# daijifeng001/MNC

Hardware: AMD Instinct MI355X
Metric: images/sec (600x1000, 300 RoIs) VGG16 MNC-5stage (higher is better)
Workload: dtype f32; 1 GPU; VGG16 MNC 5-stage inference + gpu_mask_voting; one 600x1000 uint8 image per GPU per step (8 seeded images rotating), 300 RoIs per stage, H2D + device prep + forward + tail + gpu_mask_voting + D2H of the voted instances all inside the timed region; synthetic weights; math=fp32, images_in_flight_per_gpu=12, engine=native, parallelism=single GPU

## Files before the change

### include/mnc_hip.h

```cpp
#ifndef MNC_HIP_H_
#define MNC_HIP_H_

#include <stddef.h>

#ifdef __cplusplus
extern "C" {
#endif

#define MNC_API __attribute__((visibility("default")))

enum {
  MNC_OK = 0,
  MNC_ERR_INVALID = 1,
  MNC_ERR_HIP = 2,
  MNC_ERR_NOMEM = 3,
  MNC_ERR_STATE = 4,
  MNC_ERR_UNSUPPORTED = 5
};

MNC_API const char* mnc_last_error(void);
MNC_API int mnc_device_count(int* count);
MNC_API int mnc_device_mem_info(int device_id, size_t* free_bytes, size_t* total_bytes);
MNC_API const char* mnc_version(void);

MNC_API int mnc_nms(int* keep_out, int* num_out, const float* boxes_host, int boxes_num, int boxes_dim,
                    float nms_overlap_thresh, int device_id);
MNC_API int mnc_nms_topk(int* keep_out, int* num_out, const float* boxes_host, int boxes_num, int boxes_dim,
                         float nms_overlap_thresh, int max_keep, int device_id);
MNC_API int mnc_nms_batched(int* keep_out, int* num_out, const float* boxes_host, int boxes_num, int boxes_dim,
                            const int* order_host, int batch, float nms_overlap_thresh, int max_keep, int device_id);
MNC_API int mnc_nms_mask(unsigned long long* mask_host, const float* boxes_host, int boxes_num, int boxes_dim,
                         float nms_overlap_thresh, int device_id);
#if defined(__cplusplus) && defined(MNC_HIP_REF_CXX_NAMES)
}
MNC_API void _nms(int* keep_out, int* num_out, const float* boxes_host, int boxes_num, int boxes_dim,
                  float nms_overlap_thresh, int device_id);
MNC_API void _mv(const float* all_boxes, const float* all_masks, const int all_boxes_num, const int* candidate_inds,
                 const int* candidate_start, const float* candidate_weights, const int candidate_num,
                 const int image_height, const int image_width, const int box_dim, const int mask_size,
                 const int result_num, float* finalize_output_mask, int* finalize_output_box, const int device_id);
extern "C" {
#else
MNC_API void _nms(int* keep_out, int* num_out, const float* boxes_host, int boxes_num, int boxes_dim,
                  float nms_overlap_thresh, int device_id);
#endif

MNC_API int mnc_mv(const float* all_boxes, const float* all_masks, int all_boxes_num, const int* candidate_inds,
                   const int* candidate_start, const float* candidate_weights, int candidate_num, int image_height,
                   int image_width, int box_dim, int mask_size, int result_num, float* finalize_output_mask,
                   int* finalize_output_box, int device_id);
#if !(defined(__cplusplus) && defined(MNC_HIP_REF_CXX_NAMES))
MNC_API void _mv(const float* all_boxes, const float* all_masks, const int all_boxes_num, const int* candidate_inds,
                 const int* candidate_start, const float* candidate_weights, const int candidate_num,
                 const int image_height, const int image_width, const int box_dim, const int mask_size,
                 const int result_num, float* finalize_output_mask, int* finalize_output_box, const int device_id);
#endif

MNC_API int mnc_mask_voting(const float* boxes, const float* masks, const float* scores, const int* order, int n,
                            int num_classes, int mask_size, int max_per_image, float nms_thresh, float iou_thresh,
                            int image_height, int image_width, float* out_mask, int* out_box, float* out_score,
                            int* class_count, int* result_num, int device_id);

MNC_API int mnc_mask_voting_image(const float* boxes, const float* masks, const float* scores, int n, int num_classes,
                                  int mask_size, int max_per_image, float nms_thresh, float iou_thresh, double binarize_thresh,
                                  int image_height, int image_width, float* out_mask, int* out_box, float* out_score,
                                  int* class_count, int* result_num, int device_id);

MNC_API int mnc_sds_best_overlap(const double* boxes, const unsigned char* masks, int P, int mask_size, const int* gt_begin,
                                 const int* gt_end, int G, const int* gt_bounds, const long long* gt_offsets,
                                 const unsigned char* gt_bits, size_t gt_bytes, const long long* gt_areas,
                                 double binarize_thresh, int* best_gt, long long* best_inter, long long* best_union,
                                 int device_id);

MNC_API int mnc_render_instances(const double* boxes, const float* masks, const int* classes, int n, int mask_size,
                                 double binarize_thresh, int image_height, int image_width, int* inst_img, int* cls_img,
                                 int device_id);

typedef struct mnc_mask_info {
  int x1, y1, x2, y2;
  int cls;
  float score;
  int row;
  int reserved0;
  long long offset;
  long long area;
  long long work;
  long long reserved1;
} mnc_mask_info;
typedef struct mnc_mask_head {
  int kept;
  int reserved0;
  long long bits_bytes;
  long long items;
  long long reserved1[29];
} mnc_mask_head;
MNC_API int mnc_instance_masks(const double* boxes, const float* masks, int n, int mask_size, double binarize_thresh,
                               int image_height, int image_width, int clip, int* bounds, long long* offsets, long long* areas,
                               void* bits, size_t bits_cap, size_t* bits_bytes, int device_id);

MNC_API int mnc_mask_overlaps(const int* a_bounds, const long long* a_offsets, const long long* a_areas, const void* a_bits,
                              size_t a_bytes, int na, const int* b_bounds, const long long* b_offsets, const long long* b_areas,
                              const void* b_bits, size_t b_bytes, int nb, long long* inter, double* iou, int device_id);
MNC_API int mnc_mask_nms(const int* bounds, const long long* offsets, const long long* areas, const void* bits, size_t bytes,
                         int n, const int* classes, const float* scores, double thresh, int class_aware, int* keep_out,
                         int* num_out, int device_id);

MNC_API int mnc_mask_rle(const int* bounds, const long long* offsets, const void* bits, size_t bytes, int n, int H, int W,
                         long long* run_ptr, unsigned* runs, size_t runs_cap, size_t* runs_total, int device_id);
MNC_API int mnc_mask_from_rle(const long long* run_ptr, const unsigned* runs, int n, int H, int W, int* bounds, long long* offsets,
                              long long* areas, void* bits, size_t bits_cap, size_t* bits_bytes, int device_id);

MNC_API int mnc_mask_match(const int* dt_bounds, const long long* dt_offsets, const long long* dt_areas, const void* dt_bits,
                           size_t dt_bytes, int nd, const int* dt_classes, const float* dt_scores, const int* gt_bounds,
                           const long long* gt_offsets, const long long* gt_areas, const void* gt_bits, size_t gt_bytes, int ng,
                           const int* gt_classes, const unsigned char* gt_crowd, const unsigned char* gt_ignore_in,
                           const double* gt_eval_area, const double* iou_thrs, int T, const double* area_rngs, int A, int max_det,
                           int* rank, int* dt_match, unsigned char* dt_ignore, int* gt_match, unsigned char* gt_ignore,
                           double* iou, int device_id);

MNC_API int mnc_mask_from_polygons(const double* xy, const long long* vert_ptr, const long long* poly_ptr, int n, int H, int W,
                                   int* bounds, long long* offsets, long long* areas, void* bits, size_t bits_cap,
                                   size_t* bits_bytes, int device_id);
MNC_API int mnc_mask_poly_timing(int on, double* last_ms);

MNC_API int mnc_coco_accumulate(const int* dt_class_idx, const float* dt_score, const int* dt_rank, const unsigned char* dt_flags,
                                int N, const int* gt_class_idx, const unsigned char* gt_ignore, int Gn, int K, int T, int A,
                                const int* max_dets, int M, const double* rec_thrs, int R, double* precision, double* recall,
                                long long* npig, int device_id);
MNC_API int mnc_coco_accum_timing(int on, double* last_ms);

MNC_API int mnc_mask_boundary(const int* bounds, const long long* offsets, const void* bits, size_t bytes, int n, int H, int W,
                              int d, int* out_bounds, long long* out_offsets, long long* out_areas, void* out_bits,
                              size_t bits_cap, size_t* bits_bytes, int device_id);
MNC_API int mnc_mask_match_boundary(const int* dt_bounds, const long long* dt_offsets, const long long* dt_areas, const void* dt_bits,
                                    size_t dt_bytes, int nd, const int* dt_classes, const float* dt_scores, const int* gt_bounds,
                                    const long long* gt_offsets, const long long* gt_areas, const void* gt_bits, size_t gt_bytes,
                                    int ng, const int* gt_classes, const unsigned char* gt_crowd, const unsigned char* gt_ignore_in,
                                    const double* gt_eval_area, const double* iou_thrs, int T, const double* area_rngs, int A,
                                    int max_det, int H, int W, int d, int* rank, int* dt_match, unsigned char* dt_ignore,
                                    int* gt_match, unsigned char* gt_ignore, double* iou, double* biou, int device_id);
MNC_API int mnc_mask_boundary_timing(int on, double* last_ms);

MNC_API int mnc_mask_components(const int* bounds, const long long* offsets, const void* bits, size_t bytes, int n, int connectivity,
                                long long* comp_ptr, long long* area, int* bbox, int* anchor, size_t comp_cap, size_t* n_comp,
                                int device_id);
MNC_API int mnc_mask_select(const int* bounds, const long long* offsets, const void* bits, size_t bytes, int n, int connectivity,
                            int min_area, int keep, long long* out_areas, void* out_bits, size_t bits_cap, int device_id);
MNC_API int mnc_mask_fill_holes(const int* bounds, const long long* offsets, const void* bits, size_t bytes, int n, int connectivity,
                                long long* out_areas, void* out_bits, size_t bits_cap, int device_id);
MNC_API int mnc_mask_split(const int* bounds, const long long* offsets, const void* bits, size_t bytes, int n, int connectivity,
                           int* out_bounds, long long* out_offsets, long long* out_areas, int* out_source, size_t comp_cap,
                           size_t* n_comp, void* out_bits, size_t bits_cap, size_t* bits_bytes, int device_id);
MNC_API int mnc_mask_components_timing(int on, double* last_ms);

MNC_API int mnc_mask_contours(const int* bounds, const long long* offsets, const void* bits, size_t bytes, int n, int connectivity,
                              long long* loop_ptr, long long* vert_ptr, long long* area, int* xy, size_t loop_cap, size_t vert_cap,
                              size_t* n_loops, size_t* n_verts, int device_id);
MNC_API int mnc_mask_contours_timing(int on, double* last_ms);

MNC_API int mnc_contours_simplify(const long long* vert_ptr, const int* xy, size_t n_loops, size_t n_verts, int q,
                                  long long* out_vert_ptr, int* out_xy, long long* out_index, size_t* out_verts, int device_id);
MNC_API int mnc_contours_simplify_timing(int on, double* last_ms);

MNC_API int mnc_mcg_maskdb(const int* superpixels, int H, int W, const int* label_ptr, const int* label_ids, int n,
                           int mask_size, double* boxes, unsigned char* masks, int device_id);

MNC_API int mnc_bbox_overlaps(const double* boxes, int n, const double* query_boxes, int k, double* overlaps);

typedef struct mnc_ctx mnc_ctx;

MNC_API int mnc_ctx_create(mnc_ctx** out, int device_id);
MNC_API int mnc_ctx_destroy(mnc_ctx* ctx);
MNC_API int mnc_ctx_sync(mnc_ctx* ctx);
MNC_API int mnc_ctx_device(const mnc_ctx* ctx, int* device_id);
MNC_API int mnc_ctx_arena_generation(const mnc_ctx* ctx, unsigned long* generation);

typedef struct mnc_layer_conventions {
  int warp_sample;
  int warp_round_edges;
  int warp_no_plus_one;
  int warp_oob;
  int resize_mode;
  int maskpool_binary;
  float maskpool_thresh;
  int inherit;
} mnc_layer_conventions;
MNC_API int mnc_ctx_set_layer_conventions(mnc_ctx* ctx, const mnc_layer_conventions* conv);
MNC_API int mnc_ctx_set_tuning(mnc_ctx* ctx, const char* name, const char* value);
MNC_API int mnc_ctx_get_layer_conventions(const mnc_ctx* ctx, mnc_layer_conventions* conv);

typedef struct mnc_graph mnc_graph;
MNC_API int mnc_ctx_capture_begin(mnc_ctx* ctx);
MNC_API int mnc_ctx_capture_end(mnc_ctx* ctx, mnc_graph** out);
MNC_API int mnc_graph_launch(mnc_ctx* ctx, mnc_graph* graph);
MNC_API int mnc_graph_destroy(mnc_graph* graph);
MNC_API int mnc_proposal_count_ptr(mnc_ctx* ctx, void** d_count);

MNC_API int mnc_dev_alloc(mnc_ctx* ctx, size_t bytes, void** d_ptr);
MNC_API int mnc_dev_free(mnc_ctx* ctx, void* d_ptr);
MNC_API int mnc_h2d(mnc_ctx* ctx, void* d_dst, const void* src_host, size_t bytes);
MNC_API int mnc_d2h(mnc_ctx* ctx, void* dst_host, const void* d_src, size_t bytes);
MNC_API int mnc_d2d(mnc_ctx* ctx, void* d_dst, const void* d_src, size_t bytes);
MNC_API int mnc_dev_zero(mnc_ctx* ctx, void* d_ptr, size_t bytes);
MNC_API int mnc_host_alloc(mnc_ctx* ctx, size_t bytes, void** host_ptr);
MNC_API int mnc_host_free(mnc_ctx* ctx, void* host_ptr);
MNC_API int mnc_h2d_async(mnc_ctx* ctx, void* d_dst, const void* src_host, size_t bytes);
MNC_API int mnc_d2h_async(mnc_ctx* ctx, void* dst_host, const void* d_src, size_t bytes);

MNC_API int mnc_prof_enable(mnc_ctx* ctx, int enable);
MNC_API int mnc_prof_reset(mnc_ctx* ctx);
MNC_API int mnc_prof_count(mnc_ctx* ctx, int* n_records);
MNC_API int mnc_prof_get(mnc_ctx* ctx, int index, char* name_buf, int name_cap, float* ms, double* flops,
                         double* bytes);

MNC_API int mnc_nchw_to_c8(mnc_ctx* ctx, const float* d_nchw, float* d_c8, int C, int H, int W);
MNC_API int mnc_c8_to_nchw(mnc_ctx* ctx, const float* d_c8, float* d_nchw, int C, int H, int W);
MNC_API int mnc_rchw_to_rhwc(mnc_ctx* ctx, const float* d_in, float* d_out, int R, int C, int PH, int PW);
MNC_API int mnc_rhwc_to_rchw(mnc_ctx* ctx, const float* d_in, float* d_out, int R, int C, int PH, int PW);
MNC_API int mnc_pack_conv3x3_weights(mnc_ctx* ctx, const float* d_oihw, float* d_packed, int Cout, int Cin);
MNC_API int mnc_pack_fc_weights(mnc_ctx* ctx, const float* d_nchw_cols, float* d_hwc_cols, int N, int C, int PH, int PW);

MNC_API int mnc_conv3x3_c3(mnc_ctx* ctx, const float* d_in_nchw, const float* d_w_oihw, const float* d_bias,
                           float* d_out_c8, int H, int W, int Cout, int relu);
MNC_API int mnc_conv3x3(mnc_ctx* ctx, const float* d_in_c8, const float* d_w_packed, const float* d_bias,
                        float* d_out_c8, int H, int W, int Cin, int Cout, int relu);
MNC_API int mnc_pack_conv3x3_bf16x3(mnc_ctx* ctx, const float* d_oihw, void* d_packed, int Cout, int Cin);
MNC_API int mnc_conv3x3_bf16x3(mnc_ctx* ctx, const float* d_in_c8, const void* d_w_packed, const float* d_bias,
                               float* d_out_c8, int H, int W, int Cin, int Cout, int relu);
MNC_API int mnc_pack_conv3x3_wino(mnc_ctx* ctx, const float* d_oihw, float* d_packed, int Cout, int Cin);
MNC_API int mnc_conv3x3_wino(mnc_ctx* ctx, const float* d_in_c8, const float* d_w_packed, const float* d_bias, float* d_out_c8,
                             int H, int W, int Cin, int Cout, int relu);
MNC_API int mnc_conv3x3_wino_pool(mnc_ctx* ctx, const float* d_in_c8, const float* d_w_packed, const float* d_bias,
                                  float* d_out_pooled_c8, int H, int W, int Cin, int Cout, int relu);
MNC_API int mnc_pack_conv3x3_wino4(mnc_ctx* ctx, const float* d_oihw, float* d_packed, int Cout, int Cin);
MNC_API int mnc_conv3x3_wino4(mnc_ctx* ctx, const float* d_in_c8, const float* d_w_packed, const float* d_bias, float* d_out_c8,
                              int H, int W, int Cin, int Cout, int relu);
MNC_API int mnc_conv3x3_wino4_pool(mnc_ctx* ctx, const float* d_in_c8, const float* d_w_packed, const float* d_bias,
                                   float* d_out_pooled_c8, int H, int W, int Cin, int Cout, int relu);
MNC_API int mnc_pack_conv3x3_wino4_split(mnc_ctx* ctx, const float* d_oihw, float* d_packed, int Cout, int Cin);
MNC_API size_t mnc_conv3x3_wino4_split_ws_bytes(int H, int W, int Cin, int Cout);
MNC_API int mnc_conv3x3_wino4_split_selected(mnc_ctx* ctx, int H, int W, int Cin, int Cout);
MNC_API int mnc_conv3x3_wino4_split(mnc_ctx* ctx, const float* d_in_c8, const float* d_w_split, const float* d_bias, float* d_out_c8,
                                    void* d_ws, int H, int W, int Cin, int Cout, int relu);
MNC_API int mnc_conv3x3_wino4_split_pool(mnc_ctx* ctx, const float* d_in_c8, const float* d_w_split, const float* d_bias,
                                         float* d_out_pooled_c8, void* d_ws, int H, int W, int Cin, int Cout, int relu);
MNC_API int mnc_maxpool2_c8(mnc_ctx* ctx, const float* d_in, float* d_out, int C, int H, int W);
MNC_API int mnc_conv1x1_to_nchw(mnc_ctx* ctx, const float* d_in_c8, const float* d_w, const float* d_bias,
                                float* d_out_nchw, int H, int W, int Cin, int Cout);
MNC_API int mnc_rpn_softmax(mnc_ctx* ctx, const float* d_score_nchw, float* d_prob_nchw, int A, int H, int W);
MNC_API int mnc_rpn_heads(mnc_ctx* ctx, const float* d_in_c8, const float* d_w, const float* d_bias, float* d_score_nchw,
                          float* d_prob_nchw, int H, int W, int Cin, int A);
MNC_API int mnc_roi_warp(mnc_ctx* ctx, const float* d_feat_c8, int C, int H, int W, const float* d_rois, int R,
                         int PH, int PW, float spatial_scale, int pool2, float* d_out_rhwc);
MNC_API int mnc_pack_conv_weights(mnc_ctx* ctx, const float* d_oihw, float* d_packed, int Cout, int Cin, int KH, int KW);
MNC_API int mnc_conv2d(mnc_ctx* ctx, const float* d_in_c8, const float* d_w_packed, const float* d_bias,
                       const float* d_residual_c8, float* d_out_c8, int H, int W, int Cin, int Cout, int KH, int KW, int stride,
                       int pad, int relu);
MNC_API int mnc_pack_conv_weights_f16(mnc_ctx* ctx, const float* d_oihw, void* d_packed, int Cout, int Cin, int KH, int KW);
MNC_API int mnc_conv2d_f16(mnc_ctx* ctx, const float* d_in_c8, const void* d_w_packed, const float* d_bias,
                           const float* d_residual_c8, float* d_out_c8, int H, int W, int Cin, int Cout, int KH, int KW,
                           int stride, int pad, int relu);
MNC_API int mnc_pack_conv1x1(mnc_ctx* ctx, const float* d_w, void* d_packed, int Cout, int Cin, int f16);
MNC_API int mnc_conv1x1(mnc_ctx* ctx, const float* d_in_c8, const void* d_w_packed, const float* d_bias,
                        const float* d_residual_c8, float* d_out_c8, int H, int W, int Cin, int Cout, int stride, int relu);
MNC_API int mnc_conv1x1_f16_pk(mnc_ctx* ctx, const void* d_in_pk, const void* d_w_packed, const float* d_bias,
                               const void* d_residual, void* d_out, int H, int W, int Cin, int Cout, int stride, int relu,
                               int res_packed, int out_packed);
MNC_API int mnc_conv_stem_c3(mnc_ctx* ctx, const float* d_in_nchw, const float* d_w_oihw, const float* d_bias, float* d_out_c8,
                             int H, int W, int Cout, int K, int stride, int pad, int relu);
MNC_API int mnc_conv_stem_c3_fmt(mnc_ctx* ctx, const float* d_in_nchw, const float* d_w_oihw, const float* d_bias, void* d_out,
                                 int H, int W, int Cout, int K, int stride, int pad, int relu, int out_packed);
MNC_API int mnc_pack_conv_stem_f16(mnc_ctx* ctx, const float* d_w_oihw, void* d_packed, int Cout, int K);
MNC_API int mnc_conv_stem_f16(mnc_ctx* ctx, const float* d_in_nchw, const void* d_w_packed, const float* d_bias, void* d_out, int H,
                              int W, int Cout, int K, int stride, int pad, int relu, int out_packed);
MNC_API int mnc_maxpool_c8(mnc_ctx* ctx, const float* d_in, float* d_out, int C, int H, int W, int K, int stride, int pad);
MNC_API int mnc_maxpool_c8_f16(mnc_ctx* ctx, const void* d_in, void* d_out, int C, int H, int W, int K, int stride, int pad);
MNC_API int mnc_add(mnc_ctx* ctx, const float* d_a, const float* d_b, float* d_out, size_t n, int relu);
MNC_API int mnc_prep_image(mnc_ctx* ctx, const unsigned char* d_bgr_hwc, int H, int W, const double* means_host,
                           const int* d_x0, const float* d_ax, int OW, const int* d_y0, const float* d_ay, int OH,
                           float* d_out_chw, int PH, int PW);
MNC_API int mnc_roi_pool(mnc_ctx* ctx, const float* d_feat_c8, int N, int C, int H, int W, const float* d_rois, int R,
                         int PH, int PW, float spatial_scale, float* d_out_rhwc);
MNC_API int mnc_maxpool2_rhwc(mnc_ctx* ctx, const float* d_in, float* d_out, int R, int PH, int PW, int C);
MNC_API int mnc_mask_resize(mnc_ctx* ctx, const float* d_in, float* d_out, int R, int IH, int IW, int OH, int OW);
MNC_API int mnc_mask_pool(mnc_ctx* ctx, const float* d_feat, const float* d_mask, float* d_out, int R, int PH,
                          int PW, int C, int pool2);
MNC_API int mnc_fc(mnc_ctx* ctx, const float* d_a, const float* d_w, const float* d_bias, float* d_out, int M,
                   int N, int K, int ldc, int act);
MNC_API int mnc_fc_pair(mnc_ctx* ctx, const float* d_a0, const float* d_w0, const float* d_bias0, float* d_out0, const float* d_a1,
                        const float* d_w1, const float* d_bias1, float* d_out1, int M, int N, int K, int ldc, int act);
MNC_API int mnc_fc_batch(mnc_ctx* ctx, const float* d_a, long stride_a, const float* d_w, long stride_w, float* d_out,
                         long stride_out, int B, int M, int N, int K, int ldc);
MNC_API int mnc_pack_fc_bf16x3(mnc_ctx* ctx, const float* d_w, void* d_packed, int N, int K);
MNC_API int mnc_fc_bf16x3(mnc_ctx* ctx, const float* d_a, const void* d_w_packed, const float* d_bias, float* d_out, int M,
                          int N, int K, int ldc, int act);
MNC_API size_t mnc_conv3x3_lowp_weight_bytes(int mode, int Cout, int Cin);
MNC_API int mnc_pack_conv3x3_lowp(mnc_ctx* ctx, int mode, const float* d_oihw, void* d_packed, int Cout, int Cin);
MNC_API int mnc_conv3x3_lowp(mnc_ctx* ctx, int mode, const void* d_in_packed, const void* d_w_packed, const float* d_bias,
                             void* d_out_packed, float* d_out_c8, int H, int W, int Cin, int Cout, int relu);
MNC_API int mnc_conv3x3_lowp_pool(mnc_ctx* ctx, int mode, const void* d_in_packed, const void* d_w_packed, const float* d_bias,
                                  void* d_out_pooled_packed, int H, int W, int Cin, int Cout, int relu);
MNC_API int mnc_pack_conv3x3_f16(mnc_ctx* ctx, const float* d_oihw, void* d_packed, int Cout, int Cin);
MNC_API int mnc_pack_conv3x3_bf16(mnc_ctx* ctx, const float* d_oihw, void* d_packed, int Cout, int Cin);
MNC_API int mnc_conv3x3_bf16(mnc_ctx* ctx, const float* d_in_c8, const void* d_w_packed, const float* d_bias, float* d_out_c8,
                             int H, int W, int Cin, int Cout, int relu);
MNC_API int mnc_conv3x3_f16(mnc_ctx* ctx, const float* d_in_c8, const void* d_w_packed, const float* d_bias, float* d_out_c8,
                            int H, int W, int Cin, int Cout, int relu);
MNC_API int mnc_conv3x3_bf16x3_pk(mnc_ctx* ctx, const void* d_in, const void* d_w_packed, const float* d_bias, void* d_out,
                                  int H, int W, int Cin, int Cout, int relu, int in_packed, int out_packed);
MNC_API int mnc_conv3x3_f16_pk(mnc_ctx* ctx, const void* d_in, const void* d_w_packed, const float* d_bias, void* d_out,
                               int H, int W, int Cin, int Cout, int relu, int in_packed, int out_packed);
MNC_API int mnc_conv3x3_bf16_pk(mnc_ctx* ctx, const void* d_in, const void* d_w_packed, const float* d_bias, void* d_out,
                                int H, int W, int Cin, int Cout, int relu, int in_packed, int out_packed);
MNC_API int mnc_conv3x3_c3_fmt(mnc_ctx* ctx, const float* d_in_nchw, const float* d_w_oihw, const float* d_bias, void* d_out,
                               int H, int W, int Cout, int relu, int out_fmt);
MNC_API int mnc_maxpool2_c8_bf16x3(mnc_ctx* ctx, const void* d_in, void* d_out, int C, int H, int W);
MNC_API int mnc_maxpool2_c8_f16(mnc_ctx* ctx, const void* d_in, void* d_out, int C, int H, int W);
MNC_API int mnc_maxpool2_c8_bf16(mnc_ctx* ctx, const void* d_in, void* d_out, int C, int H, int W);
MNC_API int mnc_act_pack(mnc_ctx* ctx, const float* d_c8, void* d_packed, size_t n, int f16);
MNC_API int mnc_act_unpack(mnc_ctx* ctx, const void* d_packed, float* d_c8, size_t n, int f16);
MNC_API int mnc_pack_fc_f16(mnc_ctx* ctx, const float* d_w, void* d_packed, int N, int K);
MNC_API int mnc_pack_fc_bf16(mnc_ctx* ctx, const float* d_w, void* d_packed, int N, int K);
MNC_API int mnc_fc_bf16(mnc_ctx* ctx, const float* d_a, const void* d_w_packed, const float* d_bias, float* d_out, int M, int N,
                        int K, int ldc, int act);
MNC_API int mnc_fc_f16(mnc_ctx* ctx, const float* d_a, const void* d_w_packed, const float* d_bias, float* d_out, int M, int N,
                       int K, int ldc, int act);
MNC_API int mnc_fc_lowp_pair(mnc_ctx* ctx, int mode, const float* d_a0, const void* d_a_sm0, const float* d_a1, const void* d_a_sm1,
                             int m_stride, const void* d_w0, const void* d_w1, const float* d_bias0, const float* d_bias1,
                             float* d_out0, float* d_out1, int M, int N, int K, int ldc, int act, void* d_out_sm0, void* d_out_sm1,
                             int out_sm_fmt);
MNC_API int mnc_fc_pack_act(mnc_ctx* ctx, const float* d_a, void* d_a_sm, int M, int K, int f16);
MNC_API int mnc_fc_unpack_act(mnc_ctx* ctx, const void* d_a_sm, float* d_a, int M, int K, int fmt);
MNC_API int mnc_roi_warp_sm_only_ok(mnc_ctx* ctx, int C, int pool2, int* ok);
MNC_API int mnc_fc_f16_pre(mnc_ctx* ctx, const void* d_a_sm, int m_stride, const void* d_w_packed, const float* d_bias,
                           float* d_out, int M, int N, int K, int ldc, int act);
MNC_API int mnc_fc_bf16x3_pre(mnc_ctx* ctx, const void* d_a_sm, int m_stride, const void* d_w_packed, const float* d_bias,
                              float* d_out, int M, int N, int K, int ldc, int act);
MNC_API int mnc_fc_f16_ex(mnc_ctx* ctx, const float* d_a, const void* d_a_sm, int m_stride, const void* d_w_packed,
                          const float* d_bias, float* d_out, int M, int N, int K, int ldc, int act, void* d_out_sm, int out_sm_fmt);
MNC_API int mnc_fc_bf16x3_ex(mnc_ctx* ctx, const float* d_a, const void* d_a_sm, int m_stride, const void* d_w_packed,
                             const float* d_bias, float* d_out, int M, int N, int K, int ldc, int act, void* d_out_sm,
                             int out_sm_fmt);
MNC_API int mnc_fc_bf16_ex(mnc_ctx* ctx, const float* d_a, const void* d_a_sm, int m_stride, const void* d_w_packed,
                           const float* d_bias, float* d_out, int M, int N, int K, int ldc, int act, void* d_out_sm, int out_sm_fmt);
MNC_API int mnc_roi_warp_sm(mnc_ctx* ctx, const float* d_feat_c8, int C, int H, int W, const float* d_rois, int R, int PH, int PW,
                            float spatial_scale, int pool2, float* d_out_rhwc, void* d_sm, int sm_fmt);
MNC_API int mnc_maxpool2_rhwc_sm(mnc_ctx* ctx, const float* d_in, float* d_out, int R, int PH, int PW, int C, void* d_sm,
                                 int sm_fmt);
MNC_API int mnc_mask_pool_sm(mnc_ctx* ctx, const float* d_feat, const float* d_mask, float* d_out, int R, int PH, int PW, int C,
                             int pool2, void* d_sm, int sm_fmt);
MNC_API int mnc_box_mask_pool(mnc_ctx* ctx, const float* d_feat, const float* d_mask, float* d_box_out, float* d_mask_out, int R,
                              int PH, int PW, int C, void* d_box_sm, void* d_mask_sm, int sm_fmt);
MNC_API int mnc_box_mask_pool_ex(mnc_ctx* ctx, const float* d_feat, const void* d_feat_sm, int feat_sm_fmt, const float* d_mask,
                                 float* d_box_out, float* d_mask_out, int R, int PH, int PW, int C, void* d_box_sm, void* d_mask_sm,
                                 int sm_fmt);
MNC_API int mnc_softmax_rows(mnc_ctx* ctx, const float* d_in, float* d_out, int M, int N);
MNC_API int mnc_softmax_rows_ld(mnc_ctx* ctx, const float* d_in, int ld_in, float* d_out, int M, int N);
MNC_API int mnc_eltwise(mnc_ctx* ctx, const float* d_in, float* d_out, size_t count, int op);
MNC_API int mnc_copy2d(mnc_ctx* ctx, float* d_dst, int dst_ld, const float* d_src, int src_ld, int rows, int cols);

MNC_API int mnc_proposal(mnc_ctx* ctx, const float* d_cls_prob, const float* d_bbox_pred, int A, int H, int W,
                         const float* anchors_host, int feat_stride, float im_h, float im_w, float im_scale,
                         int pre_nms_topn, int post_nms_topn, float nms_thresh, float min_size, float* d_rois,
                         int* num_rois_host);
MNC_API int mnc_mask_voting_dev(mnc_ctx* ctx, const float* d_boxes, const float* d_masks, const float* d_scores, int n,
                                int num_classes, int mask_size, int max_per_image, float nms_thresh, float iou_thresh,
                                int image_height, int image_width, float* out_mask, int* out_box, float* out_score,
                                int* class_count, int* result_num);
MNC_API int mnc_vote_instances(mnc_ctx* ctx, const float* d_boxes, const float* d_masks, const float* d_scores, int n,
                               int num_classes, int mask_size, int max_per_image, float nms_thresh, float iou_thresh,
                               int image_height, int image_width, float* d_records, int record_cap, int* d_counts);
#define MNC_VOTE_MV 0
#define MNC_VOTE_IMAGE 1
MNC_API int mnc_vote_instances_ex(mnc_ctx* ctx, int mode, const float* d_boxes, const float* d_masks, const float* d_scores,
                                  int n, int num_classes, int mask_size, int max_per_image, float nms_thresh, float iou_thresh,
                                  double binarize_thresh, int image_height, int image_width, float* d_records, int record_cap,
                                  int* d_counts);
MNC_API int mnc_render_records(mnc_ctx* ctx, const float* d_records, const int* d_counts, int record_cap, int num_classes,
                               int mask_size, double vis_thresh, double binarize_thresh, int H, int W,
                               const unsigned char* d_bgr_hwc, float alpha, int* d_inst, int* d_cls, unsigned char* d_inst_rgb,
                               unsigned char* d_cls_rgb, unsigned char* d_overlay_rgb, int* d_kept);
MNC_API int mnc_mask_records(mnc_ctx* ctx, const float* d_records, const int* d_counts, int record_cap, int num_classes,
                             int mask_size, double score_thresh, double binarize_thresh, int H, int W, void** d_info,
                             void** d_bits);
MNC_API int mnc_mask_overlaps_dev(mnc_ctx* ctx, const void* d_info, const void* d_bits, int rows_cap, const int* b_bounds,
                                  const long long* b_offsets, const long long* b_areas, const void* b_bits, size_t b_bytes, int nb,
                                  void** d_inter, void** d_iou);
MNC_API int mnc_mask_nms_dev(mnc_ctx* ctx, const void* d_info, const void* d_bits, int rows_cap, double thresh, int class_aware,
                             void** d_keep);
MNC_API int mnc_mask_rle_dev(mnc_ctx* ctx, const void* d_info, const void* d_bits, int rows_cap, int H, int W, size_t runs_cap,
                             void** d_rle);
MNC_API int mnc_mask_match_dev(mnc_ctx* ctx, const void* d_info, const void* d_bits, int rows_cap, const int* gt_bounds,
                               const long long* gt_offsets, const long long* gt_areas, const void* gt_bits, size_t gt_bytes, int ng,
                               const int* gt_classes, const unsigned char* gt_crowd, const unsigned char* gt_ignore_in,
                               const double* gt_eval_area, const double* iou_thrs, int T, const double* area_rngs, int A,
                               int max_det, int want_iou, void** d_rank, void** d_dt_match, void** d_dt_ignore, void** d_gt_match,
                               void** d_gt_ignore, void** d_iou);
MNC_API int mnc_detect_tail(mnc_ctx* ctx, const float* d_rois1, int R1, const float* d_rois2, int R2, float scale,
                            int image_height, int image_width, float* d_boxes);

MNC_API int mnc_proposal_count(mnc_ctx* ctx, int* num_rois_host);
MNC_API int mnc_proposal_candidates(mnc_ctx* ctx, float* boxes_host, float* scores_host, int capacity, int* n_host);
MNC_API int mnc_stage_bridge(mnc_ctx* ctx, const float* d_rois, const float* d_bbox_pred, int ld_bbox, const float* d_probs,
                             int ld_probs, int R, int K, float im_h, float im_w, float* d_rois_ext);

typedef struct mnc_net mnc_net;
typedef struct mnc_net_config {
  int trunk_channels[5];
  int rpn_channels;
  int num_anchors;
  float anchors[64];
  int feat_stride;
  int pre_nms_topn, post_nms_topn;
  float rpn_nms_thresh, rpn_min_size;
  int mask_fc, mask_size;
  int fc_dim;
  int num_classes;
  int roi_size;
  float spatial_scale;
  int target_size, max_size;
  double pixel_means[3];
  int max_per_image;
  float vote_nms_thresh, vote_iou_thresh;
  int math;
  int use_graph;
  int winograd;
  mnc_layer_conventions conventions;
} mnc_net_config;

MNC_API int mnc_net_default_config(mnc_net_config* cfg);
MNC_API int mnc_net_create(mnc_ctx* ctx, const mnc_net_config* cfg, mnc_net** out);
MNC_API int mnc_net_create_shared(mnc_ctx* ctx, mnc_net* parent, mnc_net** out);
MNC_API int mnc_net_set_param(mnc_net* net, const char* layer, int index, const float* data_host, size_t count);
MNC_API int mnc_net_load_file(mnc_net* net, const char* path);
MNC_API int mnc_net_set_voting(mnc_net* net, int mode, double binarize_thresh);
MNC_API int mnc_forward_image(mnc_net* net, const unsigned char* bgr_host, int H, int W, float* records_host, int record_cap,
                              int* counts_host);
MNC_API int mnc_forward_image_async(mnc_net* net, const unsigned char* bgr_host, int H, int W, float** d_records, int** d_counts);
MNC_API int mnc_net_fetch(mnc_net* net, float* records_host, int record_cap, int* counts_host);
MNC_API int mnc_net_render(mnc_net* net, double vis_thresh, double binarize_thresh, float alpha, int* inst_host, int* cls_host,
                           unsigned char* inst_rgb_host, unsigned char* cls_rgb_host, unsigned char* overlay_rgb_host,
                           int* kept_host);
MNC_API int mnc_net_masks(mnc_net* net, double score_thresh, double binarize_thresh, void* info_host, int info_cap,
                          void* bits_host, size_t bits_cap, size_t* bits_bytes);
MNC_API int mnc_net_blob(mnc_net* net, const char* name, void** d_ptr, int* dims, int* ndim);
MNC_API int mnc_net_destroy(mnc_net* net);

MNC_API int mnc_comm_unique_id(void* id_out, int capacity_bytes);
MNC_API int mnc_comm_init(mnc_ctx* ctx, const void* id, int nranks, int rank);
MNC_API int mnc_comm_info(mnc_ctx* ctx, int* nranks, int* rank, int* rccl_version);
MNC_API int mnc_gather_instances(mnc_ctx* ctx, const float* d_send, float* d_recv, size_t floats_per_rank);
MNC_API int mnc_comm_destroy(mnc_ctx* ctx);

#ifdef __cplusplus
}
#endif
#endif
```

### mnc_amd/csrc/conv_wino4_split.hip

```cpp
#include "mnc_internal.h"

namespace mnc {

typedef float s4f __attribute__((ext_vector_type(4)));

__device__ __forceinline__ s4f fma4(float s, s4f a, s4f b) {
  return s4f{fmaf(s, a.x, b.x), fmaf(s, a.y, b.y), fmaf(s, a.z, b.z), fmaf(s, a.w, b.w)};
}

__device__ __forceinline__ void bt6(const s4f (&d)[6], s4f (&x)[6]) {
  const s4f a = fma4(-4.f, d[2], d[4]), b = fma4(-4.f, d[1], d[3]), c = d[4] - d[2], e = d[3] - d[1];
  x[0] = fma4(4.f, d[0], fma4(-5.f, d[2], d[4]));
  x[1] = a + b;
  x[2] = a - b;
  x[3] = fma4(2.f, e, c);
  x[4] = fma4(-2.f, e, c);
  x[5] = fma4(4.f, d[1], fma4(-5.f, d[3], d[5]));
}

__device__ __forceinline__ void at6(const s4f (&m)[6], s4f (&y)[4]) {
  const s4f s12 = m[1] + m[2], d12 = m[1] - m[2], s34 = m[3] + m[4], d34 = m[3] - m[4];
  y[0] = (m[0] + s12) + s34;
  y[1] = fma4(2.f, d34, d12);
  y[2] = fma4(4.f, s34, s12);
  y[3] = fma4(8.f, d34, d12) + m[5];
}

__global__ __launch_bounds__(256) void wino4_split_input_kernel(const float* __restrict__ in, float* __restrict__ V, int H, int W, int Cin,
                                                                int tiles_x, int ntiles) {
  const int c4n = Cin >> 2;
  const long total = (long)ntiles * c4n;
  const long idx = (long)blockIdx.x * blockDim.x + threadIdx.x;
  if (idx >= total) return;
  const int c4 = (int)(idx % c4n), tile = (int)(idx / c4n);
  const int ty = tile / tiles_x, tx = tile - ty * tiles_x;
  const int y0 = 4 * ty - 1, x0 = 4 * tx - 1;
  const float* src = in + (long)(c4 >> 1) * H * W * 8 + (c4 & 1) * 4;
  s4f t[6][6];
#pragma unroll
  for (int j = 0; j < 6; ++j) {
    s4f d[6], x[6];
    const int xx = x0 + j;
#pragma unroll
    for (int i = 0; i < 6; ++i) {
      const int yy = y0 + i;
      d[i] = s4f{0.f, 0.f, 0.f, 0.f};
      if (yy >= 0 && yy < H && xx >= 0 && xx < W) d[i] = *reinterpret_cast<const s4f*>(src + ((long)yy * W + xx) * 8);
    }
    bt6(d, x);
#pragma unroll
    for (int i = 0; i < 6; ++i) t[i][j] = x[i];
  }
  float* dst = V + (long)tile * Cin + c4 * 4;
  const long pstride = (long)ntiles * Cin;
#pragma unroll
  for (int i = 0; i < 6; ++i) {
    s4f x[6];
    bt6(t[i], x);
#pragma unroll
    for (int j = 0; j < 6; ++j) *reinterpret_cast<s4f*>(dst + (long)(6 * i + j) * pstride) = x[j];
  }
}

template <int POOL>
__global__ __launch_bounds__(256) void wino4_split_output_kernel(const float* __restrict__ Mt, const float* __restrict__ bias,
                                                                 float* __restrict__ out, int H, int W, int Cout, int relu, int tiles_x,
                                                                 int ntiles) {
  const int c4n = Cout >> 2;
  const long total = (long)ntiles * c4n;
  const long idx = (long)blockIdx.x * blockDim.x + threadIdx.x;
  if (idx >= total) return;
  const int c4 = (int)(idx % c4n), tile = (int)(idx / c4n);
  const int ty = tile / tiles_x, tx = tile - ty * tiles_x;
  const int oy = 4 * ty, ox = 4 * tx;
  const float* src = Mt + (long)tile * Cout + c4 * 4;
  const long pstride = (long)ntiles * Cout;
  s4f z[4][6];
#pragma unroll
  for (int j = 0; j < 6; ++j) {
    s4f m[6], y[4];
#pragma unroll
    for (int i = 0; i < 6; ++i) m[i] = *reinterpret_cast<const s4f*>(src + (long)(6 * i + j) * pstride);
    at6(m, y);
#pragma unroll
    for (int i = 0; i < 4; ++i) z[i][j] = y[i];
  }
  const s4f bv = *reinterpret_cast<const s4f*>(bias + c4 * 4);
  s4f y[4][4];
#pragma unroll
  for (int i = 0; i < 4; ++i) {
    at6(z[i], y[i]);
#pragma unroll
    for (int j = 0; j < 4; ++j) {
      y[i][j] += bv;
      if (relu) y[i][j] = s4f{fmaxf(y[i][j].x, 0.f), fmaxf(y[i][j].y, 0.f), fmaxf(y[i][j].z, 0.f), fmaxf(y[i][j].w, 0.f)};
    }
  }
  const int cb = c4 >> 1, half = (c4 & 1) * 4;
  if (!POOL) {
#pragma unroll
    for (int i = 0; i < 4; ++i)
#pragma unroll
      for (int j = 0; j < 4; ++j)
        if (oy + i < H && ox + j < W) *reinterpret_cast<s4f*>(out + (((long)cb * H + oy + i) * W + ox + j) * 8 + half) = y[i][j];
  } else {
    const int OH = (H + 1) >> 1, OW = (W + 1) >> 1;
#pragma unroll
    for (int pi = 0; pi < 2; ++pi)
#pragma unroll
      for (int pj = 0; pj < 2; ++pj) {
        const int py = oy + 2 * pi, px = ox + 2 * pj;
        if (py >= H || px >= W) continue;
        s4f best = y[2 * pi][2 * pj];
#pragma unroll
        for (int di = 0; di < 2; ++di)
#pragma unroll
          for (int dj = 0; dj < 2; ++dj)
            if (py + di < H && px + dj < W) {
              const s4f o = y[2 * pi + di][2 * pj + dj];
              best = s4f{fmaxf(best.x, o.x), fmaxf(best.y, o.y), fmaxf(best.z, o.z), fmaxf(best.w, o.w)};
            }
        *reinterpret_cast<s4f*>(out + (((long)cb * OH + (py >> 1)) * OW + (px >> 1)) * 8 + half) = best;
      }
  }
}

__global__ __launch_bounds__(256) void pack_conv3x3_wino4_split_kernel(const float* __restrict__ w, float* __restrict__ U, int Cout,
                                                                       int Cin) {
  const double G[6][3] = {{6.0, 0.0, 0.0}, {-4.0, -4.0, -4.0}, {-4.0, 4.0, -4.0}, {1.0, 2.0, 4.0}, {1.0, -2.0, 4.0}, {0.0, 0.0, 24.0}};
  const long total = (long)Cout * Cin;
  for (long r = (long)blockIdx.x * blockDim.x + threadIdx.x; r < total; r += (long)gridDim.x * blockDim.x) {
    const float* f = w + r * 9;
    for (int a = 0; a < 6; ++a) {
      double tmp[3];
#pragma unroll
      for (int b = 0; b < 3; ++b) tmp[b] = G[a][0] * (double)f[b] + G[a][1] * (double)f[3 + b] + G[a][2] * (double)f[6 + b];
#pragma unroll
      for (int b = 0; b < 6; ++b)
        U[(long)(6 * a + b) * total + r] = (float)((tmp[0] * G[b][0] + tmp[1] * G[b][1] + tmp[2] * G[b][2]) / 576.0);
    }
  }
}

bool wino4_split_supported(int H, int W, int Cin, int Cout) {
  return H > 0 && W > 0 && Cin > 0 && Cin % 32 == 0 && Cout > 0 && Cout % 32 == 0 &&
         36.0 * cdiv(H, 4) * (double)cdiv(W, 4) * (Cin > Cout ? Cin : Cout) * 4.0 < 2.0e9;
}

bool wino4_split_selected(const mnc_ctx* ctx, int H, int W, int Cin, int Cout) {
  const int v = tune(ctx, T_WINO_SPLIT, kWinoSplitDefault);
  if (v == 0 || !wino4_split_supported(H, W, Cin, Cout)) return false;
  if (v == 2) return true;
  if (plan_latency(ctx)) return false;
  return wino4_split_plan_channels(Cin, Cout) && cdiv(H, 4) * cdiv(W, 4) >= 304;
}

static size_t wino4_split_v_bytes(int H, int W, int Cin) {
  return ((size_t)36 * cdiv(W, 4) * cdiv(H, 4) * Cin * 4 + 255) & ~(size_t)255;
}

static int wino4_split_impl(mnc_ctx* ctx, const float* d_in, const float* d_u, const float* d_bias, float* d_out, void* d_ws, int H,
                            int W, int Cin, int Cout, int relu, int pool) {
  MNC_REQUIRE(ctx && d_in && d_u && d_bias && d_out && d_ws, "mnc_conv3x3_wino4_split: null pointer");
  MNC_REQUIRE((reinterpret_cast<uintptr_t>(d_ws) & 15) == 0, "mnc_conv3x3_wino4_split: workspace not 16-byte aligned");
  MNC_REQUIRE(wino4_split_supported(H, W, Cin, Cout),
              "mnc_conv3x3_wino4_split: unsupported shape H=%d W=%d Cin=%d Cout=%d (need Cin%%32==0, Cout%%32==0)", H, W, Cin, Cout);
  const int tiles_x = cdiv(W, 4), ntiles = tiles_x * cdiv(H, 4);
  float* V = (float*)d_ws;
  float* Mt = (float*)((char*)d_ws + wino4_split_v_bytes(H, W, Cin));
  const double flops = 2.0 * H * W * 9.0 * Cin * Cout;
  const double out_px = pool ? (double)((H + 1) / 2) * ((W + 1) / 2) : (double)H * W;
  const double bytes = 4.0 * ((double)H * W * Cin + out_px * Cout + 9.0 * Cin * Cout);
  LaunchScope ls(ctx, "conv3x3_wino4_mfma", flops, bytes);
  const long in_items = (long)ntiles * (Cin >> 2), out_items = (long)ntiles * (Cout >> 2);
  hipLaunchKernelGGL(wino4_split_input_kernel, dim3((unsigned)((in_items + 255) / 256)), dim3(256), 0, ctx->stream, d_in, V, H, W, Cin,
                     tiles_x, ntiles);
  int rc = fc_batch_launch(ctx, V, (long)ntiles * Cin, d_u, (long)Cout * Cin, Mt, (long)ntiles * Cout, 36, ntiles, Cout, Cin, Cout);
  if (rc) {
    (void)ls.finish("conv3x3_wino4_split");
    return rc;
  }
  if (pool)
    hipLaunchKernelGGL(wino4_split_output_kernel<1>, dim3((unsigned)((out_items + 255) / 256)), dim3(256), 0, ctx->stream, Mt, d_bias,
                       d_out, H, W, Cout, relu, tiles_x, ntiles);
  else
    hipLaunchKernelGGL(wino4_split_output_kernel<0>, dim3((unsigned)((out_items + 255) / 256)), dim3(256), 0, ctx->stream, Mt, d_bias,
                       d_out, H, W, Cout, relu, tiles_x, ntiles);
  return ls.finish("conv3x3_wino4_split");
}

}

using namespace mnc;

extern "C" {

int mnc_pack_conv3x3_wino4_split(mnc_ctx* ctx, const float* d_oihw, float* d_packed, int Cout, int Cin) {
  MNC_REQUIRE(ctx && d_oihw && d_packed && Cin > 0 && Cin % 32 == 0 && Cout > 0 && Cout % 32 == 0,
              "mnc_pack_conv3x3_wino4_split: bad argument (Cin%%32==0, Cout%%32==0)");
  LaunchScope ls(ctx, "pack_conv3x3_wino4_split");
  long g = ((long)Cout * Cin + 255) / 256;
  if (g > 8192) g = 8192;
  hipLaunchKernelGGL(pack_conv3x3_wino4_split_kernel, dim3((int)g), dim3(256), 0, ctx->stream, d_oihw, d_packed, Cout, Cin);
  return ls.finish("pack_conv3x3_wino4_split_kernel");
}

size_t mnc_conv3x3_wino4_split_ws_bytes(int H, int W, int Cin, int Cout) {
  if (!wino4_split_supported(H, W, Cin, Cout)) return 0;
  return wino4_split_v_bytes(H, W, Cin) + (size_t)36 * cdiv(W, 4) * cdiv(H, 4) * Cout * 4;
}

int mnc_conv3x3_wino4_split_selected(mnc_ctx* ctx, int H, int W, int Cin, int Cout) {
  return ctx && wino4_split_selected(ctx, H, W, Cin, Cout) ? 1 : 0;
}

int mnc_conv3x3_wino4_split(mnc_ctx* ctx, const float* d_in, const float* d_u, const float* d_bias, float* d_out, void* d_ws, int H,
                            int W, int Cin, int Cout, int relu) {
  return wino4_split_impl(ctx, d_in, d_u, d_bias, d_out, d_ws, H, W, Cin, Cout, relu, 0);
}

int mnc_conv3x3_wino4_split_pool(mnc_ctx* ctx, const float* d_in, const float* d_u, const float* d_bias, float* d_out_pooled,
                                 void* d_ws, int H, int W, int Cin, int Cout, int relu) {
  MNC_REQUIRE(H >= 2 && W >= 2, "mnc_conv3x3_wino4_split_pool: map %dx%d too small for MAX 2x2/2", H, W);
  return wino4_split_impl(ctx, d_in, d_u, d_bias, d_out_pooled, d_ws, H, W, Cin, Cout, relu, 1);
}

}
```

### mnc_amd/csrc/gemm.hip

```cpp
#include <atomic>
#include <type_traits>
#include <cstdlib>

#include "fc_plan.h"
#include "mnc_internal.h"
#include "x3_split.h"

namespace mnc {

typedef float f32x16 __attribute__((ext_vector_type(16)));

constexpr int kBN = 128, kBK = 32;

__device__ __forceinline__ float apply_act(float v, int act) {
  if (act == 1) return fmaxf(v, 0.f);
  if (act == 2) return 1.0f / (1.0f + expf(-v));
  return v;
}

template <int kMT, int kSK = 32, int ABL = 0>
__global__ __launch_bounds__(256) void fc_mfma_kernel(const float* __restrict__ A, const float* __restrict__ Wt,
                                                      const float* __restrict__ bias, float* __restrict__ out,
                                                      float* __restrict__ part, int M, int N, int K, int ldc, int kper,
                                                      int act, int fused, int tn_, int splits_, int tm_) {
// ... 90 lines not shown
#pragma unroll
    for (int t = 0; t < kMT; ++t) acc[t] = __builtin_amdgcn_mfma_f32_32x32x2f32(f.a[t].z, f.b.z, acc[t], 0, 0, 0);
#pragma unroll
    for (int t = 0; t < kMT; ++t) acc[t] = __builtin_amdgcn_mfma_f32_32x32x2f32(f.a[t].w, f.b.w, acc[t], 0, 0, 0);
  };
  auto pin_acc = [&]() {
#pragma unroll
    for (int t = 0; t < kMT; ++t) asm volatile("" : "+a"(acc[t]));
  };
  constexpr int kNM = 4 * kMT;
  constexpr int kNR = kMT + 1;
  constexpr int kNS = kAPer + kBPer;
  auto stage_io = [&](int s, int buf, Regs& cur, Regs& nxt) {
    if (ABL == 0) store_stage(buf ^ 1, cur, s + 1 < nstages);
    if (ABL == 4) {
#pragma unroll
      for (int u = 0; u < kAPer; ++u) asm volatile("" :: "v"(cur.a[u].x));
#pragma unroll
      for (int u = 0; u < kBPer; ++u) asm volatile("" :: "v"(cur.b[u].x));
    }
  };
  auto step = [&](int s, int buf, Regs& cur, Regs& nxt, Frags& f0) {
    Frags f1;
    if (ABL == 0 || ABL == 4) load_stage(s + 2, nxt);
    read_frags(buf, 1, f1);
    mfmas(f0);
    stage_io(s, buf, cur, nxt);
    if (kNG == 4) {
      read_frags(buf, 2, f0);
      mfmas(f1);
      read_frags(buf, 3, f1);
      mfmas(f0);
    }
    constexpr int kG1 = kNG - 1;
#pragma unroll
    for (int i = 0; i < kG1 * kNM; ++i) {
      __builtin_amdgcn_sched_group_barrier(0x008, 1, 0);
      if (ABL != 3 && (i + 1) * kG1 * kNR / (kG1 * kNM) > i * kG1 * kNR / (kG1 * kNM)) __builtin_amdgcn_sched_group_barrier(0x100, 1, 0);
      if ((ABL == 0 || ABL == 4) && (i + 1) * kNS / (kG1 * kNM) > i * kNS / (kG1 * kNM))
        __builtin_amdgcn_sched_group_barrier(0x020, 1, 0);
      if (ABL == 0 && (i + 1) * kNS / (kG1 * kNM) > i * kNS / (kG1 * kNM)) __builtin_amdgcn_sched_group_barrier(0x200, 1, 0);
    }
    pin_acc();
    if (ABL < 2) __syncthreads();
    read_frags(buf ^ 1, 0, f0);
    mfmas(f1);
#pragma unroll
    for (int i = 0; i < kNM; ++i) {
      __builtin_amdgcn_sched_group_barrier(0x008, 1, 0);
      if (ABL != 3 && (i + 1) * kNR / kNM > i * kNR / kNM) __builtin_amdgcn_sched_group_barrier(0x100, 1, 0);
    }
    pin_acc();
  };

  if (nstages > 0) {
    Frags F0;
    load_stage(0, R0);
    store_stage(0, R0, true);
    load_stage(1, R0);
    __syncthreads();
    read_frags(0, 0, F0);
    for (int s = 0; s < nstages; s += 2) {
      step(s, 0, R0, R1, F0);
      step(s + 1, 1, R1, R0, F0);
    }
  }

  const int n = n0 + wave * 32 + j;
  if (n < N) {
    const float bv = fused ? bias[n] : 0.f;
#pragma unroll
    for (int t = 0; t < kMT; ++t) {
      if (t < mtiles) {
#pragma unroll
        for (int e = 0; e < 16; ++e) {
          const int m = m0 + t * 32 + (e & 3) + 8 * (e >> 2) + 4 * kk;
          if (m < M) {
            if (fused) out[(long)m * ldc + n] = apply_act(acc[t][e] + bv, act);
            else part[((long)split * M + m) * N + n] = acc[t][e];
          }
        }
      }
    }
  }
}

template <int kMT, int ABL = 0, int kWM = 1, int HALF = 0>
__global__ __launch_bounds__(256 * kWM) void fc_mfma_dma_kernel(const float* __restrict__ A, const float* __restrict__ Wt,
                                                          const float* __restrict__ bias, float* __restrict__ out,
                                                          float* __restrict__ part, int M, int N, int K, int ldc, int kper,
                                                          int act, int fused, int tn_, int splits_, int tm_) {
  constexpr int kBM = 32 * kMT;
  constexpr int kRows = kBM + kBN;
  constexpr int kNW = 4 * kWM;
  constexpr int TR = kMT / kWM;
  constexpr int kPer = kRows * 128 / 1024 / kNW;
  static_assert(kRows % (8 * kNW) == 0 && kMT % kWM == 0, "whole pieces and row tiles per wave");
  extern __shared__ __attribute__((aligned(1024))) char s_fc_dma[];
  constexpr int kBufXor = 65536;
  const int tid = threadIdx.x, lane = tid & 63;
  const int wave = __builtin_amdgcn_readfirstlane(tid >> 6);
  const int wn = wave & 3, wm = wave >> 2;
  const int j = lane & 31, kk = lane >> 5;
  int bn, split, bmz;
  xcd_decode(blockIdx.x, tn_, splits_, tm_, bn, split, bmz);
  const int n0 = bn * kBN, m0 = bmz * kBM;
  const int kbeg = split * kper, kend = min(K, kbeg + kper);
  const int nstages = (kend - kbeg) / 32;
  const int mrows = min(M - m0, kBM);
  const int mtiles = (mrows + 31) >> 5;

  const float* src[kPer];
#pragma unroll
  for (int i = 0; i < kPer; ++i) {
    const int slot = (wave + kNW * i) * 64 + lane, r = slot >> 3, c = (slot & 7) ^ ((r >> 1) & 7);
    src[i] = (r < kBM ? A + (long)(m0 + min(r, mrows - 1)) * K
                      : Wt + (long)min(n0 + r - kBM, N - 1) * K) + kbeg + c * 4;
  }
  const unsigned lds0 = (unsigned)(unsigned long)(__attribute__((address_space(3))) char*)s_fc_dma;
  auto dma_piece = [&](int i, long off, int buf_byte) {
    if (ABL == 3 && wave + kNW * i >= kBM / 8) off = 0;
    const float* g = src[i] + off;
    const unsigned l = __builtin_amdgcn_readfirstlane(lds0 + (unsigned)buf_byte + (unsigned)(wave + kNW * i) * 1024u);
    asm volatile("s_mov_b32 m0, %1\n\ts_nop 0\n\tglobal_load_lds_dwordx4 %0, off" ::"v"(g), "s"(l));
  };
  auto dma_stage = [&](int s, int buf_byte) {
    const long off = ABL == 1 ? 0 : (long)min(s, nstages - 1) * 32;
#pragma unroll
    for (int i = 0; i < kPer; ++i) dma_piece(i, off, buf_byte);
  };
  auto dma_wait = [&]() { asm volatile("s_waitcnt vmcnt(0)" ::: "memory"); };

  f32x16 acc[TR];
#pragma unroll
  for (int t = 0; t < TR; ++t)
#pragma unroll
    for (int e = 0; e < 16; ++e) acc[t][e] = 0.f;

  constexpr bool kHalf = HALF != 0;
  static_assert(!kHalf || (kWM == 2 && ABL == 0), "the half tile exists in the eight-wave product build only");
  const bool last_wave = kHalf && wm == kWM - 1;
  typedef float f32x4v __attribute__((ext_vector_type(4)));
  f32x4v hacc[2] = {{0.f, 0.f, 0.f, 0.f}, {0.f, 0.f, 0.f, 0.f}};
  const int r16 = lane & 15, g4 = lane >> 4;
  int h_off[8];
#pragma unroll
  for (int c = 0; c < 8; ++c)
    h_off[c] = ((2 * (c >> 1) + (g4 & 1)) ^ ((r16 >> 1) & 7)) * 16 + (2 * (c & 1) + (g4 >> 1)) * 4;
  const int ha_base = ((kMT - 1) * 32 + r16) * 128, hb_base = (kBM + wn * 32 + r16) * 128;
  int hflip = 0;

  int a_off[4], b_off[4];
#pragma unroll
  for (int kc = 0; kc < 4; ++kc) {
    const int c = (2 * kc + kk) ^ ((j >> 1) & 7);
    a_off[kc] = ((wm * TR * 32 + j) * 32 + c * 4) * 4;
    b_off[kc] = ((kBM + wn * 32 + j) * 32 + c * 4) * 4;
  }
  struct Frags { float4 a[TR]; float4 b; float ha[2]; float hb[2][2]; };
  auto read_frags = [&](int kc, int flip, Frags& f, auto last_tag) {
    constexpr bool LAST = decltype(last_tag)::value;
    f.b = *reinterpret_cast<const float4*>(s_fc_dma + (b_off[kc] ^ flip));
#pragma unroll
    for (int t = 0; t < (LAST ? TR - 1 : TR); ++t) f.a[t] = *reinterpret_cast<const float4*>(s_fc_dma + (a_off[kc] ^ flip) + t * 4096);
    if (LAST) {
      const int hf = hflip ^ flip;
#pragma unroll
      for (int h = 0; h < 2; ++h) {
        f.ha[h] = *reinterpret_cast<const float*>(s_fc_dma + ((ha_base + h_off[2 * kc + h]) ^ hf));
        f.hb[h][0] = *reinterpret_cast<const float*>(s_fc_dma + ((hb_base + h_off[2 * kc + h]) ^ hf));
        f.hb[h][1] = *reinterpret_cast<const float*>(s_fc_dma + ((hb_base + 2048 + h_off[2 * kc + h]) ^ hf));
      }
    }
  };
  auto half_mfmas = [&](const Frags& f) {
    hacc[0] = __builtin_amdgcn_mfma_f32_16x16x4f32(f.ha[0], f.hb[0][0], hacc[0], 0, 0, 0);
    hacc[1] = __builtin_amdgcn_mfma_f32_16x16x4f32(f.ha[0], f.hb[0][1], hacc[1], 0, 0, 0);
    hacc[0] = __builtin_amdgcn_mfma_f32_16x16x4f32(f.ha[1], f.hb[1][0], hacc[0], 0, 0, 0);
    hacc[1] = __builtin_amdgcn_mfma_f32_16x16x4f32(f.ha[1], f.hb[1][1], hacc[1], 0, 0, 0);
  };
  auto mfmas = [&](const Frags& f, auto last_tag) {
    constexpr bool LAST = decltype(last_tag)::value;
    constexpr int NT = LAST ? TR - 1 : TR;
#pragma unroll
    for (int t = 0; t < NT; ++t) acc[t] = __builtin_amdgcn_mfma_f32_32x32x2f32(f.a[t].x, f.b.x, acc[t], 0, 0, 0);
#pragma unroll
    for (int t = 0; t < NT; ++t) acc[t] = __builtin_amdgcn_mfma_f32_32x32x2f32(f.a[t].y, f.b.y, acc[t], 0, 0, 0);
    if (LAST) half_mfmas(f);
#pragma unroll
    for (int t = 0; t < NT; ++t) acc[t] = __builtin_amdgcn_mfma_f32_32x32x2f32(f.a[t].z, f.b.z, acc[t], 0, 0, 0);
#pragma unroll
    for (int t = 0; t < NT; ++t) acc[t] = __builtin_amdgcn_mfma_f32_32x32x2f32(f.a[t].w, f.b.w, acc[t], 0, 0, 0);
  };
  auto pin_acc = [&]() {
#pragma unroll
    for (int t = 0; t < TR; ++t) asm volatile("" : "+a"(acc[t]));
  };

  auto run = [&](auto last_tag) {
    constexpr bool LAST = decltype(last_tag)::value;
    constexpr int NT = LAST ? TR - 1 : TR;
    constexpr int kNM = 4 * NT + (LAST ? 4 : 0), kNR = NT + 1 + (LAST ? 6 : 0);
    Frags f0, f1;
    dma_stage(0, 0);
    dma_stage(1, kBufXor);
    dma_wait();
    __syncthreads();
    read_frags(0, 0, f0, last_tag);
    int cur = 0;
    for (int s = 0; s < nstages; ++s) {
      read_frags(1, 0, f1, last_tag);
      mfmas(f0, last_tag);
      read_frags(2, 0, f0, last_tag);
      mfmas(f1, last_tag);
      read_frags(3, 0, f1, last_tag);
      mfmas(f0, last_tag);
#pragma unroll
      for (int i = 0; i < 3 * kNM; ++i) {
        __builtin_amdgcn_sched_group_barrier(0x008, 1, 0);
        if ((i + 1) * 3 * kNR / (3 * kNM) > i * 3 * kNR / (3 * kNM)) __builtin_amdgcn_sched_group_barrier(0x100, 1, 0);
      }
      pin_acc();
      dma_wait();
      __syncthreads();
      read_frags(0, kBufXor, f0, last_tag);
      {
        const long off = ABL == 1 ? 0 : (long)min(s + 2, nstages - 1) * 32;
#pragma unroll
        for (int q = 0; q < 4; ++q) {
#pragma unroll
          for (int t = 0; t < NT; ++t) {
            const int i = q * NT + t;
            const float av = q == 0 ? f1.a[t].x : q == 1 ? f1.a[t].y : q == 2 ? f1.a[t].z : f1.a[t].w;
            const float bv = q == 0 ? f1.b.x : q == 1 ? f1.b.y : q == 2 ? f1.b.z : f1.b.w;
            acc[t] = __builtin_amdgcn_mfma_f32_32x32x2f32(av, bv, acc[t], 0, 0, 0);
            if (i >= 4 * NT - kPer - 2 && i < 4 * NT - 2) {
              __builtin_amdgcn_sched_barrier(0);
              dma_piece(i - (4 * NT - kPer - 2), off, cur);
              __builtin_amdgcn_sched_barrier(0);
            }
          }
          if (LAST && q == 0) half_mfmas(f1);
        }
      }
      pin_acc();
#pragma unroll
      for (int kc = 0; kc < 4; ++kc) { a_off[kc] ^= kBufXor; b_off[kc] ^= kBufXor; }
      hflip ^= kBufXor;
      cur ^= kBufXor;
    }
    dma_wait();
    __syncthreads();
  };
  if (nstages > 0) {
    if (last_wave) run(std::true_type{});
    else run(std::false_type{});
  }

  const int n = n0 + wn * 32 + j;
  if (n < N) {
    const float bv = fused ? bias[n] : 0.f;
#pragma unroll
    for (int t = 0; t < TR; ++t) {
      if (last_wave && t == TR - 1) continue;
      if (wm * TR + t < mtiles) {
#pragma unroll
        for (int e = 0; e < 16; ++e) {
          const int m = m0 + (wm * TR + t) * 32 + (e & 3) + 8 * (e >> 2) + 4 * kk;
          if (m < M) {
            if (fused) out[(long)m * ldc + n] = apply_act(acc[t][e] + bv, act);
            else part[((long)split * M + m) * N + n] = acc[t][e];
          }
        }
      }
    }
  }
  if (last_wave) {
#pragma unroll
    for (int ch = 0; ch < 2; ++ch) {
      const int nh = n0 + wn * 32 + ch * 16 + r16;
      if (nh >= N) continue;
      const float bh = fused ? bias[nh] : 0.f;
#pragma unroll
      for (int e = 0; e < 4; ++e) {
        const int m = m0 + (kMT - 1) * 32 + 4 * g4 + e;
        if (m < M) {
          if (fused) out[(long)m * ldc + nh] = apply_act(hacc[ch][e] + bh, act);
          else part[((long)split * M + m) * N + nh] = hacc[ch][e];
        }
      }
    }
  }
}

template <int kMT, int ABL = 0, int BUF = 0, int BATCH = 0>
__global__ __launch_bounds__(512) void fc_mfma_dma16_kernel(const float* __restrict__ A_0, const float* __restrict__ Wt_0,
                                                            const float* __restrict__ bias_0, float* __restrict__ out_0,
                                                            float* __restrict__ part_0, int M, int N, int K, int ldc, int kper,
                                                            int act, int fused, int tn_, int splits_, int tm_, int drop_last,
                                                            const float* __restrict__ A_1,
                                                            const float* __restrict__ Wt_1, const float* __restrict__ bias_1,
                                                            float* __restrict__ out_1, int pair_tn, long batch_a,
                                                            long batch_w, long batch_o) {
  constexpr int kBM = 32 * kMT;
  constexpr int kRows = kBM + kBN;
  constexpr int kNW = 8;
  constexpr int TS = kMT;
  constexpr int kPer = kRows * 128 / 1024 / kNW;
  static_assert(kRows % (8 * kNW) == 0 && kMT % 2 == 0, "whole pieces and row tiles per wave");
  extern __shared__ __attribute__((aligned(1024))) char s_fc_dma[];
  constexpr int kBufXor = 65536;
  const int tid = threadIdx.x, lane = tid & 63;
  const int wave = __builtin_amdgcn_readfirstlane(tid >> 6);
  const int wn = wave & 3, wm = wave >> 2;
  const int r16 = lane & 15, g4 = lane >> 4;
  int bn, split, bmz;
  xcd_decode(blockIdx.x, tn_, splits_, tm_, bn, split, bmz);
  int which = (pair_tn && bn >= pair_tn) ? 1 : 0;
  bn -= which * pair_tn;
  if (BATCH) { which = bmz; bmz = split; split = 0; }
  const float* __restrict__ A = BATCH ? A_0 + which * batch_a : which ? A_1 : A_0;
  const float* __restrict__ Wt = BATCH ? Wt_0 + which * batch_w : which ? Wt_1 : Wt_0;
  const float* __restrict__ bias = which ? bias_1 : bias_0;
  float* __restrict__ out = BATCH ? out_0 + which * batch_o : which ? out_1 : out_0;
  float* __restrict__ part = part_0;
  constexpr int kLive = kBM - 16;
  const int n0 = bn * kBN, m0 = bmz * (BATCH && drop_last ? kLive : kBM);
  const int kbeg = split * kper, kend = min(K, kbeg + kper);
  const int nstages = (kend - kbeg) / 32;
  const int mrows = min(M - m0, BATCH && drop_last ? kLive : kBM);

  const float* src[kPer];
#pragma unroll
  for (int i = 0; i < kPer; ++i) {
    const int slot = (wave + kNW * i) * 64 + lane, r = slot >> 3, c = (slot & 7) ^ ((r >> 1) & 7);
    src[i] = (r < kBM ? A + (long)(m0 + min(r, mrows - 1)) * K
                      : Wt + (long)min(n0 + r - kBM, N - 1) * K) + kbeg + c * 4;
  }
  const unsigned lds0 = (unsigned)(unsigned long)(__attribute__((address_space(3))) char*)s_fc_dma;
  typedef int i32x4d __attribute__((ext_vector_type(4)));
  auto make_rsrc = [](const float* base) {
    const unsigned long a = (unsigned long)base;
    i32x4d r;
    r.x = __builtin_amdgcn_readfirstlane((int)(unsigned)a);
    r.y = __builtin_amdgcn_readfirstlane((int)((unsigned)(a >> 32) & 0xFFFFu));
    r.z = 0x70000000;
    r.w = 0x00020000;
    return r;
  };
  const i32x4d rs_a = make_rsrc(A + (long)m0 * K + kbeg), rs_w = make_rsrc(Wt + (long)min(n0, N - 1) * K + kbeg);
  int voff[kPer];
#pragma unroll
  for (int i = 0; i < kPer; ++i) {
    const int slot = (wave + kNW * i) * 64 + lane, r = slot >> 3, c = (slot & 7) ^ ((r >> 1) & 7);
    voff[i] = (r < kBM ? min(r, mrows - 1) * K : (min(n0 + r - kBM, N - 1) - min(n0, N - 1)) * K) * 4 + c * 16;
  }
  auto dma_piece = [&](int i, long off, int buf_byte, bool in_loop = false) {
    const unsigned l = __builtin_amdgcn_readfirstlane(lds0 + (unsigned)buf_byte + (unsigned)(wave + kNW * i) * 1024u);
    if (BUF) {
      const bool is_a = (wave + kNW * i) * 8 < kBM;
      const i32x4d rs = is_a ? rs_a : rs_w;
      const int so = __builtin_amdgcn_readfirstlane((int)off * 4);
      const int vo = ((ABL & 4) && in_loop) ? 0x7FFFFFF0 : voff[i];
      asm volatile("s_mov_b32 m0, %3\n\ts_nop 0\n\tbuffer_load_dwordx4 %0, %1, %2 offen lds" ::"v"(vo), "s"(rs), "s"(so), "s"(l) : "memory");
    } else {
      const float* g = src[i] + off;
      asm volatile("s_mov_b32 m0, %1\n\ts_nop 0\n\tglobal_load_lds_dwordx4 %0, off" ::"v"(g), "s"(l));
    }
  };
  auto dma_stage = [&](int s, int buf_byte) {
    const long off = (long)min(s, nstages - 1) * 32;
#pragma unroll
    for (int i = 0; i < kPer; ++i) dma_piece(i, off, buf_byte);
  };
  auto dma_wait = [&]() { asm volatile("s_waitcnt vmcnt(0)" ::: "memory"); };

  typedef float f32x4v __attribute__((ext_vector_type(4)));
  f32x4v acc[TS][2];
#pragma unroll
  for (int i = 0; i < TS; ++i)
#pragma unroll
    for (int c = 0; c < 2; ++c) acc[i][c] = f32x4v{0.f, 0.f, 0.f, 0.f};

  int a_off[2], b_off[2];
#pragma unroll
  for (int G = 0; G < 2; ++G) {
    const int sl = ((4 * G + g4) ^ ((r16 >> 1) & 7)) * 16;
    a_off[G] = (wm * TS * 16 + r16) * 128 + sl;
    b_off[G] = (kBM + wn * 32 + r16) * 128 + sl;
  }
  const bool last_wave = drop_last && wm == 1;

  auto run = [&](auto last_tag) {
    constexpr int NS = decltype(last_tag)::value ? TS - 1 : TS;
    constexpr int kNM = 8 * NS, kNR = NS + 2;
    struct Frags { f32x4v a[NS]; f32x4v b[2]; };
    auto read_frags = [&](int G, int flip, Frags& f) {
      f.b[0] = *reinterpret_cast<const f32x4v*>(s_fc_dma + (b_off[G] ^ flip));
      f.b[1] = *reinterpret_cast<const f32x4v*>(s_fc_dma + (b_off[G] ^ flip) + 2048);
#pragma unroll
      for (int i = 0; i < NS; ++i) f.a[i] = *reinterpret_cast<const f32x4v*>(s_fc_dma + (a_off[G] ^ flip) + i * 2048);
    };
    Frags f0, f1;
    dma_stage(0, 0);
    dma_stage(1, kBufXor);
    static_assert(kPer == 7, "the literal in the wait below");
    asm volatile("s_waitcnt vmcnt(7)" ::: "memory");
    __syncthreads();
    read_frags(0, 0, f0);
    int cur = 0;
    for (int s = 0; s < nstages; ++s) {
      read_frags(1, 0, f1);
#pragma unroll
      for (int q = 0; q < 4; ++q)
#pragma unroll
        for (int i = 0; i < NS; ++i) {
          acc[i][0] = __builtin_amdgcn_mfma_f32_16x16x4f32(f0.a[i][q], f0.b[0][q], acc[i][0], 0, 0, 0);
          acc[i][1] = __builtin_amdgcn_mfma_f32_16x16x4f32(f0.a[i][q], f0.b[1][q], acc[i][1], 0, 0, 0);
        }
#pragma unroll
      for (int i = 0; i < kNM; ++i) {
        __builtin_amdgcn_sched_group_barrier(0x008, 1, 0);
        if ((i + 1) * 2 * kNR / kNM > i * 2 * kNR / kNM && i * 2 < kNM) __builtin_amdgcn_sched_group_barrier(0x100, 1, 0);
      }
      dma_wait();
      if (!(ABL & 2)) __syncthreads();
      read_frags(0, kBufXor, f0);
      {
        const long off = (long)min(s + 2, nstages - 1) * 32;
#pragma unroll
        for (int q = 0; q < 4; ++q)
#pragma unroll
          for (int i = 0; i < NS; ++i) {
            acc[i][0] = __builtin_amdgcn_mfma_f32_16x16x4f32(f1.a[i][q], f1.b[0][q], acc[i][0], 0, 0, 0);
            acc[i][1] = __builtin_amdgcn_mfma_f32_16x16x4f32(f1.a[i][q], f1.b[1][q], acc[i][1], 0, 0, 0);
            const int m = 2 * (q * NS + i);
            if (m >= kNM - 4 * kPer - 8 && m < kNM - 8 && (m - (kNM - 4 * kPer - 8)) % 4 == 0) {
              __builtin_amdgcn_sched_barrier(0);
              if (!(ABL & 1)) dma_piece((m - (kNM - 4 * kPer - 8)) / 4, off, cur, true);
              __builtin_amdgcn_sched_barrier(0);
            }
          }
      }
#pragma unroll
      for (int G = 0; G < 2; ++G) { a_off[G] ^= kBufXor; b_off[G] ^= kBufXor; }
      cur ^= kBufXor;
    }
    dma_wait();
    __syncthreads();
  };
  if (nstages > 0) {
    if (last_wave) run(std::true_type{});
    else run(std::false_type{});
  }

  const bool final_out = fused == 1;
  if (BATCH) {
#pragma unroll
    for (int c = 0; c < 2; ++c) {
      const int n = n0 + wn * 32 + c * 16 + r16;
      if (n >= N) continue;
#pragma unroll
      for (int i = 0; i < TS; ++i)
#pragma unroll
        for (int e = 0; e < 4; ++e) {
          const int r = wm * TS * 16 + i * 16 + 4 * g4 + e;
          if (r < mrows) out[(long)(m0 + r) * ldc + n] = acc[i][c][e];
        }
    }
    return;
  }
  if (fused == 0) {
    constexpr int kSlabF4 = kNW * TS * 2 * 64;
    const int tile = bmz * tn_ + which * pair_tn + bn;
    f32x4v* slab = reinterpret_cast<f32x4v*>(part) + ((size_t)tile * splits_ + split) * kSlabF4 + wave * TS * 2 * 64 + lane;
#pragma unroll
    for (int i = 0; i < TS; ++i)
#pragma unroll
      for (int c = 0; c < 2; ++c) slab[(i * 2 + c) * 64] = acc[i][c];
    return;
  }
#pragma unroll
  for (int c = 0; c < 2; ++c) {
    const int n = n0 + wn * 32 + c * 16 + r16;
    if (n >= N) continue;
    const float bv = final_out ? bias[n] : 0.f;
#pragma unroll
    for (int i = 0; i < TS; ++i)
#pragma unroll
      for (int e = 0; e < 4; ++e) {
        const int m = m0 + wm * TS * 16 + i * 16 + 4 * g4 + e;
        if (m < M) {
          out[(long)m * ldc + n] = apply_act(acc[i][c][e] + bv, act);
        }
      }
  }
}

__global__ __launch_bounds__(256) void fc_reduce_slab_kernel(const float* __restrict__ part, const float* __restrict__ bias0,
                                                             const float* __restrict__ bias1, float* __restrict__ out0,
                                                             float* __restrict__ out1, int M, int N, int ldc, int splits, int act,
                                                             int tn_all, int pair_tn, int ntiles) {
  constexpr int kSlabF4 = 8 * 10 * 2 * 64;
  typedef float f32x4v __attribute__((ext_vector_type(4)));
  const f32x4v* p4 = reinterpret_cast<const f32x4v*>(part);
  const long total = (long)ntiles * kSlabF4;
  for (long idx = (long)blockIdx.x * blockDim.x + threadIdx.x; idx < total; idx += (long)gridDim.x * blockDim.x) {
    const int tile = (int)(idx / kSlabF4), piece = (int)(idx - (long)tile * kSlabF4);
    const int lane = piece & 63, ic = (piece >> 6) % 20, wave = piece / (64 * 20);
    const int i = ic >> 1, c = ic & 1, wn = wave & 3, wm = wave >> 2, r16 = lane & 15, g4 = lane >> 4;
    const int bmz = tile / tn_all;
    int bn = tile - bmz * tn_all;
    const int which = (pair_tn && bn >= pair_tn) ? 1 : 0;
    bn -= which * pair_tn;
    const int n = bn * kBN + wn * 32 + c * 16 + r16;
    const int m0 = bmz * 320 + wm * 160 + i * 16 + 4 * g4;
    if (n >= N || m0 >= M) continue;
    const f32x4v* src = p4 + (long)tile * splits * kSlabF4 + piece;
    f32x4v v = {0.f, 0.f, 0.f, 0.f};
    int sp = 0;
    for (; sp + 4 <= splits; sp += 4) {
      const f32x4v a = src[(long)sp * kSlabF4], b = src[(long)(sp + 1) * kSlabF4], cc = src[(long)(sp + 2) * kSlabF4],
                   d = src[(long)(sp + 3) * kSlabF4];
      v = (((v + a) + b) + cc) + d;
    }
    for (; sp < splits; ++sp) v += src[(long)sp * kSlabF4];
    const float bv = (which ? bias1 : bias0)[n];
    float* o = (which ? out1 : out0) + (long)m0 * ldc + n;
#pragma unroll
    for (int e = 0; e < 4; ++e)
      if (m0 + e < M) o[(long)e * ldc] = apply_act(v[e] + bv, act);
  }
}

template <int VEC, int SM = 0>
__global__ __launch_bounds__(256) void fc_reduce_kernel(const float* __restrict__ part, const float* __restrict__ bias,
                                                        float* __restrict__ out, int M, int N, int ldc, int splits,
                                                        int act, void* __restrict__ sm = nullptr, long sm_rows = 0,
                                                        long sm_row0 = 0, const float* __restrict__ part1 = nullptr,
                                                        const float* __restrict__ bias1 = nullptr, float* __restrict__ out1 = nullptr,
                                                        void* __restrict__ sm1 = nullptr) {
  if (blockIdx.y) { part = part1; bias = bias1; out = out1; sm = sm1; }
  const long total = (long)M * N;
  if (VEC == 4) {
    const int n4 = N >> 2;
    const long total4 = total >> 2;
    const float4* p4 = reinterpret_cast<const float4*>(part);
    for (long i = (long)blockIdx.x * blockDim.x + threadIdx.x; i < total4; i += (long)gridDim.x * blockDim.x) {
      const int n = (int)(i % n4) * 4;
      const long m = i / n4;
      float4 v = make_float4(0.f, 0.f, 0.f, 0.f);
      int s = 0;
      for (; s + 4 <= splits; s += 4) {
        const float4 a = p4[(long)s * total4 + i], b = p4[(long)(s + 1) * total4 + i], c = p4[(long)(s + 2) * total4 + i],
                     d = p4[(long)(s + 3) * total4 + i];
        v.x = (((v.x + a.x) + b.x) + c.x) + d.x;
        v.y = (((v.y + a.y) + b.y) + c.y) + d.y;
        v.z = (((v.z + a.z) + b.z) + c.z) + d.z;
        v.w = (((v.w + a.w) + b.w) + c.w) + d.w;
      }
      for (; s < splits; ++s) {
        const float4 a = p4[(long)s * total4 + i];
        v.x += a.x; v.y += a.y; v.z += a.z; v.w += a.w;
      }
      const float4 b = *reinterpret_cast<const float4*>(bias + n);
      const float4 y =
          make_float4(apply_act(v.x + b.x, act), apply_act(v.y + b.y, act), apply_act(v.z + b.z, act), apply_act(v.w + b.w, act));
      *reinterpret_cast<float4*>(out + m * ldc + n) = y;
      if (SM) sm_store4<SM>(sm, sm_rows, sm_row0 + m, n, y);
    }
    return;
  }
  for (long idx = (long)blockIdx.x * blockDim.x + threadIdx.x; idx < total; idx += (long)gridDim.x * blockDim.x) {
    const int n = (int)(idx % N);
    const long m = idx / N;
    float v = 0.f;
    for (int s = 0; s < splits; ++s) v += part[(long)s * total + idx];
    out[m * ldc + n] = apply_act(v + bias[n], act);
  }
}

void fc_reduce_launch(hipStream_t stream, const float* part, const float* bias, float* out, int M, int N, int ldc, int splits,
                      int act) {
  fc_reduce_launch_sm(stream, part, bias, out, M, N, ldc, splits, act, nullptr, 0, 0, 0);
}

bool fc_reduce_launch_sm(hipStream_t stream, const float* part, const float* bias, float* out, int M, int N, int ldc, int splits,
                         int act, void* sm, int sm_fmt, long sm_rows, long sm_row0) {
  const bool vec = N % 4 == 0 && ldc % 4 == 0 && (reinterpret_cast<uintptr_t>(out) & 15) == 0 &&
                   (reinterpret_cast<uintptr_t>(bias) & 15) == 0;
  const long items = vec ? (long)M * N / 4 : (long)M * N;
  int g = (int)((items + 255) / 256);
  if (g > 4096) g = 4096;
  const bool sm_ok = sm && vec && (((sm_fmt == 1 || sm_fmt == 3) && N % 64 == 0) || (sm_fmt == 2 && N % 32 == 0));
  if (sm_ok && sm_fmt == 1)
    hipLaunchKernelGGL((fc_reduce_kernel<4, 1>), dim3(g), dim3(256), 0, stream, part, bias, out, M, N, ldc, splits, act, sm, sm_rows, sm_row0);
  else if (sm_ok && sm_fmt == 3)
    hipLaunchKernelGGL((fc_reduce_kernel<4, 3>), dim3(g), dim3(256), 0, stream, part, bias, out, M, N, ldc, splits, act, sm, sm_rows, sm_row0);
  else if (sm_ok)
    hipLaunchKernelGGL((fc_reduce_kernel<4, 2>), dim3(g), dim3(256), 0, stream, part, bias, out, M, N, ldc, splits, act, sm, sm_rows, sm_row0);
  else if (vec) hipLaunchKernelGGL((fc_reduce_kernel<4, 0>), dim3(g), dim3(256), 0, stream, part, bias, out, M, N, ldc, splits, act, nullptr, 0L, 0L);
  else hipLaunchKernelGGL((fc_reduce_kernel<1, 0>), dim3(g), dim3(256), 0, stream, part, bias, out, M, N, ldc, splits, act, nullptr, 0L, 0L);
  return sm_ok;
}

bool fc_reduce_pair_launch_sm(hipStream_t stream, const float* part0, const float* part1, const float* bias0, const float* bias1,
                              float* out0, float* out1, int M, int N, int ldc, int splits, int act, void* sm0, void* sm1, int sm_fmt,
                              long sm_rows, bool* sm_done) {
  const bool vec = N % 4 == 0 && ldc % 4 == 0 && ((reinterpret_cast<uintptr_t>(out0) | reinterpret_cast<uintptr_t>(out1) |
                                                   reinterpret_cast<uintptr_t>(bias0) | reinterpret_cast<uintptr_t>(bias1)) & 15) == 0;
  if (!vec || (sm0 != nullptr) != (sm1 != nullptr)) return false;
  const long items = (long)M * N / 4;
  int g = (int)((items + 255) / 256);
  if (g > 4096) g = 4096;
  const bool sm_ok = sm0 && (((sm_fmt == 1 || sm_fmt == 3) && N % 64 == 0) || (sm_fmt == 2 && N % 32 == 0));
  if (sm_ok && sm_fmt == 1)
    hipLaunchKernelGGL((fc_reduce_kernel<4, 1>), dim3(g, 2), dim3(256), 0, stream, part0, bias0, out0, M, N, ldc, splits, act, sm0, sm_rows, 0L,
                       part1, bias1, out1, sm1);
  else if (sm_ok && sm_fmt == 3)
    hipLaunchKernelGGL((fc_reduce_kernel<4, 3>), dim3(g, 2), dim3(256), 0, stream, part0, bias0, out0, M, N, ldc, splits, act, sm0, sm_rows, 0L,
                       part1, bias1, out1, sm1);
  else if (sm_ok)
    hipLaunchKernelGGL((fc_reduce_kernel<4, 2>), dim3(g, 2), dim3(256), 0, stream, part0, bias0, out0, M, N, ldc, splits, act, sm0, sm_rows, 0L,
                       part1, bias1, out1, sm1);
  else
    hipLaunchKernelGGL((fc_reduce_kernel<4, 0>), dim3(g, 2), dim3(256), 0, stream, part0, bias0, out0, M, N, ldc, splits, act, (void*)nullptr, 0L,
                       0L, part1, bias1, out1, (void*)nullptr);
  *sm_done = sm_ok;
  return true;
}

__global__ void softmax_rows_kernel(const float* __restrict__ in, int ld_in, float* __restrict__ out, int M, int N) {
  const int m = blockIdx.x * blockDim.x + threadIdx.x;
  if (m >= M) return;
  const float* r = in + (long)m * ld_in;
  float mx = r[0];
  for (int i = 1; i < N; ++i) mx = fmaxf(mx, r[i]);
  float sum = 0.f;
  for (int i = 0; i < N; ++i) sum += expf(r[i] - mx);
  for (int i = 0; i < N; ++i) out[(long)m * N + i] = expf(r[i] - mx) / sum;
}

__global__ __launch_bounds__(256) void softmax_rows_wave_kernel(const float* __restrict__ in, int ld_in,
                                                                float* __restrict__ out, int M, int N) {
  const int lane = threadIdx.x & 63;
  const int m = blockIdx.x * (blockDim.x >> 6) + (threadIdx.x >> 6);
  if (m >= M) return;
  const bool live = lane < N;
  const float v = live ? in[(long)m * ld_in + lane] : -INFINITY;
  float mx = v;
  for (int o = 32; o > 0; o >>= 1) mx = fmaxf(mx, __shfl_xor(mx, o));
  const float e = live ? expf(v - mx) : 0.f;
  float sum = 0.f;
  for (int i = 0; i < N; ++i) sum += __shfl(e, i);
  if (live) out[(long)m * N + lane] = e / sum;
}

__global__ void eltwise_kernel(const float* __restrict__ in, float* __restrict__ out, size_t n, int op) {
  for (size_t i = (size_t)blockIdx.x * blockDim.x + threadIdx.x; i < n; i += (size_t)gridDim.x * blockDim.x)
    out[i] = apply_act(in[i], op);
}

__global__ void pack_fc_kernel(const float* __restrict__ in, float* __restrict__ out, long N, int C, int P) {
  const long total = N * C * P;
  for (long idx = (long)blockIdx.x * blockDim.x + threadIdx.x; idx < total; idx += (long)gridDim.x * blockDim.x) {
    const int c = (int)(idx % C);
    const long r = idx / C;
    const int p = (int)(r % P);
    const long n = r / P;
    out[idx] = in[(n * C + c) * P + p];
  }
}

int fc_batch_launch(mnc_ctx* ctx, const float* d_a, long stride_a, const float* d_w, long stride_w, float* d_out, long stride_o, int B,
                    int M, int N, int K, int ldc) {
  MNC_REQUIRE(ctx && d_a && d_w && d_out, "fc_batch: null pointer");
  MNC_REQUIRE(B > 0 && M > 0 && N > 0 && K > 0 && K % kBK == 0 && ldc >= N && stride_a >= 0 && stride_w >= 0 && stride_o >= 0,
              "fc_batch: unsupported shape B=%d M=%d N=%d K=%d ldc=%d (need K%%32==0)", B, M, N, K, ldc);
  MNC_REQUIRE(320.0 * (double)K * 4.0 < 1.8e9 && stride_a % 4 == 0 && stride_w % 4 == 0 &&
                  ((reinterpret_cast<uintptr_t>(d_a) | reinterpret_cast<uintptr_t>(d_w)) & 15) == 0,
              "fc_batch: operands must be 16-byte aligned, K=%d below the descriptor range", K);
  const int drop = cdiv(M, 304) == cdiv(M, 320) ? 1 : 0;
  const int tn = cdiv(N, kBN), tm = cdiv(M, drop ? 304 : 320);
  MNC_REQUIRE((double)B * tn * tm < 2.0e9, "fc_batch: too many workgroups");
  constexpr int lds = 65536 + (320 + kBN) * 32 * 4;
  MNC_HIP_TRY((lds_limit_once<fc_mfma_dma16_kernel<10, 0, 1, 1>>(ctx->device, lds)));
  hipLaunchKernelGGL((fc_mfma_dma16_kernel<10, 0, 1, 1>), dim3(B * tn * tm), dim3(512), lds, ctx->stream, d_a, d_w, (const float*)nullptr,
                     d_out, (float*)nullptr, M, N, K, ldc, K, 0, 1, tn, tm, B, drop, (const float*)nullptr, (const float*)nullptr,
                     (const float*)nullptr, (float*)nullptr, 0, stride_a, stride_w, stride_o);
  return MNC_OK;
}

}

using namespace mnc;

extern "C" {

int mnc_fc(mnc_ctx* ctx, const float* d_a, const float* d_w, const float* d_bias, float* d_out, int M, int N, int K,
           int ldc, int act) {
  MNC_REQUIRE(ctx && d_a && d_w && d_bias && d_out, "mnc_fc: null pointer");
  MNC_REQUIRE(M >= 0 && N > 0 && K > 0 && K % kBK == 0 && ldc >= N && act >= 0 && act <= 2,
              "mnc_fc: unsupported shape M=%d N=%d K=%d ldc=%d act=%d (need K%%32==0)", M, N, K, ldc, act);
  if (M == 0) return MNC_OK;
  const FcPlan p = fc_plan(FcCall(M, N, K, ldc), ctx->tune, kTuningBuild);
  if (p.head) {
    const int head = p.head;
    const bool defer = ctx->defer_reduce;
    ctx->defer_reduce = false;
    int rc = mnc_fc(ctx, d_a, d_w, d_bias, d_out, head, N, K, ldc, act);
    if (!rc) rc = mnc_fc(ctx, d_a + (size_t)head * K, d_w, d_bias, d_out + (size_t)head * ldc, M - head, N, K, ldc, act);
    ctx->defer_reduce = defer;
    ctx->deferred_part = nullptr;
    ctx->deferred_splits = 1;
    return rc;
  }
  const int mt = p.mt, tn = p.tn, tm = p.tm, splits = p.splits, kper = p.kper;
  const bool small = p.small, dma = p.kernel == kFcDma16, slab = p.slab;
  float* part = nullptr;
  if (splits > 1) {
    int rc = ensure_scratch(ctx, p.part_bytes);
    if (rc) return rc;
    part = (float*)ctx->scratch.p;
  }
  const double flops = 2.0 * M * (double)N * K, bytes = 4.0 * ((double)N * K + (double)M * K + (double)M * N);
  {
    LaunchScope ls(ctx, small ? "fc_mfma_small" : "fc_mfma", flops, bytes);
#define MNC_FC_LAUNCH(MT, SK, A) hipLaunchKernelGGL((fc_mfma_kernel<MT, SK, A>), dim3(tn * splits * tm), dim3(256), 0, ctx->stream, \
                         d_a, d_w, d_bias, d_out, part, M, N, K, ldc, kper, act, splits == 1 ? 1 : 0, tn, splits, tm)
#define MNC_FC_DMA_LAUNCH(A, WM) MNC_FC_DMA_LAUNCH_H(A, WM, 0)
#define MNC_FC_DMA_LAUNCH_H(A, WM, H)                                                                                               \
  do {                                                                                                                              \
    MNC_HIP_TRY((lds_limit_once<fc_mfma_dma_kernel<10, A, WM, H>>(ctx->device, lds)));                                              \
    hipLaunchKernelGGL((fc_mfma_dma_kernel<10, A, WM, H>), dim3(tn * splits * tm), dim3(256 * WM), lds, ctx->stream, d_a, d_w, d_bias, \
                       d_out, part, M, N, K, ldc, kper, act, splits == 1 ? 1 : 0, tn, splits, tm);                                  \
  } while (0)
    if (dma) {
      constexpr int lds = 65536 + (320 + kBN) * 32 * 4;
      bool launched = false;
#ifdef MNC_TUNING
      const int waves = tune(ctx, T_FC_DMA_WAVES, 8), dabl = tune(ctx, T_FC_DMA_ABL, 0);
      if (dabl >= 16) {
        launched = true;
        auto kern = dabl == 17 ? fc_mfma_dma16_kernel<10, 1> : dabl == 18 ? fc_mfma_dma16_kernel<10, 2> : dabl == 19 ? fc_mfma_dma16_kernel<10, 3>
                    : dabl == 20 ? fc_mfma_dma16_kernel<10, 0, 1> : dabl == 21 ? fc_mfma_dma16_kernel<10, 4, 1> : fc_mfma_dma16_kernel<10, 0>;
        MNC_HIP_TRY(hipFuncSetAttribute(reinterpret_cast<const void*>(kern), hipFuncAttributeMaxDynamicSharedMemorySize, lds));
        hipLaunchKernelGGL(kern, dim3(tn * splits * tm), dim3(512), lds, ctx->stream, d_a, d_w, d_bias, d_out, part, M, N, K, ldc, kper,
                           act, splits == 1 ? 1 : 0, tn, splits, tm, p.drop, (const float*)nullptr, (const float*)nullptr,
                           (const float*)nullptr, (float*)nullptr, 0, 0L, 0L, 0L);
      } else if (tune(ctx, T_FC_MFMA16, 1) == 0 || waves == 4 || dabl) {
        launched = true;
        if (dabl == 1) MNC_FC_DMA_LAUNCH(1, 1);
        else if (dabl == 3) MNC_FC_DMA_LAUNCH(3, 1);
        else if (waves == 4) MNC_FC_DMA_LAUNCH(0, 1);
        else if (tm == 1 && M > 288 && M <= 304 && tune(ctx, T_FC_HALF, 1) != 0) MNC_FC_DMA_LAUNCH_H(0, 2, 1);
        else MNC_FC_DMA_LAUNCH(0, 2);
      }
#endif
      if (!launched) {
        if (p.buf) MNC_HIP_TRY((lds_limit_once<fc_mfma_dma16_kernel<10, 0, 1>>(ctx->device, lds)));
        else MNC_HIP_TRY((lds_limit_once<fc_mfma_dma16_kernel<10, 0, 0>>(ctx->device, lds)));
        hipLaunchKernelGGL((p.buf ? fc_mfma_dma16_kernel<10, 0, 1> : fc_mfma_dma16_kernel<10, 0, 0>), dim3(tn * splits * tm), dim3(512), lds,
                           ctx->stream, d_a, d_w, d_bias, d_out, part, M, N, K, ldc, kper, act, splits == 1 ? 1 : 0, tn, splits,
                           tm, p.drop, (const float*)nullptr, (const float*)nullptr, (const float*)nullptr, (float*)nullptr, 0, 0L, 0L,
                           0L);
      }
    }
    else if (mt == 2) MNC_FC_LAUNCH(2, 32, 0);
    else if (mt == 5) {
#ifdef MNC_TUNING
      const int abl = tune(ctx, T_FC_ABL, 0);
      if (abl == 1) MNC_FC_LAUNCH(5, 16, 1);
      else if (abl == 3) MNC_FC_LAUNCH(5, 16, 3);
      else
#endif
      MNC_FC_LAUNCH(5, 16, 0);
    } else {
#ifdef MNC_TUNING
      const int abl = tune(ctx, T_FC_ABL, 0);
      if (abl == 1) MNC_FC_LAUNCH(10, 32, 1);
      else if (abl == 2) MNC_FC_LAUNCH(10, 32, 2);
      else if (abl == 3) MNC_FC_LAUNCH(10, 32, 3);
      else if (abl == 4) MNC_FC_LAUNCH(10, 32, 4);
      else
#endif
      MNC_FC_LAUNCH(10, 32, 0);
    }
#undef MNC_FC_LAUNCH
#undef MNC_FC_DMA_LAUNCH
#undef MNC_FC_DMA_LAUNCH_H
    int rc = ls.finish("fc_mfma_kernel");
    if (rc) return rc;
  }
  if (ctx->defer_reduce && !slab) {
    ctx->deferred_part = splits > 1 ? part : nullptr;
    ctx->deferred_splits = splits > 1 ? splits : 1;
    return MNC_OK;
  }
  ctx->deferred_part = nullptr;
  ctx->deferred_splits = 1;
  if (splits > 1 && slab) {
    LaunchScope ls(ctx, "fc_reduce", 0.0, 4.0 * ((double)splits + 1.0) * M * N);
    long g = ((long)tn * tm * 10240 + 255) / 256;
    if (g > 8192) g = 8192;
    hipLaunchKernelGGL(fc_reduce_slab_kernel, dim3((int)g), dim3(256), 0, ctx->stream, part, d_bias, (const float*)nullptr, d_out,
                       (float*)nullptr, M, N, ldc, splits, act, tn, 0, tn * tm);
    return ls.finish("fc_reduce_slab_kernel");
  }
  if (splits > 1) {
    LaunchScope ls(ctx, "fc_reduce", 0.0, 4.0 * ((double)splits + 1.0) * M * N);
    fc_reduce_launch(ctx->stream, part, d_bias, d_out, M, N, ldc, splits, act);
    return ls.finish("fc_reduce_kernel");
  }
  return MNC_OK;
}

int mnc_fc_pair(mnc_ctx* ctx, const float* d_a0, const float* d_w0, const float* d_bias0, float* d_out0, const float* d_a1,
                const float* d_w1, const float* d_bias1, float* d_out1, int M, int N, int K, int ldc, int act) {
  MNC_REQUIRE(ctx && d_a0 && d_w0 && d_bias0 && d_out0 && d_a1 && d_w1 && d_bias1 && d_out1, "mnc_fc_pair: null pointer");
  MNC_REQUIRE(M >= 0 && N > 0 && K > 0 && K % kBK == 0 && ldc >= N && act >= 0 && act <= 2,
              "mnc_fc_pair: unsupported shape M=%d N=%d K=%d ldc=%d act=%d (need K%%32==0)", M, N, K, ldc, act);
  if (M == 0) return MNC_OK;
  FcCall call(M, N, K, ldc);
  call.defer_reduce = ctx->defer_reduce;
  call.aligned16 = ((reinterpret_cast<uintptr_t>(d_out0) | reinterpret_cast<uintptr_t>(d_out1) | reinterpret_cast<uintptr_t>(d_bias0) |
                     reinterpret_cast<uintptr_t>(d_bias1)) & 15) == 0;
  const FcPlan p = fc_pair_plan(call, ctx->tune, kTuningBuild);
  if (p.two_singles) {
    int rc = mnc_fc(ctx, d_a0, d_w0, d_bias0, d_out0, M, N, K, ldc, act);
    if (rc) return rc;
    return mnc_fc(ctx, d_a1, d_w1, d_bias1, d_out1, M, N, K, ldc, act);
  }
  const int tn = p.tn / 2, tm = p.tm, splits = p.splits, kper = p.kper;
  float* part = nullptr;
  if (splits > 1) {
    int rc = ensure_scratch(ctx, p.part_bytes);
    if (rc) return rc;
    part = (float*)ctx->scratch.p;
  }
  constexpr int lds = 65536 + (320 + kBN) * 32 * 4;
  {
    const double flops = 4.0 * M * (double)N * K, bytes = 8.0 * ((double)N * K + (double)M * K + (double)M * N);
    LaunchScope ls(ctx, "fc_mfma", flops, bytes);
    MNC_HIP_TRY((lds_limit_once<fc_mfma_dma16_kernel<10, 0, 1>>(ctx->device, lds)));
    hipLaunchKernelGGL((fc_mfma_dma16_kernel<10, 0, 1>), dim3(2 * tn * splits * tm), dim3(512), lds, ctx->stream, d_a0, d_w0, d_bias0,
                       d_out0, part, M, N, K, ldc, kper, act, splits == 1 ? 1 : 0, 2 * tn, splits, tm, p.drop, d_a1, d_w1,
                       d_bias1, d_out1, tn, 0L, 0L, 0L);
    int rc = ls.finish("fc_mfma_dma16_kernel");
    if (rc) return rc;
  }
  if (splits > 1) {
    LaunchScope ls(ctx, "fc_reduce", 0.0, 8.0 * ((double)splits + 1.0) * M * N);
    long g = ((long)2 * tn * tm * 10240 + 255) / 256;
    if (g > 8192) g = 8192;
    hipLaunchKernelGGL(fc_reduce_slab_kernel, dim3((int)g), dim3(256), 0, ctx->stream, part, d_bias0, d_bias1, d_out0, d_out1, M, N,
                       ldc, splits, act, 2 * tn, tn, 2 * tn * tm);
    return ls.finish("fc_reduce_slab_kernel");
  }
  return MNC_OK;
}

int mnc_fc_batch(mnc_ctx* ctx, const float* d_a, long stride_a, const float* d_w, long stride_w, float* d_out, long stride_out,
                 int B, int M, int N, int K, int ldc) {
  MNC_REQUIRE(ctx, "mnc_fc_batch: null context");
  LaunchScope ls(ctx, "fc_batch", 2.0 * B * M * (double)N * K, 4.0 * B * ((double)N * K + (double)M * K + (double)M * N));
  const int rc = fc_batch_launch(ctx, d_a, stride_a, d_w, stride_w, d_out, stride_out, B, M, N, K, ldc);
  const int rf = ls.finish("fc_mfma_dma16_kernel");
  return rc ? rc : rf;
}

int mnc_softmax_rows_ld(mnc_ctx* ctx, const float* d_in, int ld_in, float* d_out, int M, int N) {
  MNC_REQUIRE(ctx && d_in && d_out && M >= 0 && N > 0 && ld_in >= N, "mnc_softmax_rows: bad argument");
  if (M == 0) return MNC_OK;
  LaunchScope ls(ctx, "softmax_rows");
  if (N <= 64)
    hipLaunchKernelGGL(softmax_rows_wave_kernel, dim3(cdiv(M, 4)), dim3(256), 0, ctx->stream, d_in, ld_in, d_out, M, N);
  else
    hipLaunchKernelGGL(softmax_rows_kernel, dim3(cdiv(M, 64)), dim3(64), 0, ctx->stream, d_in, ld_in, d_out, M, N);
  return ls.finish("softmax_rows_kernel");
}

int mnc_softmax_rows(mnc_ctx* ctx, const float* d_in, float* d_out, int M, int N) {
  return mnc_softmax_rows_ld(ctx, d_in, N, d_out, M, N);
}

int mnc_eltwise(mnc_ctx* ctx, const float* d_in, float* d_out, size_t count, int op) {
  MNC_REQUIRE(ctx && (count == 0 || (d_in && d_out)) && (op == 1 || op == 2), "mnc_eltwise: bad argument");
  if (count == 0) return MNC_OK;
  LaunchScope ls(ctx, "eltwise");
  size_t g = (count + 255) / 256;
  if (g > 8192) g = 8192;
  hipLaunchKernelGGL(eltwise_kernel, dim3((int)g), dim3(256), 0, ctx->stream, d_in, d_out, count, op);
  return ls.finish("eltwise_kernel");
}

int mnc_copy2d(mnc_ctx* ctx, float* d_dst, int dst_ld, const float* d_src, int src_ld, int rows, int cols) {
  MNC_REQUIRE(ctx && rows >= 0 && cols >= 0 && dst_ld >= cols && src_ld >= cols, "mnc_copy2d: bad argument");
  if (rows == 0 || cols == 0) return MNC_OK;
  MNC_REQUIRE(d_dst && d_src, "mnc_copy2d: null pointer");
  MNC_HIP_TRY(hipMemcpy2DAsync(d_dst, (size_t)dst_ld * 4, d_src, (size_t)src_ld * 4, (size_t)cols * 4, rows,
                               hipMemcpyDeviceToDevice, ctx->stream));
  return MNC_OK;
}

int mnc_pack_fc_weights(mnc_ctx* ctx, const float* d_in, float* d_out, int N, int C, int PH, int PW) {
  MNC_REQUIRE(ctx && d_in && d_out && N > 0 && C > 0 && PH > 0 && PW > 0, "mnc_pack_fc_weights: bad argument");
  LaunchScope ls(ctx, "pack_fc");
  long total = (long)N * C * PH * PW;
  long g = (total + 255) / 256;
  if (g > 65536) g = 65536;
  hipLaunchKernelGGL(pack_fc_kernel, dim3((int)g), dim3(256), 0, ctx->stream, d_in, d_out, (long)N, C, PH * PW);
  return ls.finish("pack_fc_kernel");
}

}
```

### mnc_amd/csrc/mnc_internal.h

```cpp
#pragma once
#include <hip/hip_runtime.h>

#include <atomic>
#include <cstdarg>
#include <cstdio>
#include <cstring>
#include <mutex>
#include <string>
#include <vector>

#include "../../include/mnc_hip.h"
#include "tune.h"
#include "ws_layout.h"

namespace mnc {

struct DevArena {
  void* p = nullptr;
  size_t cap = 0;
};

void set_error(const char* fmt, ...);
void clear_error();

struct ProfRecord {
  const char* name;
  hipEvent_t start, stop;
  double flops, bytes;
};

}

namespace mnc {
constexpr int kTickets = 4096;
}

struct mnc_ctx {
  int device = 0;
  hipStream_t stream = nullptr;
  int profiling = 0;
  std::vector<mnc::ProfRecord> prof;
  std::vector<hipEvent_t> event_pool;
  mnc::DevArena scratch;
  void* proposal = nullptr;
  mnc::DevArena vote_ws;
  mnc::DevArena render_ws;
  mnc::DevArena mask_ws;
  mnc::DevArena rle_ws;
  mnc::DevArena overlap_ws;
  mnc::DevArena match_ws;
  void* comm = nullptr;
  unsigned* tickets = nullptr;
  bool defer_reduce = false;
  const float* deferred_part = nullptr;
  int deferred_splits = 0;
  unsigned long arena_gen = 0;
  mnc_layer_conventions conv = {0, 0, 0, 0, 0, 0, 0.4f, 0};
  bool capturing = false;
  unsigned long capture_gen = 0;
  int tune[mnc::T_COUNT];
};

struct mnc_graph {
  hipGraphExec_t exec = nullptr;
  mnc_ctx* ctx = nullptr;
  unsigned long arena_gen = 0;
};

namespace mnc {
inline bool tune_set(const mnc_ctx* ctx, TuneKey k) { return tune_set(ctx->tune, k); }
inline int tune(const mnc_ctx* ctx, TuneKey k, int dflt) { return tune(ctx->tune, k, dflt); }
inline bool plan_latency(const mnc_ctx* ctx) { return plan_latency(ctx->tune); }
#ifdef MNC_TUNING
constexpr bool kTuningBuild = true;
#else
constexpr bool kTuningBuild = false;
#endif
}

namespace mnc {

int arena_ensure(DevArena* a, size_t bytes, size_t slack, const char* who, hipStream_t stream, mnc_ctx* ctx = nullptr,
                 bool graph_visible = false);
void arena_free(DevArena* a);
int ensure_scratch(mnc_ctx* ctx, size_t bytes);
void prof_begin(mnc_ctx* ctx, const char* name, double flops, double bytes);
void prof_end(mnc_ctx* ctx);

#define MNC_HIP_TRY(expr)                                                                    \
  do {                                                                                       \
    hipError_t e__ = (expr);                                                                 \
    if (e__ != hipSuccess) {                                                                 \
      mnc::set_error("%s failed: %s (%s:%d)", #expr, hipGetErrorString(e__), __FILE__, __LINE__); \
      return MNC_ERR_HIP;                                                                    \
    }                                                                                        \
  } while (0)

#define MNC_NO_CAPTURE(ctx, what)                                                                        \
  do {                                                                                                   \
    if ((ctx)->capturing) {                                                                              \
      mnc::set_error("%s: synchronises or re-allocates; not allowed while a launch sequence is captured", what); \
      return MNC_ERR_STATE;                                                                              \
    }                                                                                                    \
  } while (0)

#define MNC_REQUIRE(cond, ...)       \
  do {                               \
    if (!(cond)) {                   \
      mnc::set_error(__VA_ARGS__);   \
      return MNC_ERR_INVALID;        \
    }                                \
  } while (0)

template <auto kKernel>
inline hipError_t lds_limit_once(int device, int bytes) {
  static std::atomic<unsigned long long> done{0};
  const unsigned long long bit = 1ull << (device & 63);
  if (done.load(std::memory_order_relaxed) & bit) return hipSuccess;
  const hipError_t e = hipFuncSetAttribute(reinterpret_cast<const void*>(kKernel), hipFuncAttributeMaxDynamicSharedMemorySize, bytes);
  if (e == hipSuccess) done.fetch_or(bit, std::memory_order_relaxed);
  return e;
}

struct LaunchScope {
  mnc_ctx* ctx;
  bool on;
  LaunchScope(mnc_ctx* c, const char* name, double flops = 0.0, double bytes = 0.0) : ctx(c) {
    (void)hipSetDevice(ctx->device);
    on = ctx->profiling == 1 || (ctx->profiling == 2 && flops >= 1.0e9);
    if (on) prof_begin(ctx, name, flops, bytes);
  }
  int finish(const char* name) {
    if (on) prof_end(ctx);
    hipError_t e = hipGetLastError();
    if (e != hipSuccess) {
      set_error("kernel launch %s failed: %s", name, hipGetErrorString(e));
      return MNC_ERR_HIP;
    }
    return MNC_OK;
  }
};

__device__ __forceinline__ void xcd_decode(int bid, int tn, int splits, int tm, int& bn, int& split, int& bm) {
  const int total = tn * splits * tm;
  const int q = total >> 3, r = total & 7;
  const int xcd = bid & 7, idx = bid >> 3;
  const int logical = (xcd < r ? xcd * (q + 1) : r * (q + 1) + (xcd - r) * q) + idx;
  bn = logical % tn;
  const int rest = logical / tn;
  split = rest % splits;
  bm = rest / splits;
}

typedef unsigned mnc_u32x4 __attribute__((ext_vector_type(4)));
typedef float mnc_f32x4 __attribute__((ext_vector_type(4)));
__device__ __forceinline__ __amdgpu_buffer_rsrc_t slab_rsrc(float* base) {
  return __builtin_amdgcn_make_buffer_rsrc(base, 0, 0x7FFFFFF0, 0x00020000);
}
__device__ __forceinline__ void slab_store(__amdgpu_buffer_rsrc_t rs, int voff, int soff, mnc_f32x4 v) {
  __builtin_amdgcn_raw_buffer_store_b128(__builtin_bit_cast(mnc_u32x4, v), rs, voff, soff,  16);
}
__device__ __forceinline__ mnc_f32x4 slab_load(__amdgpu_buffer_rsrc_t rs, int voff, int soff) {
  return __builtin_bit_cast(mnc_f32x4, __builtin_amdgcn_raw_buffer_load_b128(rs, voff, soff,  16));
}
__device__ __forceinline__ bool slab_last_arriver(unsigned* ticket, int arrivals, volatile unsigned* flag) {
  asm volatile("s_waitcnt vmcnt(0)" ::: "memory");
  __syncthreads();
  if (threadIdx.x == 0) *flag = __hip_atomic_fetch_add(ticket, 1u, __ATOMIC_RELAXED, __HIP_MEMORY_SCOPE_AGENT);
  __syncthreads();
  const bool last = __builtin_amdgcn_readfirstlane(*flag) == (unsigned)(arrivals - 1);
  if (last) {
    if (threadIdx.x == 0) {
      __hip_atomic_store(ticket, 0u, __ATOMIC_RELAXED, __HIP_MEMORY_SCOPE_AGENT);
      __builtin_amdgcn_fence(__ATOMIC_ACQUIRE, "agent");
    }
    __syncthreads();
  }
  return last;
}

struct CallBuf {
  void* p = nullptr;
  ~CallBuf() { if (p) (void)hipFree(p); }
  int alloc(const char* who, size_t bytes);
};

struct HostScope {
  std::unique_lock<std::mutex> lock;
  hipStream_t stream = nullptr;
  void* buf = nullptr;
  int open(int device_id, size_t bytes);
  hipError_t up(void* d_dst, const void* src, size_t bytes) const {
    return bytes ? hipMemcpyAsync(d_dst, src, bytes, hipMemcpyHostToDevice, stream) : hipSuccess;
  }
  hipError_t down(void* dst, const void* d_src, size_t bytes) const {
    return bytes ? hipMemcpyAsync(dst, d_src, bytes, hipMemcpyDeviceToHost, stream) : hipSuccess;
  }
  hipError_t sync() const { return hipStreamSynchronize(stream); }
};

struct CallTimer {
  std::atomic<int> on{0};
  std::atomic<double> last_ms{-1.0};
  int set(int enable, double* out_last_ms);
};

struct TimedSpan {
  CallTimer& timer;
  hipEvent_t a = nullptr, b = nullptr;
  bool on = false;
  explicit TimedSpan(CallTimer& t) : timer(t) {}
  TimedSpan(const TimedSpan&) = delete;
  ~TimedSpan() {
    if (a) (void)hipEventDestroy(a);
    if (b) (void)hipEventDestroy(b);
  }
  void begin(hipStream_t s) {
    if (!timer.on.load(std::memory_order_relaxed)) return;
    on = hipEventCreate(&a) == hipSuccess && hipEventCreate(&b) == hipSuccess && hipEventRecord(a, s) == hipSuccess;
  }
  void end(hipStream_t s) { if (on) on = hipEventRecord(b, s) == hipSuccess; }
  double ms() {
    float t = 0.f;
    if (on) on = hipEventElapsedTime(&t, a, b) == hipSuccess;
    return on ? (double)t : 0.0;
  }
  void keep() {
    const double t = ms();
    if (on) timer.last_ms.store(t);
  }
  void keep_sum(TimedSpan& earlier) {
    const double t = earlier.ms() + ms();
    if (on && earlier.on) timer.last_ms.store(t);
  }
};

int nms_mask_launch(hipStream_t stream, const float* d_boxes, const int* d_order, int n, int dim, float thr,
                    unsigned long long* d_mask, int batch);
int nms_scan_launch(hipStream_t stream, const unsigned long long* d_mask, int n, int max_keep, int* d_keep, int* d_num,
                    int batch);
int nms_mask_launch_indirect(hipStream_t stream, const float* d_boxes, const int* d_order, const int* d_n, int n_cap,
                             int dim, float thr, unsigned long long* d_mask);
int nms_scan_launch_indirect(hipStream_t stream, const unsigned long long* d_mask, const int* d_n, int n_cap, int max_keep,
                             int* d_keep, int* d_num, const float* d_gather_boxes = nullptr, const int* d_gather_order = nullptr,
                             float* d_rois = nullptr, int rois_cap = 0);
void proposal_state_free(void* state);
void comm_free(mnc_ctx* ctx);
void fc_reduce_launch(hipStream_t stream, const float* part, const float* bias, float* out, int M, int N, int ldc, int splits,
                      int act);
bool fc_reduce_launch_sm(hipStream_t stream, const float* part, const float* bias, float* out, int M, int N, int ldc, int splits,
                         int act, void* sm, int sm_fmt, long sm_rows, long sm_row0);
int fc_batch_launch(mnc_ctx* ctx, const float* d_a, long stride_a, const float* d_w, long stride_w, float* d_out, long stride_o, int B,
                    int M, int N, int K, int ldc);
bool wino4_split_supported(int H, int W, int Cin, int Cout);
bool wino4_split_selected(const mnc_ctx* ctx, int H, int W, int Cin, int Cout);
bool fc_reduce_pair_launch_sm(hipStream_t stream, const float* part0, const float* part1, const float* bias0, const float* bias1,
                              float* out0, float* out1, int M, int N, int ldc, int splits, int act, void* sm0, void* sm1, int sm_fmt,
                              long sm_rows, bool* sm_done);
void conv_splitk_reduce_launch(hipStream_t stream, const float* d_part, const float* d_bias, float* d_out, int H, int W,
                               int Cout, int ksplit, int relu);
int heads_finish_launch(mnc_ctx* ctx, const float* part, int splits, const float* bias, float* heads, int ld, int M, int K,
                        float* scores, const float* rois, float im_h, float im_w, float* rois_ext, const float* rois1,
                        const float* rois2, float scale, int image_height, int image_width, float* boxes, const int* copy_src,
                        int* copy_dst);
int c8_to_hwc_launch(mnc_ctx* ctx, const float* d_feat, float* d_hwc, int C, int H, int W);
int roi_warp_from_hwc(mnc_ctx* ctx, const float* d_hwc, int C, int H, int W, const float* d_rois, int R, int PH, int PW, float scale,
                      int pool2, float* d_out, void* d_sm, int sm_fmt);
bool roi_warp_sm_only_ok(const mnc_ctx* ctx, int C, int pool2);
int detect_tail_launch(mnc_ctx* ctx, const float* d_rois1, int R1, const float* d_rois2, int R2, float scale, int image_height,
                       int image_width, float* d_boxes, const int* d_copy_src, int* d_copy_dst);
int mv_launch(hipStream_t stream, const float* d_boxes, int box_dim, const float* d_masks, int S, const int* d_inds,
              const int* d_begins, const int* d_ends, const float* d_wts, int H, int W, int R, int* d_bounds,
              float* d_out_mask, int* d_out_box);
int mv_image_launch(hipStream_t stream, const float* d_boxes, const float* d_masks, int S, const int* d_inds, const int* d_begins,
                    const int* d_ends, const float* d_wts, int H, int W, double thresh, int R, const int* d_rcount, int grid_rows,
                    int* d_bounds, float* d_records, const float* d_rscore, const int* d_rows, int record_cap);

}
```

### mnc_amd/csrc/pipeline.hip

```cpp
#include <atomic>
#include <cmath>
#include <map>
#include <string>

#include "mnc_internal.h"

namespace mnc {
int* proposal_count_ptr(mnc_ctx* ctx);
}

using namespace mnc;

namespace {

struct HostBlob {
  std::vector<float> v;
};

struct DevBuf {
  void* p = nullptr;
  size_t cap = 0;
};

const char* kTrunk[13] = {"conv1_1", "conv1_2", "conv2_1", "conv2_2", "conv3_1", "conv3_2", "conv3_3",
                          "conv4_1", "conv4_2", "conv4_3", "conv5_1", "conv5_2", "conv5_3"};
const int kTrunkStage[13] = {0, 0, 1, 1, 2, 2, 2, 3, 3, 3, 4, 4, 4};
const bool kPoolAfter[13] = {false, true, false, true, false, false, true, false, false, true, false, false, false};

inline int pool_out(int n) { return (n - 2 + 1) / 2 + 1; }

void linear_taps(int n_dst, int n_src, double scale, int* lo, float* frac) {
  const double inv = 1.0 / scale;
  for (int i = 0; i < n_dst; ++i) {
    const float src = (float)(((double)i + 0.5) * inv - 0.5);
    long l = (long)std::floor((double)src);
    float f = (float)((double)src - (double)l);
    if (l < 0) { l = 0; f = 0.0f; }
    if (l >= n_src - 1) { l = n_src - 1; f = 0.0f; }
    lo[i] = (int)l;
    frac[i] = f;
  }
}

}

struct mnc_net {
  mnc_ctx* ctx = nullptr;
  mnc_ctx* ctx_b = nullptr;
  hipEvent_t ev_fork[2] = {nullptr, nullptr}, ev_join[2] = {nullptr, nullptr};
  mnc_net_config cfg;
  std::map<std::string, HostBlob> params;
  bool finalized = false;
  mnc_net* owner = nullptr;
  std::atomic<int> sharers{0};
  float* w_c3 = nullptr;
  void* w_conv[14] = {nullptr};
  float* w_split[14] = {nullptr};
  bool packed_trunk = false;
  bool conv_fast[14] = {false};
  float* b_conv[14] = {nullptr};
  float *w_rpn = nullptr, *b_rpn = nullptr;
  struct Fc { void* w = nullptr; float* b = nullptr; int N = 0, K = 0, kind = 0; };
  Fc fc_maskest, fc_maskpred, fc6, fc7, fc6m, fc7m, fc_heads;
  int cap_ph = 0, cap_pw = 0, cap_src = 0;
  DevBuf img, taps, data, act[13], pooled[4], act12_pk, rpn_out, rpn_score, rpn_prob;
  float* rpn_bbox_p = nullptr;
  DevBuf rois, rois_ext, feat14, h_mask, m14, box7, mask7, f6, f6m, join, heads, boxes, masks, scores;
  DevBuf outblk;
  DevBuf wino_ws;
  DevBuf hwc5;
  float* records() const { return (float*)((char*)outblk.p + 512); }
  int* counts() const { return (int*)outblk.p; }
  int* prop_count() const { return (int*)((char*)outblk.p + 256); }
  DevBuf feat14_sm, box7_sm, mask7_sm, f6_sm, f6m_sm;
  unsigned char* pin_img = nullptr; size_t pin_img_cap = 0;
  float* pin_out = nullptr; size_t pin_out_cap = 0;
  int H = 0, W = 0, OH = 0, OW = 0, fh = 0, fw = 0;
  float im_scale = 1.0f;
  int tap_key_h = -1, tap_key_w = -1;
  int last_r1 = 0, last_r2 = 0;
  bool fc_sm = true, fuse_pools = true;
  bool fuse_small = true;
  bool tail_done = false;
  bool in_flight = false;
  hipGraphExec_t gexec = nullptr;
  int graph_h = -1, graph_w = -1, seen_h = -1, seen_w = -1;
  unsigned long graph_gen = 0;
  void* render_dev = nullptr; void* render_pin = nullptr; size_t render_cap = 0;
  int vote_mode = MNC_VOTE_MV;
  double vote_binarize = 0.4;
};

namespace {

int dev_ensure(mnc_net* n, DevBuf* b, size_t bytes) {
  if (bytes <= b->cap) return MNC_OK;
  if (b->p) {
    int rc = mnc_dev_free(n->ctx, b->p);
    if (rc) return rc;
    b->p = nullptr; b->cap = 0;
  }
  const size_t want = bytes + (bytes >> 3) + 256;
  int rc = mnc_dev_alloc(n->ctx, want, &b->p);
  if (rc) return rc;
  b->cap = want;
  if (n->gexec) { (void)hipGraphExecDestroy(n->gexec); n->gexec = nullptr; n->graph_h = n->graph_w = -1; }
  return MNC_OK;
}

const HostBlob* find(mnc_net* n, const std::string& layer, int index) {
  auto it = n->params.find(layer + "/" + std::to_string(index));
  return it == n->params.end() ? nullptr : &it->second;
}

int upload(mnc_net* n, const std::vector<float>& v, float** out) {
  void* p = nullptr;
  int rc = mnc_dev_alloc(n->ctx, v.size() * 4, &p);
  if (rc) return rc;
  rc = mnc_h2d(n->ctx, p, v.data(), v.size() * 4);
  if (rc) return rc;
  *out = (float*)p;
  return MNC_OK;
}

#define NET_TRY(expr)        \
  do {                       \
    int rc__ = (expr);       \
    if (rc__) return rc__;   \
  } while (0)

int need(mnc_net* n, const char* layer, int index, size_t count, const HostBlob** out) {
  const HostBlob* b = find(n, layer, index);
  if (!b) {
    set_error("mnc_net: parameter %s/%d has not been set", layer, index);
    return MNC_ERR_STATE;
  }
  if (b->v.size() != count) {
    set_error("mnc_net: parameter %s/%d holds %zu values, the configured graph needs %zu", layer, index, b->v.size(), count);
    return MNC_ERR_INVALID;
  }
  *out = b;
  return MNC_OK;
}

static inline int conv_math(const mnc_net_config& c) { return c.math == 3 ? 1 : c.math; }
static inline int lowp_mode(int cm) { return cm == 1 ? 0 : cm == 2 ? 1 : 2; }
static inline int fc_math(const mnc_net_config& c) { return c.math == 3 ? 2 : c.math; }

int prepare_fc(mnc_net* n, const char* layer, int N, int K, int C, int PH, int PW, mnc_net::Fc* fc) {
  const HostBlob *w, *b;
  NET_TRY(need(n, layer, 0, (size_t)N * K, &w));
  NET_TRY(need(n, layer, 1, (size_t)N, &b));
  fc->N = N; fc->K = K;
  NET_TRY(upload(n, b->v, &fc->b));
  float* raw = nullptr;
  NET_TRY(upload(n, w->v, &raw));
  if (PH * PW > 1) {
    void* perm = nullptr;
    NET_TRY(mnc_dev_alloc(n->ctx, (size_t)N * K * 4, &perm));
    NET_TRY(mnc_pack_fc_weights(n->ctx, raw, (float*)perm, N, C, PH, PW));
    NET_TRY(mnc_dev_free(n->ctx, raw));
    raw = (float*)perm;
  }
  const bool big = 2.0 * n->cfg.post_nms_topn * (double)N * (double)K >= 2.0e9;
  const int fm = (n->cfg.math == 3 && K > 50000) ? 1 : fc_math(n->cfg);
  const bool bf = fm == 4 && K % 64 == 0 && big;
  const bool f16 = (fm == 2 && K % 64 == 0 && big) || bf;
  const bool x3 = !f16 && (fm == 1 || fm == 2) && K % 32 == 0 && big;
  fc->kind = bf ? 3 : f16 ? 2 : x3 ? 1 : 0;
  if (fc->kind == 0) { fc->w = raw; return MNC_OK; }
  void* packed = nullptr;
  NET_TRY(mnc_dev_alloc(n->ctx, (size_t)((N + 127) / 128) * 128 * K * (f16 ? 2 : 4), &packed));
  NET_TRY(bf ? mnc_pack_fc_bf16(n->ctx, raw, packed, N, K)
             : f16 ? mnc_pack_fc_f16(n->ctx, raw, packed, N, K) : mnc_pack_fc_bf16x3(n->ctx, raw, packed, N, K));
  NET_TRY(mnc_dev_free(n->ctx, raw));
  fc->w = packed;
  return MNC_OK;
}

int run_fc(mnc_ctx* ctx, const mnc_net::Fc& fc, const float* a, float* out, int M, int ldc, int act) {
  if (M == 0) return MNC_OK;
  if (fc.kind == 3) return mnc_fc_bf16(ctx, a, fc.w, fc.b, out, M, fc.N, fc.K, ldc, act);
  if (fc.kind == 2) return mnc_fc_f16(ctx, a, fc.w, fc.b, out, M, fc.N, fc.K, ldc, act);
  if (fc.kind == 1) return mnc_fc_bf16x3(ctx, a, fc.w, fc.b, out, M, fc.N, fc.K, ldc, act);
  return mnc_fc(ctx, a, (const float*)fc.w, fc.b, out, M, fc.N, fc.K, ldc, act);
}
int run_fc(mnc_net* n, const mnc_net::Fc& fc, const float* a, float* out, int M, int ldc, int act) {
  return run_fc(n->ctx, fc, a, out, M, ldc, act);
}
int sm_format(const mnc_net* n, const mnc_net::Fc& fc, int C) {
  if (!n->fc_sm) return 0;
  if (fc.kind == 2) return C % 64 == 0 ? 1 : 0;
  if (fc.kind == 1) return C % 32 == 0 ? 2 : 0;
  if (fc.kind == 3) return C % 64 == 0 ? 3 : 0;
  return 0;
}
int run_fc_sm(mnc_ctx* ctx, const mnc_net::Fc& fc, const float* a, const void* a_sm, int fmt, float* out, int M, int ldc, int act,
              void* out_sm = nullptr, int out_fmt = 0) {
  if (M == 0) return MNC_OK;
  if (!out_sm) out_fmt = 0;
  if (fc.kind == 2) return mnc_fc_f16_ex(ctx, fmt == 1 ? nullptr : a, fmt == 1 ? a_sm : nullptr, M, fc.w, fc.b, out, M, fc.N, fc.K, ldc,
                                         act, out_fmt ? out_sm : nullptr, out_fmt);
  if (fc.kind == 1) return mnc_fc_bf16x3_ex(ctx, fmt == 2 ? nullptr : a, fmt == 2 ? a_sm : nullptr, M, fc.w, fc.b, out, M, fc.N, fc.K,
                                            ldc, act, out_fmt ? out_sm : nullptr, out_fmt);
  if (fc.kind == 3) return mnc_fc_bf16_ex(ctx, fmt == 3 ? nullptr : a, fmt == 3 ? a_sm : nullptr, M, fc.w, fc.b, out, M, fc.N, fc.K, ldc,
                                          act, out_fmt ? out_sm : nullptr, out_fmt);
  return run_fc(ctx, fc, a, out, M, ldc, act);
}

int finalize(mnc_net* n) {
  if (n->finalized) return MNC_OK;
  const mnc_net_config& c = n->cfg;
  const HostBlob *w, *b;
  int cin = 3;
  for (int i = 0; i < 14; ++i) {
    const char* name = i < 13 ? kTrunk[i] : "rpn_conv_3x3";
    const int cout = i < 13 ? c.trunk_channels[kTrunkStage[i]] : c.rpn_channels;
    NET_TRY(need(n, name, 0, (size_t)cout * cin * 9, &w));
    NET_TRY(need(n, name, 1, (size_t)cout, &b));
    NET_TRY(upload(n, b->v, &n->b_conv[i]));
    if (i == 0) {
      NET_TRY(upload(n, w->v, &n->w_c3));
    } else {
      float* raw = nullptr;
      NET_TRY(upload(n, w->v, &raw));
      n->conv_fast[i] = cout % 32 == 0;
      if (n->conv_fast[i]) {
        const int cm = conv_math(c);
        const int pitch = c.winograd == 4 ? 288 : c.winograd ? 136 : 76;
        const size_t wbytes = cm == 0 ? (size_t)(cin / 8) * cout * pitch * 4 : mnc_conv3x3_lowp_weight_bytes(lowp_mode(cm), cout, cin);
        NET_TRY(mnc_dev_alloc(n->ctx, wbytes, &n->w_conv[i]));
        NET_TRY(cm == 0 ? (c.winograd == 4 ? mnc_pack_conv3x3_wino4(n->ctx, raw, (float*)n->w_conv[i], cout, cin)
                               : c.winograd ? mnc_pack_conv3x3_wino(n->ctx, raw, (float*)n->w_conv[i], cout, cin)
                                            : mnc_pack_conv3x3_weights(n->ctx, raw, (float*)n->w_conv[i], cout, cin))
                : cm == 1 ? mnc_pack_conv3x3_bf16x3(n->ctx, raw, n->w_conv[i], cout, cin)
                : cm == 4 ? mnc_pack_conv3x3_bf16(n->ctx, raw, n->w_conv[i], cout, cin)
                              : mnc_pack_conv3x3_f16(n->ctx, raw, n->w_conv[i], cout, cin));
      } else if (conv_math(c) == 2) {
        NET_TRY(mnc_dev_alloc(n->ctx, (size_t)9 * ((cin + 31) / 32) * 32 * cout * 2, &n->w_conv[i]));
        NET_TRY(mnc_pack_conv_weights_f16(n->ctx, raw, n->w_conv[i], cout, cin, 3, 3));
      } else {
        NET_TRY(mnc_dev_alloc(n->ctx, (size_t)cout * cin * 9 * 4, &n->w_conv[i]));
        NET_TRY(mnc_pack_conv_weights(n->ctx, raw, (float*)n->w_conv[i], cout, cin, 3, 3));
      }
      const int ws = tune(n->ctx, T_WINO_SPLIT, kWinoSplitDefault);
      if (n->conv_fast[i] && conv_math(c) == 0 && c.winograd == 4 && wino4_split_supported(4, 4, cin, cout) &&
          (ws == 2 || (ws == 1 && wino4_split_plan_channels(cin, cout)))) {
        void* u = nullptr;
        NET_TRY(mnc_dev_alloc(n->ctx, (size_t)36 * cout * cin * 4, &u));
        n->w_split[i] = (float*)u;
        NET_TRY(mnc_pack_conv3x3_wino4_split(n->ctx, raw, n->w_split[i], cout, cin));
      }
      NET_TRY(mnc_dev_free(n->ctx, raw));
    }
    cin = cout;
  }
  n->packed_trunk = conv_math(c) != 0 && tune(n->ctx, T_PACKED_ACT, 1) != 0;
  for (int i = 1; i < 13; ++i) n->packed_trunk = n->packed_trunk && n->conv_fast[i];
  const int A = c.num_anchors, RC = c.rpn_channels;
  {
    const HostBlob *wc, *bc, *wb, *bb;
    NET_TRY(need(n, "rpn_cls_score", 0, (size_t)2 * A * RC, &wc));
    NET_TRY(need(n, "rpn_cls_score", 1, (size_t)2 * A, &bc));
    NET_TRY(need(n, "rpn_bbox_pred", 0, (size_t)4 * A * RC, &wb));
    NET_TRY(need(n, "rpn_bbox_pred", 1, (size_t)4 * A, &bb));
    std::vector<float> wcat(wc->v), bcat(bc->v);
    wcat.insert(wcat.end(), wb->v.begin(), wb->v.end());
    bcat.insert(bcat.end(), bb->v.begin(), bb->v.end());
    NET_TRY(upload(n, wcat, &n->w_rpn));
    NET_TRY(upload(n, bcat, &n->b_rpn));
  }
  const int C5 = c.trunk_channels[4], P = c.roi_size, S = c.mask_size, F = c.fc_dim, K = c.num_classes;
  NET_TRY(prepare_fc(n, "fc6_maskest", c.mask_fc, C5 * P * P, C5, P, P, &n->fc_maskest));
  NET_TRY(prepare_fc(n, "mask_pred", S * S, c.mask_fc, c.mask_fc, 1, 1, &n->fc_maskpred));
  NET_TRY(prepare_fc(n, "fc6", F, C5 * (P / 2) * (P / 2), C5, P / 2, P / 2, &n->fc6));
  NET_TRY(prepare_fc(n, "fc7", F, F, F, 1, 1, &n->fc7));
  NET_TRY(prepare_fc(n, "fc6_mask", F, C5 * (P / 2) * (P / 2), C5, P / 2, P / 2, &n->fc6m));
  NET_TRY(prepare_fc(n, "fc7_mask", F, F, F, 1, 1, &n->fc7m));
  {
    const char* names[3] = {"cls_score", "seg_cls_score", "bbox_pred"};
    const int widths[3] = {K, K, 4 * K};
    std::vector<float> W, B;
    for (int i = 0; i < 3; ++i) {
      NET_TRY(need(n, names[i], 0, (size_t)widths[i] * 2 * F, &w));
      NET_TRY(need(n, names[i], 1, (size_t)widths[i], &b));
      W.insert(W.end(), w->v.begin(), w->v.end());
      B.insert(B.end(), b->v.begin(), b->v.end());
    }
    n->fc_heads.N = 6 * K; n->fc_heads.K = 2 * F; n->fc_heads.kind = 0;
    float* dw = nullptr;
    NET_TRY(upload(n, W, &dw));
    n->fc_heads.w = dw;
    NET_TRY(upload(n, B, &n->fc_heads.b));
  }
  NET_TRY(mnc_ctx_sync(n->ctx));
  n->params.clear();
  n->finalized = true;
  return MNC_OK;
}

int ensure_buffers(mnc_net* n, int H, int W, int OH, int OW) {
  const mnc_net_config& c = n->cfg;
  NET_TRY(dev_ensure(n, &n->img, (size_t)H * W * 3));
  NET_TRY(dev_ensure(n, &n->taps, (size_t)(2 * OW + 2 * OH) * 4));
  NET_TRY(dev_ensure(n, &n->data, (size_t)3 * OH * OW * 4));
  int h = OH, w = OW, pi = 0;
  size_t split_ws = 0;
  auto split_need = [&](int i, int hh, int ww, int cin, int cout) {
    if (n->w_split[i] && wino4_split_selected(n->ctx, hh, ww, cin, cout)) {
      const size_t b = mnc_conv3x3_wino4_split_ws_bytes(hh, ww, cin, cout);
      if (b > split_ws) split_ws = b;
    }
  };
  for (int i = 0; i < 13; ++i) {
    const int ch = c.trunk_channels[kTrunkStage[i]];
    if (i > 0) split_need(i, h, w, c.trunk_channels[kTrunkStage[i - 1]], ch);
    NET_TRY(dev_ensure(n, &n->act[i], (size_t)ch * h * w * 4));
    if (kPoolAfter[i]) {
      h = pool_out(h); w = pool_out(w);
      NET_TRY(dev_ensure(n, &n->pooled[pi++], (size_t)ch * h * w * 4));
    }
  }
  split_need(13, h, w, c.trunk_channels[4], c.rpn_channels);
  if (split_ws) NET_TRY(dev_ensure(n, &n->wino_ws, split_ws));
  const int A = c.num_anchors;
  if (n->packed_trunk) NET_TRY(dev_ensure(n, &n->act12_pk, (size_t)c.trunk_channels[4] * h * w * 4));
  NET_TRY(dev_ensure(n, &n->hwc5, (size_t)c.trunk_channels[4] * h * w * 4));
  NET_TRY(dev_ensure(n, &n->rpn_out, (size_t)c.rpn_channels * h * w * 4));
  NET_TRY(dev_ensure(n, &n->rpn_score, (size_t)6 * A * h * w * 4));
  NET_TRY(dev_ensure(n, &n->rpn_prob, (size_t)2 * A * h * w * 4));
  n->rpn_bbox_p = (float*)n->rpn_score.p + (size_t)2 * A * h * w;
  const int R = c.post_nms_topn, C5 = c.trunk_channels[4], P = c.roi_size, S = c.mask_size, F = c.fc_dim, K = c.num_classes;
  NET_TRY(dev_ensure(n, &n->rois, (size_t)R * 5 * 4));
  NET_TRY(dev_ensure(n, &n->rois_ext, (size_t)R * 5 * 4));
  NET_TRY(dev_ensure(n, &n->feat14, (size_t)R * P * P * C5 * 4));
  NET_TRY(dev_ensure(n, &n->h_mask, (size_t)R * c.mask_fc * 4));
  NET_TRY(dev_ensure(n, &n->m14, (size_t)R * P * P * 4));
  NET_TRY(dev_ensure(n, &n->box7, (size_t)R * (P / 2) * (P / 2) * C5 * 4));
  NET_TRY(dev_ensure(n, &n->mask7, (size_t)R * (P / 2) * (P / 2) * C5 * 4));
  if (sm_format(n, n->fc_maskest, C5)) NET_TRY(dev_ensure(n, &n->feat14_sm, (size_t)R * P * P * C5 * (n->fc_maskest.kind == 1 ? 4 : 2)));
  if (sm_format(n, n->fc6, C5)) NET_TRY(dev_ensure(n, &n->box7_sm, (size_t)R * (P / 2) * (P / 2) * C5 * (n->fc6.kind == 1 ? 4 : 2)));
  if (sm_format(n, n->fc6m, C5)) NET_TRY(dev_ensure(n, &n->mask7_sm, (size_t)R * (P / 2) * (P / 2) * C5 * (n->fc6m.kind == 1 ? 4 : 2)));
  NET_TRY(dev_ensure(n, &n->f6, (size_t)R * F * 4));
  NET_TRY(dev_ensure(n, &n->f6m, (size_t)R * F * 4));
  if (sm_format(n, n->fc7, F)) NET_TRY(dev_ensure(n, &n->f6_sm, (size_t)R * F * (n->fc7.kind == 1 ? 4 : 2)));
  if (sm_format(n, n->fc7m, F)) NET_TRY(dev_ensure(n, &n->f6m_sm, (size_t)R * F * (n->fc7m.kind == 1 ? 4 : 2)));
  NET_TRY(dev_ensure(n, &n->join, (size_t)R * 2 * F * 4));
  NET_TRY(dev_ensure(n, &n->heads, (size_t)2 * R * 6 * K * 4));
  NET_TRY(dev_ensure(n, &n->boxes, (size_t)2 * R * 4 * 4));
  NET_TRY(dev_ensure(n, &n->masks, (size_t)2 * R * S * S * 4));
  NET_TRY(dev_ensure(n, &n->scores, (size_t)2 * R * K * 4));
  const size_t rows = (size_t)(K - 1) * c.max_per_image;
  NET_TRY(dev_ensure(n, &n->outblk, 512 + rows * (6 + S * S) * 4));
  if ((size_t)H * W * 3 > n->pin_img_cap) {
    if (n->pin_img) NET_TRY(mnc_host_free(n->ctx, n->pin_img));
    n->pin_img = nullptr;
    NET_TRY(mnc_host_alloc(n->ctx, (size_t)H * W * 3 + 4096, (void**)&n->pin_img));
    n->pin_img_cap = (size_t)H * W * 3 + 4096;
    if (n->gexec) { (void)hipGraphExecDestroy(n->gexec); n->gexec = nullptr; n->graph_h = n->graph_w = -1; }
  }
  const size_t out_bytes = 512 + rows * (6 + S * S) * 4;
  if (out_bytes > n->pin_out_cap) {
    if (n->pin_out) NET_TRY(mnc_host_free(n->ctx, n->pin_out));
    n->pin_out = nullptr;
    NET_TRY(mnc_host_alloc(n->ctx, out_bytes, (void**)&n->pin_out));
    n->pin_out_cap = out_bytes;
    if (n->gexec) { (void)hipGraphExecDestroy(n->gexec); n->gexec = nullptr; n->graph_h = n->graph_w = -1; }
  }
  return MNC_OK;
}

int set_geometry(mnc_net* n, int H, int W) {
  const mnc_net_config& c = n->cfg;
  const int shortside = H < W ? H : W, longside = H < W ? W : H;
  double scale = (double)c.target_size / (double)shortside;
  if (std::nearbyint(scale * longside) > c.max_size) scale = (double)c.max_size / (double)longside;
  const int OH = (int)std::nearbyint(H * scale), OW = (int)std::nearbyint(W * scale);
  NET_TRY(ensure_buffers(n, H, W, OH, OW));
  n->H = H; n->W = W; n->OH = OH; n->OW = OW;
  n->im_scale = (float)scale;
  if (n->tap_key_h != H || n->tap_key_w != W) {
    std::vector<int> lo(OW > OH ? OW : OH);
    std::vector<float> fr(lo.size());
    std::vector<float> table((size_t)2 * OW + 2 * OH);
    linear_taps(OW, W, scale, lo.data(), fr.data());
    memcpy(table.data(), lo.data(), (size_t)OW * 4);
    memcpy(table.data() + OW, fr.data(), (size_t)OW * 4);
    linear_taps(OH, H, scale, lo.data(), fr.data());
    memcpy(table.data() + 2 * OW, lo.data(), (size_t)OH * 4);
    memcpy(table.data() + 2 * OW + OH, fr.data(), (size_t)OH * 4);
    NET_TRY(mnc_h2d(n->ctx, n->taps.p, table.data(), table.size() * 4));
    n->tap_key_h = H; n->tap_key_w = W;
  }
  return MNC_OK;
}

int conv3(mnc_net* n, int i, const float* in, float* out, int h, int w, int cin, int cout) {
  const mnc_net_config& c = n->cfg;
  const int cm = conv_math(c);
  if (!n->conv_fast[i]) {
    if (cm == 2) return mnc_conv2d_f16(n->ctx, in, n->w_conv[i], n->b_conv[i], nullptr, out, h, w, cin, cout, 3, 3, 1, 1, 1);
    return mnc_conv2d(n->ctx, in, (const float*)n->w_conv[i], n->b_conv[i], nullptr, out, h, w, cin, cout, 3, 3, 1, 1, 1);
  }
  if (cm == 0 && c.winograd == 4 && n->w_split[i] && wino4_split_selected(n->ctx, h, w, cin, cout))
    return mnc_conv3x3_wino4_split(n->ctx, in, n->w_split[i], n->b_conv[i], out, n->wino_ws.p, h, w, cin, cout, 1);
  if (cm == 0 && c.winograd == 4)
    return mnc_conv3x3_wino4(n->ctx, in, (const float*)n->w_conv[i], n->b_conv[i], out, h, w, cin, cout, 1);
  if (cm == 0 && c.winograd)
    return mnc_conv3x3_wino(n->ctx, in, (const float*)n->w_conv[i], n->b_conv[i], out, h, w, cin, cout, 1);
  if (cm == 0) return mnc_conv3x3(n->ctx, in, (const float*)n->w_conv[i], n->b_conv[i], out, h, w, cin, cout, 1);
  if (cm == 1) return mnc_conv3x3_bf16x3(n->ctx, in, n->w_conv[i], n->b_conv[i], out, h, w, cin, cout, 1);
  if (cm == 4) return mnc_conv3x3_bf16(n->ctx, in, n->w_conv[i], n->b_conv[i], out, h, w, cin, cout, 1);
  return mnc_conv3x3_f16(n->ctx, in, n->w_conv[i], n->b_conv[i], out, h, w, cin, cout, 1);
}

int run_trunk(mnc_net* n) {
  const mnc_net_config& c = n->cfg;
  mnc_ctx* ctx = n->ctx;
  const float* t = (const float*)n->taps.p;
  NET_TRY(mnc_prep_image(ctx, (const unsigned char*)n->img.p, n->H, n->W, c.pixel_means, (const int*)t, t + n->OW, n->OW,
                         (const int*)(t + 2 * n->OW), t + 2 * n->OW + n->OH, n->OH, (float*)n->data.p, n->OH, n->OW));
  int h = n->OH, w = n->OW, pi = 0, cin = 3;
  const float* cur = (const float*)n->data.p;
  if (n->packed_trunk) {
    const int mode = lowp_mode(conv_math(c));
    const void* pc = cur;
    for (int i = 0; i < 13; ++i) {
      const int cout = c.trunk_channels[kTrunkStage[i]];
      void* out = n->act[i].p;
      if (kPoolAfter[i] && i > 0 && n->fuse_small) {
        void* p = n->pooled[pi++].p;
        NET_TRY(mnc_conv3x3_lowp_pool(ctx, mode, pc, n->w_conv[i], n->b_conv[i], p, h, w, cin, cout, 1));
        h = pool_out(h); w = pool_out(w);
        pc = p; cin = cout;
        continue;
      }
      if (i == 0) NET_TRY(mnc_conv3x3_c3_fmt(ctx, cur, n->w_c3, n->b_conv[0], out, h, w, cout, 1, mode + 1));
      else if (i < 12) NET_TRY(mnc_conv3x3_lowp(ctx, mode, pc, n->w_conv[i], n->b_conv[i], out, nullptr, h, w, cin, cout, 1));
      else NET_TRY(mnc_conv3x3_lowp(ctx, mode, pc, n->w_conv[i], n->b_conv[i], n->act12_pk.p, (float*)out, h, w, cin, cout, 1));
      pc = out; cin = cout;
      if (kPoolAfter[i]) {
        void* p = n->pooled[pi++].p;
        NET_TRY(mode == 1 ? mnc_maxpool2_c8_f16(ctx, pc, p, cout, h, w)
                          : mode == 2 ? mnc_maxpool2_c8_bf16(ctx, pc, p, cout, h, w) : mnc_maxpool2_c8_bf16x3(ctx, pc, p, cout, h, w));
        h = pool_out(h); w = pool_out(w);
        pc = p;
      }
    }
    cur = (const float*)pc;
  } else
  for (int i = 0; i < 13; ++i) {
    const int cout = c.trunk_channels[kTrunkStage[i]];
    float* out = (float*)n->act[i].p;
    if (kPoolAfter[i] && i > 0 && conv_math(c) == 0 && c.winograd && n->conv_fast[i]) {
      float* p = (float*)n->pooled[pi++].p;
      if (c.winograd == 4 && n->w_split[i] && wino4_split_selected(ctx, h, w, cin, cout))
        NET_TRY(mnc_conv3x3_wino4_split_pool(ctx, cur, n->w_split[i], n->b_conv[i], p, n->wino_ws.p, h, w, cin, cout, 1));
      else
      NET_TRY(c.winograd == 4 ? mnc_conv3x3_wino4_pool(ctx, cur, (const float*)n->w_conv[i], n->b_conv[i], p, h, w, cin, cout, 1)
                              : mnc_conv3x3_wino_pool(ctx, cur, (const float*)n->w_conv[i], n->b_conv[i], p, h, w, cin, cout, 1));
      h = pool_out(h); w = pool_out(w);
      cur = p; cin = cout;
      continue;
    }
    if (i == 0) NET_TRY(mnc_conv3x3_c3(ctx, cur, n->w_c3, n->b_conv[0], out, h, w, cout, 1));
    else NET_TRY(conv3(n, i, cur, out, h, w, cin, cout));
    cur = out; cin = cout;
    if (kPoolAfter[i]) {
      float* p = (float*)n->pooled[pi++].p;
      NET_TRY(mnc_maxpool2_c8(ctx, cur, p, cout, h, w));
      h = pool_out(h); w = pool_out(w);
      cur = p;
    }
  }
  n->fh = h; n->fw = w;
  if (n->fuse_small)
    NET_TRY(c8_to_hwc_launch(ctx, (const float*)n->act[12].p, (float*)n->hwc5.p, c.trunk_channels[4], h, w));
  const int A = c.num_anchors;
  if (n->packed_trunk && n->conv_fast[13])
    NET_TRY(mnc_conv3x3_lowp(ctx, lowp_mode(conv_math(c)), n->act12_pk.p, n->w_conv[13], n->b_conv[13], nullptr, (float*)n->rpn_out.p, h, w,
                             cin, c.rpn_channels, 1));
  else NET_TRY(conv3(n, 13, cur, (float*)n->rpn_out.p, h, w, cin, c.rpn_channels));
  if (n->fuse_small) {
    NET_TRY(mnc_rpn_heads(ctx, (const float*)n->rpn_out.p, n->w_rpn, n->b_rpn, (float*)n->rpn_score.p, (float*)n->rpn_prob.p, h, w,
                          c.rpn_channels, A));
  } else {
    NET_TRY(mnc_conv1x1_to_nchw(ctx, (const float*)n->rpn_out.p, n->w_rpn, n->b_rpn, (float*)n->rpn_score.p, h, w, c.rpn_channels,
                                6 * A));
    NET_TRY(mnc_rpn_softmax(ctx, (const float*)n->rpn_score.p, (float*)n->rpn_prob.p, A, h, w));
  }
  NET_TRY(mnc_proposal(ctx, (const float*)n->rpn_prob.p, (const float*)n->rpn_bbox_p, A, h, w, c.anchors, c.feat_stride,
                       (float)n->OH, (float)n->OW, n->im_scale, c.pre_nms_topn, c.post_nms_topn, c.rpn_nms_thresh,
                       c.rpn_min_size, (float*)n->rois.p, nullptr));
  return MNC_OK;
}

int run_stage(mnc_net* n, const float* rois, int R, bool second, int row0) {
  const mnc_net_config& c = n->cfg;
  mnc_ctx* ctx = n->ctx;
  const int C5 = c.trunk_channels[4], P = c.roi_size, S = c.mask_size, F = c.fc_dim, K = c.num_classes;
  const float* conv5 = (const float*)n->act[12].p;
  float* feat14 = (float*)n->feat14.p;
  const int sm_feat = sm_format(n, n->fc_maskest, C5), sm_box = sm_format(n, n->fc6, C5), sm_mask = sm_format(n, n->fc6m, C5);
  const bool fork0 = n->ctx_b && ctx->profiling == 0 && R > 0;
  const bool lowp_pairs = n->fuse_small && n->fuse_pools && sm_box == sm_mask && !fork0 && n->fc6.kind != 0 && n->fc6m.kind == n->fc6.kind &&
                          n->fc7.kind == n->fc6.kind && n->fc7m.kind == n->fc6.kind && n->fc6.K == n->fc6m.K &&
                          sm_format(n, n->fc7, F) == sm_format(n, n->fc7m, F) && R > 0;
  const bool sm_only = lowp_pairs && sm_box != 0;
  const bool feat_sm_only = sm_only && sm_feat != 0 && (P * P * C5) % 64 == 0 && roi_warp_sm_only_ok(ctx, C5, second ? 0 : 1);
  if (feat_sm_only) feat14 = nullptr;
  if (n->fuse_small)
    NET_TRY(roi_warp_from_hwc(ctx, (const float*)n->hwc5.p, C5, n->fh, n->fw, rois, R, P, P, c.spatial_scale, second ? 0 : 1, feat14,
                              n->feat14_sm.p, sm_feat));
  else
    NET_TRY(mnc_roi_warp_sm(ctx, conv5, C5, n->fh, n->fw, rois, R, P, P, c.spatial_scale, second ? 0 : 1, feat14, n->feat14_sm.p,
                            sm_feat));
  float* masks = (float*)n->masks.p + (size_t)row0 * S * S;
  NET_TRY(run_fc_sm(ctx, n->fc_maskest, feat14, n->feat14_sm.p, sm_feat, (float*)n->h_mask.p, R, c.mask_fc, 1));
  NET_TRY(run_fc(n, n->fc_maskpred, (const float*)n->h_mask.p, masks, R, S * S, 2));
  NET_TRY(mnc_mask_resize(ctx, masks, (float*)n->m14.p, R, S, S, P, P));
  float* join = (float*)n->join.p;
  const bool one_pass = n->fuse_pools && sm_box == sm_mask;
  if (one_pass)
    NET_TRY(mnc_box_mask_pool_ex(ctx, feat14, sm_feat ? n->feat14_sm.p : nullptr, sm_feat, (const float*)n->m14.p,
                                 sm_only ? nullptr : (float*)n->box7.p, sm_only ? nullptr : (float*)n->mask7.p, R, P, P, C5, n->box7_sm.p,
                                 n->mask7_sm.p, sm_box));
  const bool fork = n->ctx_b && ctx->profiling == 0 && R > 0;
  mnc_ctx* cb = fork ? n->ctx_b : ctx;
  const int si = second ? 1 : 0;
  if (fork) {
    MNC_HIP_TRY(hipEventRecord(n->ev_fork[si], ctx->stream));
    MNC_HIP_TRY(hipStreamWaitEvent(cb->stream, n->ev_fork[si], 0));
  }
  if (!one_pass) NET_TRY(mnc_maxpool2_rhwc_sm(cb, feat14, (float*)n->box7.p, R, P, P, C5, n->box7_sm.p, sm_box));
  const int sm_f6 = sm_format(n, n->fc7, F), sm_f6m = sm_format(n, n->fc7m, F);
  if (n->fuse_small && one_pass && !fork && n->fc6.kind == 0 && n->fc6m.kind == 0 && n->fc7.kind == 0 && n->fc7m.kind == 0 &&
      n->fc6.K == n->fc6m.K) {
    NET_TRY(mnc_fc_pair(ctx, (const float*)n->box7.p, (const float*)n->fc6.w, n->fc6.b, (float*)n->f6.p, (const float*)n->mask7.p,
                        (const float*)n->fc6m.w, n->fc6m.b, (float*)n->f6m.p, R, F, n->fc6.K, F, 1));
    NET_TRY(mnc_fc_pair(ctx, (const float*)n->f6.p, (const float*)n->fc7.w, n->fc7.b, join + F, (const float*)n->f6m.p,
                        (const float*)n->fc7m.w, n->fc7m.b, join, R, F, F, 2 * F, 1));
  } else if (lowp_pairs) {
    const int mode = n->fc6.kind == 1 ? 0 : n->fc6.kind == 2 ? 1 : 2;
    const bool pre6 = sm_box != 0, pre7 = sm_f6 != 0;
    NET_TRY(mnc_fc_lowp_pair(ctx, mode, pre6 ? nullptr : (const float*)n->box7.p, pre6 ? n->box7_sm.p : nullptr,
                             pre6 ? nullptr : (const float*)n->mask7.p, pre6 ? n->mask7_sm.p : nullptr, R, n->fc6.w, n->fc6m.w, n->fc6.b,
                             n->fc6m.b, (float*)n->f6.p, (float*)n->f6m.p, R, F, n->fc6.K, F, 1, pre7 ? n->f6_sm.p : nullptr,
                             pre7 ? n->f6m_sm.p : nullptr, sm_f6));
    NET_TRY(mnc_fc_lowp_pair(ctx, mode, pre7 ? nullptr : (const float*)n->f6.p, pre7 ? n->f6_sm.p : nullptr,
                             pre7 ? nullptr : (const float*)n->f6m.p, pre7 ? n->f6m_sm.p : nullptr, R, n->fc7.w, n->fc7m.w, n->fc7.b,
                             n->fc7m.b, join + F, join, R, F, F, 2 * F, 1, nullptr, nullptr, 0));
  } else {
  NET_TRY(run_fc_sm(cb, n->fc6, (const float*)n->box7.p, n->box7_sm.p, sm_box, (float*)n->f6.p, R, F, 1, n->f6_sm.p, sm_f6));
  NET_TRY(run_fc_sm(cb, n->fc7, (const float*)n->f6.p, n->f6_sm.p, n->fc6.kind ? sm_f6 : 0, join + F, R, 2 * F, 1));
  if (fork) MNC_HIP_TRY(hipEventRecord(n->ev_join[si], cb->stream));
  if (!one_pass)
    NET_TRY(mnc_mask_pool_sm(ctx, feat14, (const float*)n->m14.p, (float*)n->mask7.p, R, P, P, C5, 1, n->mask7_sm.p, sm_mask));
  NET_TRY(run_fc_sm(ctx, n->fc6m, (const float*)n->mask7.p, n->mask7_sm.p, sm_mask, (float*)n->f6m.p, R, F, 1, n->f6m_sm.p, sm_f6m));
  NET_TRY(run_fc_sm(ctx, n->fc7m, (const float*)n->f6m.p, n->f6m_sm.p, n->fc6m.kind ? sm_f6m : 0, join, R, 2 * F, 1));
  if (fork) MNC_HIP_TRY(hipStreamWaitEvent(ctx->stream, n->ev_join[si], 0));
  }
  float* heads = (float*)n->heads.p + (size_t)row0 * 6 * K;
  float* scores = (float*)n->scores.p + (size_t)row0 * K;
  n->tail_done = false;
  if (n->fuse_small && R > 0 && K <= 64 && n->fc_heads.kind == 0 && 2.0 * R * 6.0 * K * n->fc_heads.K < 2.0e9) {
    ctx->defer_reduce = true;
    int rc = run_fc(n, n->fc_heads, join, heads, R, 6 * K, 0);
    ctx->defer_reduce = false;
    if (rc) return rc;
    NET_TRY(heads_finish_launch(ctx, ctx->deferred_part, ctx->deferred_splits, n->fc_heads.b, heads, 6 * K, R, K, scores, rois,
                                (float)n->OH, (float)n->OW, second ? nullptr : (float*)n->rois_ext.p, (const float*)n->rois.p,
                                (const float*)n->rois_ext.p, n->im_scale, n->H, n->W, second ? (float*)n->boxes.p : nullptr,
                                second ? proposal_count_ptr(ctx) : nullptr, second ? n->prop_count() : nullptr));
    n->tail_done = second;
    return MNC_OK;
  }
  NET_TRY(run_fc(n, n->fc_heads, join, heads, R, 6 * K, 0));
  if (R) NET_TRY(mnc_softmax_rows_ld(ctx, heads + K, 6 * K, scores, R, K));
  if (!second)
    NET_TRY(mnc_stage_bridge(ctx, rois, heads + 2 * K, 6 * K, scores, K, R, K, (float)n->OH, (float)n->OW,
                             (float*)n->rois_ext.p));
  return MNC_OK;
}

int run_heads_and_vote(mnc_net* n, int r1) {
  const mnc_net_config& c = n->cfg;
  mnc_ctx* ctx = n->ctx;
  const int S = c.mask_size, K = c.num_classes;
  NET_TRY(run_stage(n, (const float*)n->rois.p, r1, false, 0));
  NET_TRY(run_stage(n, (const float*)n->rois_ext.p, r1, true, r1));
  if (!n->tail_done)
    NET_TRY(detect_tail_launch(ctx, (const float*)n->rois.p, r1, (const float*)n->rois_ext.p, r1, n->im_scale, n->H, n->W,
                               (float*)n->boxes.p, proposal_count_ptr(ctx), n->prop_count()));
  const int rows = (K - 1) * c.max_per_image;
  NET_TRY(mnc_vote_instances_ex(ctx, n->vote_mode, (const float*)n->boxes.p, (const float*)n->masks.p, (const float*)n->scores.p,
                                2 * r1, K, S, c.max_per_image, c.vote_nms_thresh, c.vote_iou_thresh, n->vote_binarize, n->H, n->W,
                                n->records(), rows, n->counts()));
  n->last_r1 = r1; n->last_r2 = r1;
  return MNC_OK;
}

int enqueue_outputs(mnc_net* n) {
  const mnc_net_config& c = n->cfg;
  const size_t rec_bytes = (size_t)c.max_per_image * (6 + c.mask_size * c.mask_size) * 4;
  NET_TRY(mnc_d2h_async(n->ctx, n->pin_out, n->outblk.p, 512 + rec_bytes));
  return MNC_OK;
}

int enqueue_image(mnc_net* n) {
  NET_TRY(mnc_h2d_async(n->ctx, n->img.p, n->pin_img, (size_t)n->H * n->W * 3));
  NET_TRY(run_trunk(n));
  NET_TRY(run_heads_and_vote(n, n->cfg.post_nms_topn));
  return enqueue_outputs(n);
}

unsigned long arena_gen(const mnc_net* n) { return n->ctx->arena_gen + (n->ctx_b ? n->ctx_b->arena_gen : 0); }

int launch_image(mnc_net* n, const unsigned char* bgr_host, int H, int W) {
  MNC_REQUIRE(n && bgr_host && H >= 16 && W >= 16, "mnc_forward_image: bad argument");
  NET_TRY(finalize(n));
  MNC_HIP_TRY(hipSetDevice(n->ctx->device));
  if (n->in_flight) MNC_HIP_TRY(hipStreamSynchronize(n->ctx->stream));
  NET_TRY(set_geometry(n, H, W));
  memcpy(n->pin_img, bgr_host, (size_t)H * W * 3);
  n->in_flight = true;
  hipStream_t s = n->ctx->stream;
  const bool want_graph = n->cfg.use_graph && n->ctx->profiling == 0;
  if (n->gexec && n->graph_gen != arena_gen(n)) {
    (void)hipGraphExecDestroy(n->gexec);
    n->gexec = nullptr; n->graph_h = n->graph_w = -1; n->seen_h = n->seen_w = -1;
  }
  if (want_graph && n->gexec && n->graph_h == H && n->graph_w == W) {
    MNC_HIP_TRY(hipGraphLaunch(n->gexec, s));
    return MNC_OK;
  }
  if (want_graph && n->seen_h == H && n->seen_w == W) {
    if (n->gexec) { (void)hipGraphExecDestroy(n->gexec); n->gexec = nullptr; }
    hipGraph_t g = nullptr;
    MNC_HIP_TRY(hipStreamBeginCapture(s, hipStreamCaptureModeRelaxed));
    const unsigned long gen0 = arena_gen(n);
    n->ctx->capturing = true;
    if (n->ctx_b) n->ctx_b->capturing = true;
    int rc = enqueue_image(n);
    n->ctx->capturing = false;
    if (n->ctx_b) n->ctx_b->capturing = false;
    hipError_t e = hipStreamEndCapture(s, &g);
    if (rc == MNC_OK && e == hipSuccess && g && gen0 == arena_gen(n)) {
      e = hipGraphInstantiate(&n->gexec, g, nullptr, nullptr, 0);
      (void)hipGraphDestroy(g);
      if (e == hipSuccess) {
        n->graph_h = H; n->graph_w = W;
        n->graph_gen = gen0;
        MNC_HIP_TRY(hipGraphLaunch(n->gexec, s));
        return MNC_OK;
      }
      n->gexec = nullptr;
      (void)hipGetLastError();
      n->cfg.use_graph = 0;
    } else {
      if (g) (void)hipGraphDestroy(g);
      (void)hipGetLastError();
      if (e != hipSuccess) n->cfg.use_graph = 0;
    }
  }
  n->seen_h = H; n->seen_w = W;
  return enqueue_image(n);
}

}

extern "C" {

int mnc_net_default_config(mnc_net_config* cfg) {
  MNC_REQUIRE(cfg, "mnc_net_default_config: null pointer");
  memset(cfg, 0, sizeof(*cfg));
  const int tc[5] = {64, 128, 256, 512, 512};
  memcpy(cfg->trunk_channels, tc, sizeof(tc));
  cfg->rpn_channels = 512;
  cfg->num_anchors = 9;
  const float a[36] = {-84, -40, 99, 55,  -176, -88, 191, 103,  -360, -184, 375, 199,  -56, -56, 71, 71,  -120, -120, 135, 135,
                       -248, -248, 263, 263,  -36, -80, 51, 95,  -80, -168, 95, 183,  -168, -344, 183, 359};
  memcpy(cfg->anchors, a, sizeof(a));
  cfg->feat_stride = 16;
  cfg->pre_nms_topn = 6000; cfg->post_nms_topn = 300;
  cfg->rpn_nms_thresh = 0.7f; cfg->rpn_min_size = 16.0f;
  cfg->mask_fc = 256; cfg->mask_size = 21;
  cfg->fc_dim = 4096;
  cfg->num_classes = 21;
  cfg->roi_size = 14;
  cfg->spatial_scale = 0.0625f;
  cfg->target_size = 600; cfg->max_size = 1000;
  cfg->pixel_means[0] = 102.9801; cfg->pixel_means[1] = 115.9465; cfg->pixel_means[2] = 122.7717;
  cfg->max_per_image = 100;
  cfg->vote_nms_thresh = 0.3f; cfg->vote_iou_thresh = 0.5f;
  cfg->math = 0;
  cfg->use_graph = 1;
  cfg->winograd = 4;
  cfg->conventions.maskpool_thresh = 0.4f;
  cfg->conventions.inherit = 1;
  clear_error();
  return MNC_OK;
}

int mnc_net_create(mnc_ctx* ctx, const mnc_net_config* cfg, mnc_net** out) {
  MNC_REQUIRE(ctx && cfg && out, "mnc_net_create: null pointer");
  *out = nullptr;
  for (int i = 0; i < 5; ++i)
    MNC_REQUIRE(cfg->trunk_channels[i] > 0 && cfg->trunk_channels[i] % 8 == 0 && cfg->trunk_channels[i] <= 4096,
                "mnc_net_create: trunk width %d must be a positive multiple of 8", cfg->trunk_channels[i]);
  MNC_REQUIRE(cfg->trunk_channels[0] <= 512, "mnc_net_create: conv1 width %d > 512", cfg->trunk_channels[0]);
  MNC_REQUIRE(cfg->rpn_channels > 0 && cfg->rpn_channels % 8 == 0 && cfg->num_anchors > 0 && cfg->num_anchors <= 16,
              "mnc_net_create: RPN shape");
  MNC_REQUIRE(cfg->roi_size > 0 && cfg->roi_size % 2 == 0 && cfg->mask_size >= 2 && cfg->num_classes >= 2 &&
              cfg->post_nms_topn > 0 && cfg->max_per_image > 0 && cfg->fc_dim > 0 && cfg->mask_fc > 0,
              "mnc_net_create: head shape");
  MNC_REQUIRE(cfg->num_classes <= 64, "mnc_net_create: num_classes %d > 64 (the result header holds 64 counts)", cfg->num_classes);
  MNC_REQUIRE(cfg->math >= 0 && cfg->math <= 4, "mnc_net_create: math must be 0 (fp32), 1 (bf16x3), 2 (f16), 3 (mixed) or 4 (bf16)");
  MNC_REQUIRE(cfg->target_size > 0 && cfg->max_size >= cfg->target_size, "mnc_net_create: target_size / max_size");
  if (!cfg->conventions.inherit) {
    int rc = mnc_ctx_set_layer_conventions(ctx, &cfg->conventions);
    if (rc) return rc;
  }
  MNC_REQUIRE(cfg->math != 0 || cfg->winograd != 4 ||
                  (double)cfg->trunk_channels[0] * cfg->max_size * (double)cfg->max_size * 4.0 < 2147483648.0,
              "mnc_net_create: winograd = 4 with max_size %d: a %d-channel %dx%d map exceeds the F(4x4) kernel's 2 GB operand range; "
              "use winograd = 2", cfg->max_size, cfg->trunk_channels[0], cfg->max_size, cfg->max_size);
  mnc_net* n = new (std::nothrow) mnc_net();
  if (!n) { set_error("mnc_net_create: out of host memory"); return MNC_ERR_NOMEM; }
  n->ctx = ctx;
  n->cfg = *cfg;
  n->cfg.conventions = ctx->conv;
  n->fc_sm = tune(ctx, T_FC_SM, 1) != 0;
  n->fuse_pools = tune(ctx, T_FUSE_POOLS, 1) != 0;
  n->fuse_small = tune(ctx, T_FUSE_SMALL, 1) != 0;
  if (tune(ctx, T_BRANCH_STREAMS, 0) == 1) {
    if (mnc_ctx_create(&n->ctx_b, ctx->device) != MNC_OK) n->ctx_b = nullptr;
    if (n->ctx_b) (void)mnc_ctx_set_layer_conventions(n->ctx_b, &ctx->conv);
    for (int i = 0; i < 2 && n->ctx_b; ++i) {
      if (hipEventCreateWithFlags(&n->ev_fork[i], hipEventDisableTiming) != hipSuccess ||
          hipEventCreateWithFlags(&n->ev_join[i], hipEventDisableTiming) != hipSuccess) {
        (void)mnc_ctx_destroy(n->ctx_b);
        n->ctx_b = nullptr;
      }
    }
  }
  *out = n;
  clear_error();
  return MNC_OK;
}

int mnc_net_create_shared(mnc_ctx* ctx, mnc_net* parent, mnc_net** out) {
  MNC_REQUIRE(ctx && parent && out, "mnc_net_create_shared: null pointer");
  *out = nullptr;
  MNC_REQUIRE(!parent->owner, "mnc_net_create_shared: `parent` borrows its weights itself; share with the net that owns them");
  MNC_REQUIRE(ctx->device == parent->ctx->device, "mnc_net_create_shared: context on device %d, the weights live on device %d",
              ctx->device, parent->ctx->device);
  MNC_REQUIRE(ctx != parent->ctx, "mnc_net_create_shared: give the sharing net its own context (stream and scratch arenas)");
  NET_TRY(finalize(parent));
  mnc_net* n = nullptr;
  {
// ... 318 lines not shown
```

### mnc_amd/csrc/tune.h

```cpp
#pragma once
#include <climits>

namespace mnc {
#define MNC_TUNE_KEYS(X)                                                                                                          \
  X(CONV_COT) X(CONV_ROWS) X(CONV_KSPLIT) X(CONV_ABL) X(CONV1X1_TILE) X(CONV2D_WIDE) X(WINO_ROWS) X(WINO_TAIL) X(WINO_V) X(WINO_VAR)  \
  X(WINO_DMA) X(WINO_XCD) X(CONVX3_TILE) X(FC_NOTAIL) X(FC_TILE) X(FC_ABL) X(FC_DMA) X(PLAN) X(FC_RANGE_K) X(FC_SLOTS) X(FC_EVEN) X(FC_SPLIT_DIV) X(WINO_FILL) X(CONVX3_P0MIN) X(CONVX3_P1MIN) X(FC_DMA_ABL) X(FC_DMA_WAVES)    \
  X(FC_NO256) X(FCX3_TILE) X(FC_ORDER) X(FCX3_ABL) X(FC_SM) X(PACKED_ACT) X(FUSE_POOLS) X(BRANCH_STREAMS) X(TOPK_SINGLE_WG)           \
  X(ROI_SM_VARIANT) X(ROI_WARP_VARIANT) X(FC_REDUCE) X(WINO_F4) X(FUSE_SMALL) X(FCX3_WIDE) X(FC_HALF) X(WINO_STREAM) X(FC_MFMA16) X(WINO_MFMA16) X(ROI_ROW_SEGS) X(WINO_SPLIT)
enum TuneKey {
#define MNC_TUNE_ENUM(n) T_##n,
  MNC_TUNE_KEYS(MNC_TUNE_ENUM)
#undef MNC_TUNE_ENUM
  T_COUNT
};
constexpr int kTuneUnset = INT_MIN;

inline bool tune_set(const int* t, TuneKey k) { return t[k] != kTuneUnset; }
inline int tune(const int* t, TuneKey k, int dflt) { return t[k] != kTuneUnset ? t[k] : dflt; }
inline bool plan_latency(const int* t) { return tune(t, T_PLAN, 0) == 1; }

constexpr int kWinoSplitDefault = 1;
inline bool wino4_split_plan_channels(int Cin, int Cout) { return Cin >= 512 && Cout >= 512; }

static inline int cdiv(long a, long b) { return (int)((a + b - 1) / b); }
}
```

Before: 270.6 images/s.

## Fuse Winograd split output transform with next layer's input transform in LDS

Adds a boundary kernel that runs one conv layer's Winograd output transform (bias, ReLU, optional pool), writes the output and keeps the map in LDS. It then computes the next layer's Winograd input transform from LDS, so the next layer skips reading its activation back from global memory. The V and M workspaces are split into separate regions so the next layer's V can be written while M is read. It also adds a smaller 160-row batched GEMM variant for small M. The boundary kernel runs one workgroup per 8 channels, which may give low parallelism on large maps.

```diff
diff --git a/include/mnc_hip.h b/include/mnc_hip.h
--- a/include/mnc_hip.h
+++ b/include/mnc_hip.h
@@ -244,6 +244,15 @@
                                     void* d_ws, int H, int W, int Cin, int Cout, int relu);
 MNC_API int mnc_conv3x3_wino4_split_pool(mnc_ctx* ctx, const float* d_in_c8, const float* d_w_split, const float* d_bias,
                                          float* d_out_pooled_c8, void* d_ws, int H, int W, int Cin, int Cout, int relu);
+MNC_API int mnc_conv3x3_wino4_split_steps(mnc_ctx* ctx, const float* d_in_c8, const float* d_w_split, const float* d_bias,
+                                          float* d_out_c8, float* d_v, float* d_m, float* d_v_next, int H, int W, int Cin, int Cout,
+                                          int relu, int pool);
+MNC_API int mnc_wino4_split_boundary_supported(int H, int W, int C);
+MNC_API int mnc_wino4_split_input(mnc_ctx* ctx, const float* d_in_c8, float* d_v, int H, int W, int C);
+MNC_API int mnc_wino4_split_output(mnc_ctx* ctx, const float* d_m, const float* d_bias, float* d_out_c8, int H, int W, int C, int relu,
+                                   int pool);
+MNC_API int mnc_wino4_split_boundary(mnc_ctx* ctx, const float* d_m, const float* d_bias, float* d_out_c8, float* d_v_next, int H, int W,
+                                     int C, int relu, int pool);
 MNC_API int mnc_maxpool2_c8(mnc_ctx* ctx, const float* d_in, float* d_out, int C, int H, int W);
 MNC_API int mnc_conv1x1_to_nchw(mnc_ctx* ctx, const float* d_in_c8, const float* d_w, const float* d_bias,
                                 float* d_out_nchw, int H, int W, int Cin, int Cout);
diff --git a/mnc_amd/csrc/conv_wino4_split.hip b/mnc_amd/csrc/conv_wino4_split.hip
--- a/mnc_amd/csrc/conv_wino4_split.hip
+++ b/mnc_amd/csrc/conv_wino4_split.hip
@@ -26,6 +26,37 @@
   y[3] = fma4(8.f, d34, d12) + m[5];
 }
 
+template <class Load>
+__device__ __forceinline__ void wino4_split_input_item(Load load, float* __restrict__ V, int H, int W, int Cin, int tiles_x, int ntiles,
+                                                       int tile, int c4) {
+  const int ty = tile / tiles_x, tx = tile - ty * tiles_x;
+  const int y0 = 4 * ty - 1, x0 = 4 * tx - 1;
+  s4f t[6][6];
+#pragma unroll
+  for (int j = 0; j < 6; ++j) {
+    s4f d[6], x[6];
+    const int xx = x0 + j;
+#pragma unroll
+    for (int i = 0; i < 6; ++i) {
+      const int yy = y0 + i;
+      d[i] = s4f{0.f, 0.f, 0.f, 0.f};
+      if (yy >= 0 && yy < H && xx >= 0 && xx < W) d[i] = load(yy, xx);
+    }
+    bt6(d, x);
+#pragma unroll
+    for (int i = 0; i < 6; ++i) t[i][j] = x[i];
+  }
+  float* dst = V + (long)tile * Cin + c4 * 4;
+  const long pstride = (long)ntiles * Cin;
+#pragma unroll
+  for (int i = 0; i < 6; ++i) {
+    s4f x[6];
+    bt6(t[i], x);
+#pragma unroll
+    for (int j = 0; j < 6; ++j) *reinterpret_cast<s4f*>(dst + (long)(6 * i + j) * pstride) = x[j];
+  }
+}
+
 __global__ __launch_bounds__(256) void wino4_split_input_kernel(const float* __restrict__ in, float* __restrict__ V, int H, int W, int Cin,
                                                                 int tiles_x, int ntiles) {
   const int c4n = Cin >> 2;
@@ -33,32 +64,63 @@
   const long idx = (long)blockIdx.x * blockDim.x + threadIdx.x;
   if (idx >= total) return;
   const int c4 = (int)(idx % c4n), tile = (int)(idx / c4n);
+  const float* src = in + (long)(c4 >> 1) * H * W * 8 + (c4 & 1) * 4;
+  wino4_split_input_item([&](int yy, int xx) { return *reinterpret_cast<const s4f*>(src + ((long)yy * W + xx) * 8); }, V, H, W, Cin,
+                         tiles_x, ntiles, tile, c4);
+}
+
+template <int POOL, class Store>
+__device__ __forceinline__ void wino4_split_output_item(const float* __restrict__ Mt, const float* __restrict__ bias, int H, int W,
+                                                        int Cout, int relu, int tiles_x, int ntiles, int tile, int c4, Store store) {
   const int ty = tile / tiles_x, tx = tile - ty * tiles_x;
-  const int y0 = 4 * ty - 1, x0 = 4 * tx - 1;
-  const float* src = in + (long)(c4 >> 1) * H * W * 8 + (c4 & 1) * 4;
-  s4f t[6][6];
+  const int oy = 4 * ty, ox = 4 * tx;
+  const float* src = Mt + (long)tile * Cout + c4 * 4;
+  const long pstride = (long)ntiles * Cout;
+  s4f z[4][6];
 #pragma unroll
   for (int j = 0; j < 6; ++j) {
-    s4f d[6], x[6];
-    const int xx = x0 + j;
-#pragma unroll
-    for (int i = 0; i < 6; ++i) {
-      const int yy = y0 + i;
-      d[i] = s4f{0.f, 0.f, 0.f, 0.f};
-      if (yy >= 0 && yy < H && xx >= 0 && xx < W) d[i] = *reinterpret_cast<const s4f*>(src + ((long)yy * W + xx) * 8);
+    s4f m[6], y[4];
+#pragma unroll
+    for (int i = 0; i < 6; ++i) m[i] = *reinterpret_cast<const s4f*>(src + (long)(6 * i + j) * pstride);
+    at6(m, y);
+#pragma unroll
+    for (int i = 0; i < 4; ++i) z[i][j] = y[i];
+  }
+  const s4f bv = *reinterpret_cast<const s4f*>(bias + c4 * 4);
+  s4f y[4][4];
+#pragma unroll
+  for (int i = 0; i < 4; ++i) {
+    at6(z[i], y[i]);
+#pragma unroll
+    for (int j = 0; j < 4; ++j) {
+      y[i][j] += bv;
+      if (relu) y[i][j] = s4f{fmaxf(y[i][j].x, 0.f), fmaxf(y[i][j].y, 0.f), fmaxf(y[i][j].z, 0.f), fmaxf(y[i][j].w, 0.f)};
     }
-    bt6(d, x);
-#pragma unroll
-    for (int i = 0; i < 6; ++i) t[i][j] = x[i];
-  }
-  float* dst = V + (long)tile * Cin + c4 * 4;
-  const long pstride = (long)ntiles * Cin;
-#pragma unroll
-  for (int i = 0; i < 6; ++i) {
-    s4f x[6];
-    bt6(t[i], x);
-#pragma unroll
-    for (int j = 0; j < 6; ++j) *reinterpret_cast<s4f*>(dst + (long)(6 * i + j) * pstride) = x[j];
+  }
+  if (!POOL) {
+#pragma unroll
+    for (int i = 0; i < 4; ++i)
+#pragma unroll
+      for (int j = 0; j < 4; ++j)
+        if (oy + i < H && ox + j < W) store(oy + i, ox + j, y[i][j]);
+  } else {
+#pragma unroll
+    for (int pi = 0; pi < 2; ++pi)
+#pragma unroll
+      for (int pj = 0; pj < 2; ++pj) {
+        const int py = oy + 2 * pi, px = ox + 2 * pj;
+        if (py >= H || px >= W) continue;
+        s4f best = y[2 * pi][2 * pj];
+#pragma unroll
+        for (int di = 0; di < 2; ++di)
+#pragma unroll
+          for (int dj = 0; dj < 2; ++dj)
+            if (py + di < H && px + dj < W) {
+              const s4f o = y[2 * pi + di][2 * pj + dj];
+              best = s4f{fmaxf(best.x, o.x), fmaxf(best.y, o.y), fmaxf(best.z, o.z), fmaxf(best.w, o.w)};
+            }
+        store(py >> 1, px >> 1, best);
+      }
   }
 }
 
@@ -71,57 +133,33 @@
   const long idx = (long)blockIdx.x * blockDim.x + threadIdx.x;
   if (idx >= total) return;
   const int c4 = (int)(idx % c4n), tile = (int)(idx / c4n);
-  const int ty = tile / tiles_x, tx = tile - ty * tiles_x;
-  const int oy = 4 * ty, ox = 4 * tx;
-  const float* src = Mt + (long)tile * Cout + c4 * 4;
-  const long pstride = (long)ntiles * Cout;
-  s4f z[4][6];
-#pragma unroll
-  for (int j = 0; j < 6; ++j) {
-    s4f m[6], y[4];
-#pragma unroll
-    for (int i = 0; i < 6; ++i) m[i] = *reinterpret_cast<const s4f*>(src + (long)(6 * i + j) * pstride);
-    at6(m, y);
-#pragma unroll
-    for (int i = 0; i < 4; ++i) z[i][j] = y[i];
-  }
-  const s4f bv = *reinterpret_cast<const s4f*>(bias + c4 * 4);
-  s4f y[4][4];
-#pragma unroll
-  for (int i = 0; i < 4; ++i) {
-    at6(z[i], y[i]);
-#pragma unroll
-    for (int j = 0; j < 4; ++j) {
-      y[i][j] += bv;
-      if (relu) y[i][j] = s4f{fmaxf(y[i][j].x, 0.f), fmaxf(y[i][j].y, 0.f), fmaxf(y[i][j].z, 0.f), fmaxf(y[i][j].w, 0.f)};
-    }
-  }
   const int cb = c4 >> 1, half = (c4 & 1) * 4;
-  if (!POOL) {
-#pragma unroll
-    for (int i = 0; i < 4; ++i)
-#pragma unroll
-      for (int j = 0; j < 4; ++j)
-        if (oy + i < H && ox + j < W) *reinterpret_cast<s4f*>(out + (((long)cb * H + oy + i) * W + ox + j) * 8 + half) = y[i][j];
-  } else {
-    const int OH = (H + 1) >> 1, OW = (W + 1) >> 1;
-#pragma unroll
-    for (int pi = 0; pi < 2; ++pi)
-#pragma unroll
-      for (int pj = 0; pj < 2; ++pj) {
-        const int py = oy + 2 * pi, px = ox + 2 * pj;
-        if (py >= H || px >= W) continue;
-        s4f best = y[2 * pi][2 * pj];
-#pragma unroll
-        for (int di = 0; di < 2; ++di)
-#pragma unroll
-          for (int dj = 0; dj < 2; ++dj)
-            if (py + di < H && px + dj < W) {
-              const s4f o = y[2 * pi + di][2 * pj + dj];
-              best = s4f{fmaxf(best.x, o.x), fmaxf(best.y, o.y), fmaxf(best.z, o.z), fmaxf(best.w, o.w)};
-            }
-        *reinterpret_cast<s4f*>(out + (((long)cb * OH + (py >> 1)) * OW + (px >> 1)) * 8 + half) = best;
-      }
+  const int OH = POOL ? (H + 1) >> 1 : H, OW = POOL ? (W + 1) >> 1 : W;
+  wino4_split_output_item<POOL>(Mt, bias, H, W, Cout, relu, tiles_x, ntiles, tile, c4, [&](int y, int x, s4f v) {
+    *reinterpret_cast<s4f*>(out + (((long)cb * OH + y) * OW + x) * 8 + half) = v;
+  });
+}
+
+constexpr int kBoundaryLdsBytes = 80 * 1024;
+template <int POOL>
+__global__ __launch_bounds__(512) void wino4_split_boundary_kernel(const float* __restrict__ Mt, const float* __restrict__ bias,
+                                                                   float* __restrict__ out, float* __restrict__ Vn, int H, int W, int C,
+                                                                   int relu, int tiles_x, int ntiles, int OH, int OW, int otiles_x,
+                                                                   int ontiles) {
+  extern __shared__ __attribute__((aligned(16))) float s_map[];
+  const int cb = blockIdx.x;
+  for (int idx = threadIdx.x; idx < 2 * ntiles; idx += blockDim.x) {
+    const int tile = idx >> 1, half = (idx & 1) * 4;
+    wino4_split_output_item<POOL>(Mt, bias, H, W, C, relu, tiles_x, ntiles, tile, cb * 2 + (idx & 1), [&](int y, int x, s4f v) {
+      *reinterpret_cast<s4f*>(out + (((long)cb * OH + y) * OW + x) * 8 + half) = v;
+      *reinterpret_cast<s4f*>(s_map + (y * OW + x) * 8 + half) = v;
+    });
+  }
+  __syncthreads();
+  for (int idx = threadIdx.x; idx < 2 * ontiles; idx += blockDim.x) {
+    const int tile = idx >> 1, half = (idx & 1) * 4;
+    wino4_split_input_item([&](int yy, int xx) { return *reinterpret_cast<const s4f*>(s_map + (yy * OW + xx) * 8 + half); }, Vn, OH, OW,
+                           C, otiles_x, ontiles, tile, cb * 2 + (idx & 1));
   }
 }
 
@@ -152,41 +190,85 @@
   if (v == 0 || !wino4_split_supported(H, W, Cin, Cout)) return false;
   if (v == 2) return true;
   if (plan_latency(ctx)) return false;
-  return wino4_split_plan_channels(Cin, Cout) && cdiv(H, 4) * cdiv(W, 4) >= 304;
+  return wino4_split_plan_channels(Cin, Cout) && wino4_split_plan_tiles(v, cdiv(H, 4) * cdiv(W, 4));
 }
 
 static size_t wino4_split_v_bytes(int H, int W, int Cin) {
   return ((size_t)36 * cdiv(W, 4) * cdiv(H, 4) * Cin * 4 + 255) & ~(size_t)255;
 }
 
-static int wino4_split_impl(mnc_ctx* ctx, const float* d_in, const float* d_u, const float* d_bias, float* d_out, void* d_ws, int H,
-                            int W, int Cin, int Cout, int relu, int pool) {
-  MNC_REQUIRE(ctx && d_in && d_u && d_bias && d_out && d_ws, "mnc_conv3x3_wino4_split: null pointer");
-  MNC_REQUIRE((reinterpret_cast<uintptr_t>(d_ws) & 15) == 0, "mnc_conv3x3_wino4_split: workspace not 16-byte aligned");
+static void input_launch(mnc_ctx* ctx, const float* d_in, float* V, int H, int W, int C) {
+  const int tiles_x = cdiv(W, 4), ntiles = tiles_x * cdiv(H, 4);
+  const long items = (long)ntiles * (C >> 2);
+  hipLaunchKernelGGL(wino4_split_input_kernel, dim3((unsigned)((items + 255) / 256)), dim3(256), 0, ctx->stream, d_in, V, H, W, C, tiles_x,
+                     ntiles);
+}
+
+static void output_launch(mnc_ctx* ctx, const float* Mt, const float* d_bias, float* d_out, int H, int W, int C, int relu, int pool) {
+  const int tiles_x = cdiv(W, 4), ntiles = tiles_x * cdiv(H, 4);
+  const long items = (long)ntiles * (C >> 2);
+  if (pool)
+    hipLaunchKernelGGL(wino4_split_output_kernel<1>, dim3((unsigned)((items + 255) / 256)), dim3(256), 0, ctx->stream, Mt, d_bias, d_out, H,
+                       W, C, relu, tiles_x, ntiles);
+  else
+    hipLaunchKernelGGL(wino4_split_output_kernel<0>, dim3((unsigned)((items + 255) / 256)), dim3(256), 0, ctx->stream, Mt, d_bias, d_out, H,
+                       W, C, relu, tiles_x, ntiles);
+}
+
+bool wino4_split_boundary_supported(int H, int W, int C) {
+  return H > 0 && W > 0 && C > 0 && C % 8 == 0 && (long)H * W * 32 <= kBoundaryLdsBytes;
+}
+
+static int boundary_launch(mnc_ctx* ctx, const float* Mt, const float* d_bias, float* d_out, float* Vn, int H, int W, int C, int relu,
+                           int pool) {
+  const int OH = pool ? (H + 1) / 2 : H, OW = pool ? (W + 1) / 2 : W;
+  if (!wino4_split_boundary_supported(OH, OW, C)) {
+    output_launch(ctx, Mt, d_bias, d_out, H, W, C, relu, pool);
+    input_launch(ctx, d_out, Vn, OH, OW, C);
+    return MNC_OK;
+  }
+  const int tiles_x = cdiv(W, 4), ntiles = tiles_x * cdiv(H, 4), otiles_x = cdiv(OW, 4), ontiles = otiles_x * cdiv(OH, 4);
+  const int lds = OH * OW * 32;
+  if (pool) {
+    MNC_HIP_TRY((lds_limit_once<wino4_split_boundary_kernel<1>>(ctx->device, kBoundaryLdsBytes)));
+    hipLaunchKernelGGL(wino4_split_boundary_kernel<1>, dim3(C / 8), dim3(512), lds, ctx->stream, Mt, d_bias, d_out, Vn, H, W, C, relu,
+                       tiles_x, ntiles, OH, OW, otiles_x, ontiles);
+  } else {
+    MNC_HIP_TRY((lds_limit_once<wino4_split_boundary_kernel<0>>(ctx->device, kBoundaryLdsBytes)));
+    hipLaunchKernelGGL(wino4_split_boundary_kernel<0>, dim3(C / 8), dim3(512), lds, ctx->stream, Mt, d_bias, d_out, Vn, H, W, C, relu,
+                       tiles_x, ntiles, OH, OW, otiles_x, ontiles);
+  }
+  return MNC_OK;
+}
+
+static int wino4_split_steps(mnc_ctx* ctx, const float* d_in, const float* d_u, const float* d_bias, float* d_out, float* V, float* Mt,
+                             float* Vn, int H, int W, int Cin, int Cout, int relu, int pool) {
+  MNC_REQUIRE(ctx && d_u && d_bias && d_out && V && Mt, "mnc_conv3x3_wino4_split: null pointer");
+  MNC_REQUIRE(((reinterpret_cast<uintptr_t>(V) | reinterpret_cast<uintptr_t>(Mt) | reinterpret_cast<uintptr_t>(Vn)) & 15) == 0,
+              "mnc_conv3x3_wino4_split: workspace not 16-byte aligned");
   MNC_REQUIRE(wino4_split_supported(H, W, Cin, Cout),
               "mnc_conv3x3_wino4_split: unsupported shape H=%d W=%d Cin=%d Cout=%d (need Cin%%32==0, Cout%%32==0)", H, W, Cin, Cout);
-  const int tiles_x = cdiv(W, 4), ntiles = tiles_x * cdiv(H, 4);
-  float* V = (float*)d_ws;
-  float* Mt = (float*)((char*)d_ws + wino4_split_v_bytes(H, W, Cin));
+  const int ntiles = cdiv(W, 4) * cdiv(H, 4);
   const double flops = 2.0 * H * W * 9.0 * Cin * Cout;
   const double out_px = pool ? (double)((H + 1) / 2) * ((W + 1) / 2) : (double)H * W;
   const double bytes = 4.0 * ((double)H * W * Cin + out_px * Cout + 9.0 * Cin * Cout);
   LaunchScope ls(ctx, "conv3x3_wino4_mfma", flops, bytes);
-  const long in_items = (long)ntiles * (Cin >> 2), out_items = (long)ntiles * (Cout >> 2);
-  hipLaunchKernelGGL(wino4_split_input_kernel, dim3((unsigned)((in_items + 255) / 256)), dim3(256), 0, ctx->stream, d_in, V, H, W, Cin,
-                     tiles_x, ntiles);
+  if (d_in) input_launch(ctx, d_in, V, H, W, Cin);
   int rc = fc_batch_launch(ctx, V, (long)ntiles * Cin, d_u, (long)Cout * Cin, Mt, (long)ntiles * Cout, 36, ntiles, Cout, Cin, Cout);
+  if (!rc && Vn) rc = boundary_launch(ctx, Mt, d_bias, d_out, Vn, H, W, Cout, relu, pool);
   if (rc) {
     (void)ls.finish("conv3x3_wino4_split");
     return rc;
   }
-  if (pool)
-    hipLaunchKernelGGL(wino4_split_output_kernel<1>, dim3((unsigned)((out_items + 255) / 256)), dim3(256), 0, ctx->stream, Mt, d_bias,
-                       d_out, H, W, Cout, relu, tiles_x, ntiles);
-  else
-    hipLaunchKernelGGL(wino4_split_output_kernel<0>, dim3((unsigned)((out_items + 255) / 256)), dim3(256), 0, ctx->stream, Mt, d_bias,
-                       d_out, H, W, Cout, relu, tiles_x, ntiles);
+  if (!Vn) output_launch(ctx, Mt, d_bias, d_out, H, W, Cout, relu, pool);
   return ls.finish("conv3x3_wino4_split");
+}
+
+static int wino4_split_impl(mnc_ctx* ctx, const float* d_in, const float* d_u, const float* d_bias, float* d_out, void* d_ws, int H,
+                            int W, int Cin, int Cout, int relu, int pool) {
+  MNC_REQUIRE(d_in && d_ws, "mnc_conv3x3_wino4_split: null pointer");
+  return wino4_split_steps(ctx, d_in, d_u, d_bias, d_out, (float*)d_ws, (float*)((char*)d_ws + wino4_split_v_bytes(H, W, Cin)), nullptr,
+                           H, W, Cin, Cout, relu, pool);
 }
 
 }
@@ -225,4 +307,40 @@
   return wino4_split_impl(ctx, d_in, d_u, d_bias, d_out_pooled, d_ws, H, W, Cin, Cout, relu, 1);
 }
 
-}
+int mnc_conv3x3_wino4_split_steps(mnc_ctx* ctx, const float* d_in, const float* d_u, const float* d_bias, float* d_out, float* d_v,
+                                  float* d_m, float* d_v_next, int H, int W, int Cin, int Cout, int relu, int pool) {
+  MNC_REQUIRE(!pool || (H >= 2 && W >= 2), "mnc_conv3x3_wino4_split_steps: map %dx%d too small for MAX 2x2/2", H, W);
+  return wino4_split_steps(ctx, d_in, d_u, d_bias, d_out, d_v, d_m, d_v_next, H, W, Cin, Cout, relu, pool);
+}
+
+int mnc_wino4_split_boundary_supported(int H, int W, int C) { return wino4_split_boundary_supported(H, W, C) ? 1 : 0; }
+
+static bool transform_args_ok(const void* a, const void* b, const void* c, int H, int W, int C, int pool) {
+  return a && b && c && H > 0 && W > 0 && C > 0 && C % 8 == 0 && (!pool || (H >= 2 && W >= 2)) &&
+         36.0 * cdiv(H, 4) * (double)cdiv(W, 4) * C * 4.0 < 2.0e9;
+}
+
+int mnc_wino4_split_input(mnc_ctx* ctx, const float* d_in, float* d_v, int H, int W, int C) {
+  MNC_REQUIRE(ctx && transform_args_ok(d_in, d_v, d_v, H, W, C, 0), "mnc_wino4_split_input: bad argument (C%%8==0)");
+  LaunchScope ls(ctx, "wino4_split_input");
+  input_launch(ctx, d_in, d_v, H, W, C);
+  return ls.finish("wino4_split_input_kernel");
+}
+
+int mnc_wino4_split_output(mnc_ctx* ctx, const float* d_m, const float* d_bias, float* d_out, int H, int W, int C, int relu, int pool) {
+  MNC_REQUIRE(ctx && transform_args_ok(d_m, d_bias, d_out, H, W, C, pool), "mnc_wino4_split_output: bad argument (C%%8==0)");
+  LaunchScope ls(ctx, "wino4_split_output");
+  output_launch(ctx, d_m, d_bias, d_out, H, W, C, relu, pool);
+  return ls.finish("wino4_split_output_kernel");
+}
+
+int mnc_wino4_split_boundary(mnc_ctx* ctx, const float* d_m, const float* d_bias, float* d_out, float* d_v_next, int H, int W, int C,
+                             int relu, int pool) {
+  MNC_REQUIRE(ctx && d_v_next && transform_args_ok(d_m, d_bias, d_out, H, W, C, pool), "mnc_wino4_split_boundary: bad argument (C%%8==0)");
+  LaunchScope ls(ctx, "wino4_split_boundary");
+  const int rc = boundary_launch(ctx, d_m, d_bias, d_out, d_v_next, H, W, C, relu, pool);
+  const int rf = ls.finish("wino4_split_boundary_kernel");
+  return rc ? rc : rf;
+}
+
+}
diff --git a/mnc_amd/csrc/gemm.hip b/mnc_amd/csrc/gemm.hip
--- a/mnc_amd/csrc/gemm.hip
+++ b/mnc_amd/csrc/gemm.hip
@@ -416,14 +416,17 @@
                                                             const float* __restrict__ Wt_1, const float* __restrict__ bias_1,
                                                             float* __restrict__ out_1, int pair_tn, long batch_a,
                                                             long batch_w, long batch_o) {
-  constexpr int kBM = 32 * kMT;
+  constexpr bool HALF = BATCH == 2;
+  constexpr int kBM = HALF ? 16 * kMT : 32 * kMT;
   constexpr int kRows = kBM + kBN;
-  constexpr int kNW = 8;
+  constexpr int kNW = HALF ? 4 : 8;
   constexpr int TS = kMT;
   constexpr int kPer = kRows * 128 / 1024 / kNW;
   static_assert(kRows % (8 * kNW) == 0 && kMT % 2 == 0, "whole pieces and row tiles per wave");
   extern __shared__ __attribute__((aligned(1024))) char s_fc_dma[];
-  constexpr int kBufXor = 65536;
+  constexpr int kBufXor = HALF ? 1024 : 65536;
+  constexpr int kPiece = HALF ? 2048 : 1024;
+  constexpr int kSub = 2 * kPiece;
   const int tid = threadIdx.x, lane = tid & 63;
   const int wave = __builtin_amdgcn_readfirstlane(tid >> 6);
   const int wn = wave & 3, wm = wave >> 2;
@@ -470,7 +473,7 @@
     voff[i] = (r < kBM ? min(r, mrows - 1) * K : (min(n0 + r - kBM, N - 1) - min(n0, N - 1)) * K) * 4 + c * 16;
   }
   auto dma_piece = [&](int i, long off, int buf_byte, bool in_loop = false) {
-    const unsigned l = __builtin_amdgcn_readfirstlane(lds0 + (unsigned)buf_byte + (unsigned)(wave + kNW * i) * 1024u);
+    const unsigned l = __builtin_amdgcn_readfirstlane(lds0 + (unsigned)buf_byte + (unsigned)(wave + kNW * i) * (unsigned)kPiece);
     if (BUF) {
       const bool is_a = (wave + kNW * i) * 8 < kBM;
       const i32x4d rs = is_a ? rs_a : rs_w;
@@ -500,10 +503,10 @@
 #pragma unroll
   for (int G = 0; G < 2; ++G) {
     const int sl = ((4 * G + g4) ^ ((r16 >> 1) & 7)) * 16;
-    a_off[G] = (wm * TS * 16 + r16) * 128 + sl;
-    b_off[G] = (kBM + wn * 32 + r16) * 128 + sl;
-  }
-  const bool last_wave = drop_last && wm == 1;
+    a_off[G] = (HALF ? (r16 >> 3) * kPiece + (r16 & 7) * 128 : (wm * TS * 16 + r16) * 128) + sl;
+    b_off[G] = (HALF ? (kBM / 8 + wn * 4 + (r16 >> 3)) * kPiece + (r16 & 7) * 128 : (kBM + wn * 32 + r16) * 128) + sl;
+  }
+  const bool last_wave = drop_last && wm == (HALF ? 0 : 1);
 
   auto run = [&](auto last_tag) {
     constexpr int NS = decltype(last_tag)::value ? TS - 1 : TS;
@@ -511,15 +514,16 @@
     struct Frags { f32x4v a[NS]; f32x4v b[2]; };
     auto read_frags = [&](int G, int flip, Frags& f) {
       f.b[0] = *reinterpret_cast<const f32x4v*>(s_fc_dma + (b_off[G] ^ flip));
-      f.b[1] = *reinterpret_cast<const f32x4v*>(s_fc_dma + (b_off[G] ^ flip) + 2048);
-#pragma unroll
-      for (int i = 0; i < NS; ++i) f.a[i] = *reinterpret_cast<const f32x4v*>(s_fc_dma + (a_off[G] ^ flip) + i * 2048);
+      f.b[1] = *reinterpret_cast<const f32x4v*>(s_fc_dma + (b_off[G] ^ flip) + kSub);
+#pragma unroll
+      for (int i = 0; i < NS; ++i) f.a[i] = *reinterpret_cast<const f32x4v*>(s_fc_dma + (a_off[G] ^ flip) + i * kSub);
     };
     Frags f0, f1;
     dma_stage(0, 0);
     dma_stage(1, kBufXor);
-    static_assert(kPer == 7, "the literal in the wait below");
-    asm volatile("s_waitcnt vmcnt(7)" ::: "memory");
+    static_assert(kPer == 7 || kPer == 9, "the literals in the wait below");
+    if (kPer == 7) asm volatile("s_waitcnt vmcnt(7)" ::: "memory");
+    else asm volatile("s_waitcnt vmcnt(9)" ::: "memory");
     __syncthreads();
     read_frags(0, 0, f0);
     int cur = 0;
@@ -794,9 +798,18 @@
   MNC_REQUIRE(320.0 * (double)K * 4.0 < 1.8e9 && stride_a % 4 == 0 && stride_w % 4 == 0 &&
                   ((reinterpret_cast<uintptr_t>(d_a) | reinterpret_cast<uintptr_t>(d_w)) & 15) == 0,
               "fc_batch: operands must be 16-byte aligned, K=%d below the descriptor range", K);
-  const int drop = cdiv(M, 304) == cdiv(M, 320) ? 1 : 0;
-  const int tn = cdiv(N, kBN), tm = cdiv(M, drop ? 304 : 320);
+  const int rows = fc_batch_rows(ctx->tune, M);
+  const int drop = cdiv(M, rows - 16) == cdiv(M, rows) ? 1 : 0;
+  const int tn = cdiv(N, kBN), tm = cdiv(M, drop ? rows - 16 : rows);
   MNC_REQUIRE((double)B * tn * tm < 2.0e9, "fc_batch: too many workgroups");
+  if (rows == 160) {
+    constexpr int lds = 2 * (160 + kBN) * 32 * 4;
+    MNC_HIP_TRY((lds_limit_once<fc_mfma_dma16_kernel<10, 0, 1, 2>>(ctx->device, lds)));
+    hipLaunchKernelGGL((fc_mfma_dma16_kernel<10, 0, 1, 2>), dim3(B * tn * tm), dim3(256), lds, ctx->stream, d_a, d_w,
+                       (const float*)nullptr, d_out, (float*)nullptr, M, N, K, ldc, K, 0, 1, tn, tm, B, drop, (const float*)nullptr,
+                       (const float*)nullptr, (const float*)nullptr, (float*)nullptr, 0, stride_a, stride_w, stride_o);
+    return MNC_OK;
+  }
   constexpr int lds = 65536 + (320 + kBN) * 32 * 4;
   MNC_HIP_TRY((lds_limit_once<fc_mfma_dma16_kernel<10, 0, 1, 1>>(ctx->device, lds)));
   hipLaunchKernelGGL((fc_mfma_dma16_kernel<10, 0, 1, 1>), dim3(B * tn * tm), dim3(512), lds, ctx->stream, d_a, d_w, (const float*)nullptr,
diff --git a/mnc_amd/csrc/mnc_internal.h b/mnc_amd/csrc/mnc_internal.h
--- a/mnc_amd/csrc/mnc_internal.h
+++ b/mnc_amd/csrc/mnc_internal.h
@@ -254,6 +254,7 @@
                     int M, int N, int K, int ldc);
 bool wino4_split_supported(int H, int W, int Cin, int Cout);
 bool wino4_split_selected(const mnc_ctx* ctx, int H, int W, int Cin, int Cout);
+bool wino4_split_boundary_supported(int H, int W, int C);
 bool fc_reduce_pair_launch_sm(hipStream_t stream, const float* part0, const float* part1, const float* bias0, const float* bias1,
                               float* out0, float* out1, int M, int N, int ldc, int splits, int act, void* sm0, void* sm1, int sm_fmt,
                               long sm_rows, bool* sm_done);
diff --git a/mnc_amd/csrc/pipeline.hip b/mnc_amd/csrc/pipeline.hip
--- a/mnc_amd/csrc/pipeline.hip
+++ b/mnc_amd/csrc/pipeline.hip
@@ -68,6 +68,8 @@
   DevBuf rois, rois_ext, feat14, h_mask, m14, box7, mask7, f6, f6m, join, heads, boxes, masks, scores;
   DevBuf outblk;
   DevBuf wino_ws;
+  size_t wino_v_bytes = 0;
+  bool split_v_ready = false;
   DevBuf hwc5;
   float* records() const { return (float*)((char*)outblk.p + 512); }
   int* counts() const { return (int*)outblk.p; }
@@ -245,7 +247,7 @@
       }
       const int ws = tune(n->ctx, T_WINO_SPLIT, kWinoSplitDefault);
       if (n->conv_fast[i] && conv_math(c) == 0 && c.winograd == 4 && wino4_split_supported(4, 4, cin, cout) &&
-          (ws == 2 || (ws == 1 && wino4_split_plan_channels(cin, cout)))) {
+          (ws == 2 || ((ws == 1 || ws == 3) && wino4_split_plan_channels(cin, cout)))) {
         void* u = nullptr;
         NET_TRY(mnc_dev_alloc(n->ctx, (size_t)36 * cout * cin * 4, &u));
         n->w_split[i] = (float*)u;
@@ -305,11 +307,13 @@
   NET_TRY(dev_ensure(n, &n->taps, (size_t)(2 * OW + 2 * OH) * 4));
   NET_TRY(dev_ensure(n, &n->data, (size_t)3 * OH * OW * 4));
   int h = OH, w = OW, pi = 0;
-  size_t split_ws = 0;
+  size_t split_v = 0, split_m = 0;
   auto split_need = [&](int i, int hh, int ww, int cin, int cout) {
     if (n->w_split[i] && wino4_split_selected(n->ctx, hh, ww, cin, cout)) {
-      const size_t b = mnc_conv3x3_wino4_split_ws_bytes(hh, ww, cin, cout);
-      if (b > split_ws) split_ws = b;
+      const size_t t36 = (size_t)36 * cdiv(hh, 4) * cdiv(ww, 4) * 4;
+      const size_t v = (t36 * cin + 255) & ~(size_t)255, m = t36 * cout;
+      if (v > split_v) split_v = v;
+      if (m > split_m) split_m = m;
     }
   };
   for (int i = 0; i < 13; ++i) {
@@ -322,7 +326,11 @@
     }
   }
   split_need(13, h, w, c.trunk_channels[4], c.rpn_channels);
-  if (split_ws) NET_TRY(dev_ensure(n, &n->wino_ws, split_ws));
+  if (split_v > n->wino_v_bytes) {
+    n->wino_v_bytes = split_v;
+    if (n->gexec) { (void)hipGraphExecDestroy(n->gexec); n->gexec = nullptr; n->graph_h = n->graph_w = -1; }
+  }
+  if (split_v) NET_TRY(dev_ensure(n, &n->wino_ws, n->wino_v_bytes + split_m));
   const int A = c.num_anchors;
   if (n->packed_trunk) NET_TRY(dev_ensure(n, &n->act12_pk, (size_t)c.trunk_channels[4] * h * w * 4));
   NET_TRY(dev_ensure(n, &n->hwc5, (size_t)c.trunk_channels[4] * h * w * 4));
@@ -395,6 +403,21 @@
   return MNC_OK;
 }
 
+int split_layer(mnc_net* n, int i, const float* in, float* out, int h, int w, int cin, int cout, int pool, bool next_ok) {
+  const mnc_net_config& c = n->cfg;
+  float* V = (float*)n->wino_ws.p;
+  float* M = (float*)((char*)n->wino_ws.p + n->wino_v_bytes);
+  const bool have_v = n->split_v_ready;
+  n->split_v_ready = false;
+  if (next_ok && i < 13 && tune(n->ctx, T_WINO_BOUNDARY, 1) != 0) {
+    const int j = i + 1, nh = pool ? pool_out(h) : h, nw = pool ? pool_out(w) : w;
+    const int ncout = j < 13 ? c.trunk_channels[kTrunkStage[j]] : c.rpn_channels;
+    n->split_v_ready = n->w_split[j] && wino4_split_selected(n->ctx, nh, nw, cout, ncout) && wino4_split_boundary_supported(nh, nw, cout);
+  }
+  return mnc_conv3x3_wino4_split_steps(n->ctx, have_v ? nullptr : in, n->w_split[i], n->b_conv[i], out, V, M,
+                                       n->split_v_ready ? V : nullptr, h, w, cin, cout, 1, pool);
+}
+
 int conv3(mnc_net* n, int i, const float* in, float* out, int h, int w, int cin, int cout) {
   const mnc_net_config& c = n->cfg;
   const int cm = conv_math(c);
@@ -403,7 +426,7 @@
     return mnc_conv2d(n->ctx, in, (const float*)n->w_conv[i], n->b_conv[i], nullptr, out, h, w, cin, cout, 3, 3, 1, 1, 1);
   }
   if (cm == 0 && c.winograd == 4 && n->w_split[i] && wino4_split_selected(n->ctx, h, w, cin, cout))
-    return mnc_conv3x3_wino4_split(n->ctx, in, n->w_split[i], n->b_conv[i], out, n->wino_ws.p, h, w, cin, cout, 1);
+    return split_layer(n, i, in, out, h, w, cin, cout, 0, i == 13 || !kPoolAfter[i]);
   if (cm == 0 && c.winograd == 4)
     return mnc_conv3x3_wino4(n->ctx, in, (const float*)n->w_conv[i], n->b_conv[i], out, h, w, cin, cout, 1);
   if (cm == 0 && c.winograd)
@@ -422,6 +445,7 @@
                          (const int*)(t + 2 * n->OW), t + 2 * n->OW + n->OH, n->OH, (float*)n->data.p, n->OH, n->OW));
   int h = n->OH, w = n->OW, pi = 0, cin = 3;
   const float* cur = (const float*)n->data.p;
+  n->split_v_ready = false;
   if (n->packed_trunk) {
     const int mode = lowp_mode(conv_math(c));
     const void* pc = cur;
@@ -455,7 +479,7 @@
     if (kPoolAfter[i] && i > 0 && conv_math(c) == 0 && c.winograd && n->conv_fast[i]) {
       float* p = (float*)n->pooled[pi++].p;
       if (c.winograd == 4 && n->w_split[i] && wino4_split_selected(ctx, h, w, cin, cout))
-        NET_TRY(mnc_conv3x3_wino4_split_pool(ctx, cur, n->w_split[i], n->b_conv[i], p, n->wino_ws.p, h, w, cin, cout, 1));
+        NET_TRY(split_layer(n, i, cur, p, h, w, cin, cout, 1, true));
       else
       NET_TRY(c.winograd == 4 ? mnc_conv3x3_wino4_pool(ctx, cur, (const float*)n->w_conv[i], n->b_conv[i], p, h, w, cin, cout, 1)
                               : mnc_conv3x3_wino_pool(ctx, cur, (const float*)n->w_conv[i], n->b_conv[i], p, h, w, cin, cout, 1));
diff --git a/mnc_amd/csrc/tune.h b/mnc_amd/csrc/tune.h
--- a/mnc_amd/csrc/tune.h
+++ b/mnc_amd/csrc/tune.h
@@ -6,7 +6,7 @@
   X(CONV_COT) X(CONV_ROWS) X(CONV_KSPLIT) X(CONV_ABL) X(CONV1X1_TILE) X(CONV2D_WIDE) X(WINO_ROWS) X(WINO_TAIL) X(WINO_V) X(WINO_VAR)  \
   X(WINO_DMA) X(WINO_XCD) X(CONVX3_TILE) X(FC_NOTAIL) X(FC_TILE) X(FC_ABL) X(FC_DMA) X(PLAN) X(FC_RANGE_K) X(FC_SLOTS) X(FC_EVEN) X(FC_SPLIT_DIV) X(WINO_FILL) X(CONVX3_P0MIN) X(CONVX3_P1MIN) X(FC_DMA_ABL) X(FC_DMA_WAVES)    \
   X(FC_NO256) X(FCX3_TILE) X(FC_ORDER) X(FCX3_ABL) X(FC_SM) X(PACKED_ACT) X(FUSE_POOLS) X(BRANCH_STREAMS) X(TOPK_SINGLE_WG)           \
-  X(ROI_SM_VARIANT) X(ROI_WARP_VARIANT) X(FC_REDUCE) X(WINO_F4) X(FUSE_SMALL) X(FCX3_WIDE) X(FC_HALF) X(WINO_STREAM) X(FC_MFMA16) X(WINO_MFMA16) X(ROI_ROW_SEGS) X(WINO_SPLIT)
+  X(ROI_SM_VARIANT) X(ROI_WARP_VARIANT) X(FC_REDUCE) X(WINO_F4) X(FUSE_SMALL) X(FCX3_WIDE) X(FC_HALF) X(WINO_STREAM) X(FC_MFMA16) X(WINO_MFMA16) X(ROI_ROW_SEGS) X(WINO_SPLIT) X(FC_BATCH_ROWS) X(WINO_BOUNDARY)
 enum TuneKey {
 #define MNC_TUNE_ENUM(n) T_##n,
   MNC_TUNE_KEYS(MNC_TUNE_ENUM)
@@ -21,6 +21,12 @@
 
 constexpr int kWinoSplitDefault = 1;
 inline bool wino4_split_plan_channels(int Cin, int Cout) { return Cin >= 512 && Cout >= 512; }
+inline bool wino4_split_plan_tiles(int v, int ntiles) { return ntiles >= 304 || (v == 3 && ntiles <= 160); }
+
+inline int fc_batch_rows(const int* t, int M) {
+  const int v = tune(t, T_FC_BATCH_ROWS, 0);
+  return v == 160 || v == 320 ? v : M <= 160 ? 160 : 320;
+}
 
 static inline int cdiv(long a, long b) { return (int)((a + b - 1) / b); }
 }
```

Result: no change. 271.2 images/s (median of 5 runs) (+0.2%).
